# deepsphere/deepsphere-cosmo-tf2

Measured on AMD Instinct MI355X. Metric: Mpix*channels/s Chebyshev-conv fwd, nside=1024 K=5 F=64; HBM roofline %, higher is better.
Workload: dtype f32 (recurrence f32; contraction 3-pass split-bf16 MFMA with f32 accumulate; precision 'bf16x3' = the layer default for 64 input channels)

## Files before the change

deepsphere-cosmo-tf2_amd/csrc/cheb_qstrip_kernel.h:

```cpp
#pragma once

#include <type_traits>

#include "cheb_qtape.h"

namespace dsph {

constexpr int QS_PX = 64;
constexpr int QS_D = 4;
constexpr int QS_USE = QS_PX - 2 * QS_D;
constexpr int QS_THREADS = 512;
constexpr int QS_RUNIN = 2 * QS_D + 1;

struct QStripArgs {
  const float* x;
  const float* bias;
  float* y;
  const unsigned char* wimg;
  const float* gvals8;
  const float* gdiag;
  const QStrip* strips;
  const int32_t* tab;
  const int32_t* prefix;
  int64_t x_rows, y_rows;
  int nstrips, N, Fin, Fout, ld, act;
  int pieces, wg_per_piece;
  float xsc, xsc_inv;
#ifdef DSPH_QS_STAMPS
  unsigned* stamps;
#endif
};

#ifdef DSPH_QS_STAMPS
#define QS_STAMP(id)                                                                                          \
  do {                                                                                                        \
    if (stamp_on) {                                                                                           \
      unsigned long long t_;                                                                                  \
      asm volatile("s_memtime %0\n\ts_waitcnt lgkmcnt(0)" : "=s"(t_)::"memory");                              \
      if (lane == 0) a.stamps[(wave * 4 + (stamp_step & 3)) * 10 + (id)] = (unsigned)t_;                      \
    }                                                                                                         \
  } while (0)
#define QS_STAMP_DECL                                                                                         \
  const int stamp_step = ytop - (st.y0 - D) - 60;                                                             \
  const bool stamp_on = blockIdx.x == 72 && stamp_step >= 0 && stamp_step < 4;
#else
#define QS_STAMP(id)
#define QS_STAMP_DECL
#endif

#ifdef DSPH_QS_ABL
#define QS_ABL DSPH_QS_ABL
#else
#define QS_ABL 0
#endif

#if QS_ABL & 64
#define QS_FD "v_fmac_f32_e32 "
#define QS_DPPL "\n\t"
#define QS_DPPR "\n\t"
#else
#define QS_FD "v_fmac_f32_dpp "
#define QS_DPPL " row_shr:1 row_mask:0xf bank_mask:0xf bound_ctrl:1\n\t"
#define QS_DPPR " row_shl:1 row_mask:0xf bank_mask:0xf bound_ctrl:1\n\t"
#endif

template <bool F16> __device__ __forceinline__ void qs_m(qs_f4& acc, const qs_bf8& wa, const qs_bf8& bb) {
  if (QS_ABL & 2) { asm volatile("" : "+v"(acc) : "v"(wa), "v"(bb) : "memory"); return; }
  if (F16) asm volatile("v_mfma_f32_16x16x32_f16 %0, %1, %2, %0" : "+v"(acc) : "v"(wa), "v"(bb) : "memory");
  else asm volatile("v_mfma_f32_16x16x32_bf16 %0, %1, %2, %0" : "+v"(acc) : "v"(wa), "v"(bb) : "memory");
}
template <bool F16> __device__ __forceinline__ void qs_m0(qs_f4& acc, const qs_bf8& wa, const qs_bf8& bb) {
  if (QS_ABL & 2) { acc = qs_f4{0.f, 0.f, 0.f, 0.f}; asm volatile("" : "+v"(acc) : "v"(wa), "v"(bb) : "memory"); return; }
  if (F16) asm volatile("v_mfma_f32_16x16x32_f16 %0, %1, %2, 0" : "=&v"(acc) : "v"(wa), "v"(bb) : "memory");
  else asm volatile("v_mfma_f32_16x16x32_bf16 %0, %1, %2, 0" : "=&v"(acc) : "v"(wa), "v"(bb) : "memory");
}
template <int N> __device__ __forceinline__ void qs_settle(QRow& r) {
  if (N == 9) asm volatile("s_nop 9" : "+v"(r.t[0]), "+v"(r.t[1]), "+v"(r.t[2]), "+v"(r.t[3]) : : "memory");
  else asm volatile("s_nop 1" : "+v"(r.t[0]), "+v"(r.t[1]), "+v"(r.t[2]), "+v"(r.t[3]) : : "memory");
}

template <bool INIT, bool NEG>
__device__ __forceinline__ void qs_u12(float& a0, float& a1, float& a2, float& a3, float s0, float s1, float s2, float s3,
                                       const qs_f4& cw, const qs_f4& cc, const qs_f4& ce) {
  if ((QS_ABL & 64) && NEG) { qs_u12<INIT, false>(a0, a1, a2, a3, s0, s1, s2, s3, cw, cc, ce); return; }
  const float w0 = cw[0], w1 = cw[1], w2 = cw[2], w3 = cw[3], c0 = cc[0], c1 = cc[1], c2 = cc[2], c3 = cc[3], e0 = ce[0], e1 = ce[1],
              e2 = ce[2], e3 = ce[3];
#define QS_OPS_IN "v"(s0), "v"(s1), "v"(s2), "v"(s3), "v"(w0), "v"(w1), "v"(w2), "v"(w3), "v"(c0), "v"(c1), "v"(c2), "v"(c3), "v"(e0), "v"(e1), "v"(e2), "v"(e3)
  if (!INIT && !NEG)
    asm volatile(
        "v_fmac_f32_e32 %0, %4, %12\n\tv_fmac_f32_e32 %1, %5, %13\n\tv_fmac_f32_e32 %2, %6, %14\n\tv_fmac_f32_e32 %3, %7, %15\n\t"
        "v_fmac_f32_e32 %1, %4, %9\n\tv_fmac_f32_e32 %2, %5, %10\n\tv_fmac_f32_e32 %3, %6, %11\n\t"
        "v_fmac_f32_e32 %0, %5, %16\n\tv_fmac_f32_e32 %1, %6, %17\n\tv_fmac_f32_e32 %2, %7, %18\n\t"
        QS_FD "%0, %7, %8" QS_DPPL QS_FD "%3, %4, %19" QS_DPPR
        : "+v"(a0), "+v"(a1), "+v"(a2), "+v"(a3)
        : QS_OPS_IN
        : "memory");
  else if (!INIT && NEG)
    asm volatile(
        "v_fma_f32 %0, %4, -%12, %0\n\tv_fma_f32 %1, %5, -%13, %1\n\tv_fma_f32 %2, %6, -%14, %2\n\tv_fma_f32 %3, %7, -%15, %3\n\t"
        "v_fma_f32 %1, %4, -%9, %1\n\tv_fma_f32 %2, %5, -%10, %2\n\tv_fma_f32 %3, %6, -%11, %3\n\t"
        "v_fma_f32 %0, %5, -%16, %0\n\tv_fma_f32 %1, %6, -%17, %1\n\tv_fma_f32 %2, %7, -%18, %2\n\t"
        QS_FD "%0, %7, -%8" QS_DPPL QS_FD "%3, %4, -%19" QS_DPPR
        : "+v"(a0), "+v"(a1), "+v"(a2), "+v"(a3)
        : QS_OPS_IN
        : "memory");
  else if (INIT && !NEG)
    asm volatile(
        "v_mul_f32_e32 %0, %4, %12\n\tv_mul_f32_e32 %1, %5, %13\n\tv_mul_f32_e32 %2, %6, %14\n\tv_mul_f32_e32 %3, %7, %15\n\t"
        "v_fmac_f32_e32 %1, %4, %9\n\tv_fmac_f32_e32 %2, %5, %10\n\tv_fmac_f32_e32 %3, %6, %11\n\t"
        "v_fmac_f32_e32 %0, %5, %16\n\tv_fmac_f32_e32 %1, %6, %17\n\tv_fmac_f32_e32 %2, %7, %18\n\t"
        QS_FD "%0, %7, %8" QS_DPPL QS_FD "%3, %4, %19" QS_DPPR
        : "=&v"(a0), "=&v"(a1), "=&v"(a2), "=&v"(a3)
        : QS_OPS_IN
        : "memory");
  else
    asm volatile(
        "v_mul_f32_e64 %0, %4, -%12\n\tv_mul_f32_e64 %1, %5, -%13\n\tv_mul_f32_e64 %2, %6, -%14\n\tv_mul_f32_e64 %3, %7, -%15\n\t"
        "v_fma_f32 %1, %4, -%9, %1\n\tv_fma_f32 %2, %5, -%10, %2\n\tv_fma_f32 %3, %6, -%11, %3\n\t"
        "v_fma_f32 %0, %5, -%16, %0\n\tv_fma_f32 %1, %6, -%17, %1\n\tv_fma_f32 %2, %7, -%18, %2\n\t"
        QS_FD "%0, %7, -%8" QS_DPPL QS_FD "%3, %4, -%19" QS_DPPR
        : "=&v"(a0), "=&v"(a1), "=&v"(a2), "=&v"(a3)
        : QS_OPS_IN
        : "memory");
#undef QS_OPS_IN
}
template <bool INIT, bool NEG>
__device__ __forceinline__ void qs_unit(QRow& acc, const QRow& src, int e, const qs_f4& cw, const qs_f4& cc, const qs_f4& ce) {
  if ((QS_ABL & 4) && !INIT) {
    asm volatile("" : "+v"(acc.t[0]), "+v"(acc.t[1]), "+v"(acc.t[2]), "+v"(acc.t[3]) : "v"(src.t[0]), "v"(src.t[3]), "v"(cw), "v"(cc), "v"(ce) : "memory");
    return;
  }
#define QS_UE(E)                                                                                                          \
  {                                                                                                                       \
    float a0 = 0.f, a1 = 0.f, a2 = 0.f, a3 = 0.f;                                                                         \
    if (!INIT) { a0 = acc.t[0][E]; a1 = acc.t[1][E]; a2 = acc.t[2][E]; a3 = acc.t[3][E]; }                                \
    qs_u12<INIT, NEG>(a0, a1, a2, a3, src.t[0][E], src.t[1][E], src.t[2][E], src.t[3][E], cw, cc, ce);                    \
    acc.t[0][E] = a0; acc.t[1][E] = a1; acc.t[2][E] = a2; acc.t[3][E] = a3;                                               \
  }
  if (e == 0) QS_UE(0)
  else if (e == 1) QS_UE(1)
  else if (e == 2) QS_UE(2)
  else QS_UE(3)
#undef QS_UE
}

#define QS_UPR 4
#define QS_UNIT qs_unit

__host__ __device__ constexpr float qs_wsign(bool cheb, int j) { return cheb && ((j & 3) >= 2) ? -1.f : 1.f; }

template <bool CHEB, bool F16>
__global__ __launch_bounds__(QS_THREADS, 2) void cheb_qstrip5_kernel(QStripArgs a) {
  constexpr int K = 5, D = QS_D, RING = K + 2;
#ifdef DSPH_QS_NOH1
  constexpr bool H1 = false;
#else
  constexpr bool H1 = CHEB;
#endif
  constexpr int ROWB = 2 * 2 * 4 * QS_FRAG;
  constexpr int RINGB = RING * ROWB;
  constexpr int HAND1 = 2 * 4 * QS_FRAG;
  constexpr int HANDB = 4 * HAND1;
  constexpr int CRING = K + 1;
  constexpr int CRINGB = CRING * QS_CROWB;
  constexpr int LDS_HAND = RINGB, LDS_C = RINGB + HANDB, LDS_FLAG = LDS_C + CRINGB;
  __shared__ __attribute__((aligned(16))) unsigned char smem[LDS_FLAG + 64];

  const int tid = threadIdx.x, lane = tid & 63;
  const int wave = __builtin_amdgcn_readfirstlane(tid >> 6);
  const bool roleL = wave >= 4;
  const int oq = wave & 3;
  const int p = lane & 15, q4 = lane >> 4;
  const unsigned lane16 = (unsigned)lane * 16u;
  const unsigned hand = (unsigned)LDS_HAND + (unsigned)oq * HAND1 + lane16;
  const unsigned flag_addr = (unsigned)LDS_FLAG + 4u * (unsigned)oq;
  auto flag_set = [&](int v) __attribute__((always_inline)) { qt_flag_set(flag_addr, v); };
  auto flag_get = [&]() __attribute__((always_inline)) -> int { return qt_flag_get(flag_addr); };
  for (int i = tid; i < (LDS_FLAG + 64) / 16; i += QS_THREADS) reinterpret_cast<qs_f4*>(smem)[i] = qs_f4{0.f, 0.f, 0.f, 0.f};

  const QTapePiece wg = qt_piece(a.wg_per_piece);
  if (wg.piece >= a.pieces) return;
  const QTapeRange tape = qt_tape_range(a.prefix, a.nstrips, wg.piece, a.pieces);
  auto locate = [&](int64_t r, int64_t r_end, QStrip& st) __attribute__((always_inline)) -> int {
    return qt_locate(a.prefix, a.strips, a.nstrips, r, r_end, st);
  };
  const unsigned xrowb = (unsigned)a.Fin * 4u, yrowb = (unsigned)a.ld * 4u;

#if defined(DSPH_QS_XALL)
  constexpr bool X_BY_H = false;
#elif defined(DSPH_QS_XBYH)
  constexpr bool X_BY_H = true;
#else
  constexpr bool X_BY_H = !H1;
#endif
  constexpr int XN = X_BY_H ? 4 : 2;
  const int xt = wave & 3, xpix = X_BY_H ? ((lane >> 1) & 15) : (((lane >> 1) & 7) + 8 * (wave >> 2));
  const unsigned x_goff = X_BY_H ? (unsigned)(2 * (lane >> 5) + (lane & 1)) * 16u
                                 : (unsigned)(lane >> 5) * 64u + (unsigned)(2 * ((lane >> 4) & 1) + (lane & 1)) * 16u;
  const unsigned x_loff = (unsigned)xt * QS_FRAG + (unsigned)(lane & 1) * 8u +
                          (X_BY_H ? (unsigned)(xpix + 16 * (lane >> 5)) * 16u : (unsigned)(xpix + 16 * (2 * (lane >> 5) + ((lane >> 4) & 1))) * 16u);
  auto tab_lane = [&](const QStrip& st, unsigned ci, int yrow) __attribute__((always_inline)) -> unsigned {
    return qt_tab_lane(a.tab, st, ci, min(max(yrow, st.ylo), st.yhi));
  };
  auto my_of = [&](int yrow) __attribute__((always_inline)) -> unsigned { return st_spread((unsigned)yrow & 15u) << 1; };
  auto my_next = [&](unsigned m) __attribute__((always_inline)) -> unsigned { return ((m | 0x55u) + 1u) & 0xaau; };
  auto xfetch = [&](const char* xmap, unsigned xrow, qs_f4 (&xv)[XN]) __attribute__((always_inline)) {
    if (QS_ABL & 8) {
#pragma unroll
      for (int i = 0; i < XN; ++i) xv[i] = qs_f4{0.f, 0.f, 0.f, 0.f};
      return;
    }
    const char* src = xmap + (size_t)(xrow * xrowb + x_goff);
#pragma unroll
    for (int i = 0; i < XN; ++i) xv[i] = *reinterpret_cast<const qs_f4*>(src + (X_BY_H ? 64 : 128) * i);
  };
  auto xw_wait = [&](qs_f4 (&xv)[XN]) __attribute__((always_inline)) {
    if (X_BY_H) asm volatile("" : "+v"(xv[0]), "+v"(xv[1]), "+v"(xv[XN - 2]), "+v"(xv[XN - 1]) : : "memory");
    else asm volatile("" : "+v"(xv[0]), "+v"(xv[1]) : : "memory");
  };
  auto xstore = [&](int slot, const qs_f4 (&xv)[XN]) __attribute__((always_inline)) {
    if (QS_ABL & 4096) {
#pragma unroll
      for (int i = 0; i < XN; ++i) asm volatile("" : : "v"(xv[i]));
      return;
    }
    unsigned char* q = smem + (unsigned)slot * ROWB + x_loff;
#pragma unroll
    for (int i = 0; i < XN; ++i) {
      const unsigned fo = X_BY_H ? (unsigned)(i >> 1) * (2 * 4 * QS_FRAG) + (unsigned)(i & 1) * (32u * 16u) : (unsigned)i * (2 * 4 * QS_FRAG);
      qs_u2 hi, lo;
#pragma unroll
      for (int j = 0; j < 2; ++j) {
        const float a0 = F16 ? xv[i][2 * j] * a.xsc : xv[i][2 * j], a1 = F16 ? xv[i][2 * j + 1] * a.xsc : xv[i][2 * j + 1];
        const qs_u2 hl = qt_split<F16>(a0, a1);
        hi[j] = hl[0];
        lo[j] = hl[1];
      }
      *reinterpret_cast<qs_u2*>(q + fo) = hi;
      *reinterpret_cast<qs_u2*>(q + fo + 4 * QS_FRAG) = lo;
    }
  };
  auto cfetch = [&](unsigned rid, qs_f4& cv, float& cd) __attribute__((always_inline)) { qt_cfetch(a.gvals8, a.gdiag, rid, q4, cv, cd); };
  auto cw_wait = [&](qs_f4& cv, float& cd) __attribute__((always_inline)) {
    asm volatile("" : "+v"(cv), "+v"(cd) : : "memory");
  };
  auto cstore = [&](int slot, qs_f4 cv, float cd) __attribute__((always_inline)) {
    if (CHEB) { cv = cv + cv; cd = cd + cd; }
    unsigned char* q = smem + LDS_C + (unsigned)slot * QS_CROWB + (unsigned)p * 16u + (unsigned)oq * 4u;
    if (q4 < 2) {
#pragma unroll
      for (int d = 0; d < 4; ++d) *reinterpret_cast<float*>(q + (unsigned)(1 + 4 * q4 + d) * 256u) = cv[d];
    }
    if (q4 == 2) *reinterpret_cast<float*>(q) = cd;
  };
  constexpr bool C_OFF = (QS_ABL & 1024) != 0;
  auto clo_read = [&](int slot) __attribute__((always_inline)) -> QCoefLo { return qt_clo_read<C_OFF>(smem + LDS_C, slot, p); };
  auto chi_read = [&](int slot) __attribute__((always_inline)) -> QCoefHi { return qt_chi_read<C_OFF>(smem + LDS_C, slot, p); };

#if QS_ABL & 512
#define QS_FRLOAD(P) (wr[0][0][0])
#else
#define QS_FRLOAD(P) (*reinterpret_cast<const qs_bf8*>(P))
#endif
#define QS_ORD_A(j) ((j) == 1 ? 1 : 0)
#define QS_ORD_B(j) ((j) == 0 ? 1 : 0)
#define QS_FR0(FADDR)                                                                                                     \
  _Pragma("unroll") for (int u = 0; u < 2; ++u) {                                                                         \
    fr[0][u][0] = QS_FRLOAD(smem + (FADDR) + (unsigned)u * QS_FRAG);                                                      \
    fr[0][u][1] = QS_FRLOAD(smem + (FADDR) + (unsigned)(4 + u) * QS_FRAG);                                                \
  }
#define QS_SETS(S0, S1, ROW, ZERO, WLEV, FADDR, NU, ...)                                                                  \
  _Pragma("unroll") for (int s = (S0); s < (S1); ++s) {                 \
    if (s + 1 < 4) {                                                                                                      \
      _Pragma("unroll") for (int u = 0; u < 2; ++u) {                                                                     \
        const unsigned fo = (unsigned)(((s + 1) >> 1) * 8 + ((s + 1) & 1) * 2 + u) * QS_FRAG;                             \
        fr[(s + 1) & 1][u][0] = QS_FRLOAD(smem + (FADDR) + fo);                                                           \
        fr[(s + 1) & 1][u][1] = QS_FRLOAD(smem + (FADDR) + fo + 4 * QS_FRAG);                                             \
      }                                                                                                                   \
    }                                                                                                                     \
    _Pragma("unroll") for (int j = 0; j < 3; ++j) {                                                                       \
      _Pragma("unroll") for (int u = 0; u < 2; ++u) {                                                                     \
        const int m = (s * 3 + j) * 2 + u;                                                                                \
        const int tt = (s & 1) * 2 + u;                                                                                   \
        const qs_bf8& wa_ = wr[WLEV][s >> 1][QS_ORD_A(j)];                                                                \
        const qs_bf8& bb_ = fr[s & 1][u][QS_ORD_B(j)];                                                                    \
        if ((ZERO) && s < 2 && j == 0) qs_m0<F16>((ROW).t[tt], wa_, bb_);                                                 \
        else qs_m<F16>((ROW).t[tt], wa_, bb_);                                                                            \
        _Pragma("unroll") for (int qq = (m * (NU)) / 18; qq < ((m + 1) * (NU)) / 18 && m < 18; ++qq) { __VA_ARGS__; }     \
      }                                                                                                                   \
    }                                                                                                                     \
  }
#define QS_CHAIN(ROW, ZERO, WLEV, FADDR, NU, TAIL, ...)                                                                   \
  {                                                                                                                       \
    QS_SETS(0, 3, ROW, ZERO, WLEV, FADDR, NU, __VA_ARGS__)                                                                \
    TAIL;                                                                                                                 \
    QS_SETS(3, 4, ROW, ZERO, WLEV, FADDR, NU, __VA_ARGS__)                                                                \
  }

  __syncthreads();

  if (!roleL) {
    qs_bf8 wr[4][2][2];
    if (H1) {
      const unsigned char* wp1 = a.wimg + ((size_t)(1 * 4 + oq) * 3) * (2 * 2 * QS_FRAG) + lane16;
#pragma unroll
      for (int kb = 0; kb < 2; ++kb)
#pragma unroll
        for (int h = 0; h < 2; ++h) wr[3][kb][h] = *reinterpret_cast<const qs_bf8*>(wp1 + (size_t)(kb * 2 + h) * QS_FRAG);
    }
    {
      const unsigned char* wp = a.wimg + ((size_t)(0 * 4 + oq) * 3) * (2 * 2 * QS_FRAG) + lane16;
#pragma unroll
      for (int l = 0; l < 3; ++l)
#pragma unroll
        for (int kb = 0; kb < 2; ++kb)
#pragma unroll
          for (int h = 0; h < 2; ++h) wr[l][kb][h] = *reinterpret_cast<const qs_bf8*>(wp + ((size_t)(l * 2 + kb) * 2 + h) * QS_FRAG);
    }
    int handed = 0;
    for (int64_t tr = tape.begin; tr < tape.end;) {
      QStrip st;
      tr += locate(tr, tape.end, st);
      for (int nq = wg.map0; nq < a.N; nq += a.wg_per_piece) {
      const int Xc = min(max(st.xs + 4 * p + oq, st.xlo), st.xhi);
      const int Xf = min(max(st.xs + 4 * xpix + xt, st.xlo), st.xhi);
      const int tc0 = max(st.xs, st.xlo) >> 4;
      const unsigned ciC = (unsigned)((Xc >> 4) - tc0), mXc = st_spread((unsigned)Xc & 15u);
      const unsigned ciF = (unsigned)((Xf >> 4) - tc0), mXf = st_spread((unsigned)Xf & 15u);
      const int T3 = ((st.y1 - st.y0) + 2 * D + 1 + 3) / 3;
      const char* __restrict__ xmap = reinterpret_cast<const char*>(a.x) + (size_t)nq * a.x_rows * xrowb;
      QRow R[2][3];
#pragma unroll
      for (int i = 0; i < 2; ++i)
#pragma unroll
        for (int s = 0; s < 3; ++s)
#pragma unroll
          for (int t = 0; t < 4; ++t) R[i][s].t[t] = qs_f4{0.f, 0.f, 0.f, 0.f};
      int ytop = st.y0 - D, slot_top = 0, cs_top = 0;
      qt_step_barrier();
      {
        qs_f4 cv, xv[XN];
        float cd;
        cfetch(qt_row_in(st, tab_lane(st, ciC, ytop - 1), mXc, ytop - 1), cv, cd);
        xfetch(xmap, qt_row_in(st, tab_lane(st, ciF, ytop), mXf, ytop), xv);
        cw_wait(cv, cd);
        cstore(CRING - 1, cv, cd);
        xw_wait(xv);
        xstore(0, xv);
      }
      unsigned bXf = tab_lane(st, ciF, ytop + 1), bXc = tab_lane(st, ciC, ytop);
      unsigned myX = my_of(ytop + 1), myC = my_of(ytop);
      qt_step_barrier();
      auto step = [&](auto ph_c) __attribute__((always_inline)) {
        constexpr int PH = decltype(ph_c)::value;
        constexpr int L0 = PH % 3, L1 = (PH + 1) % 3, L2 = (PH + 2) % 3;
        int snew = slot_top + 1;
        snew = snew == RING ? 0 : snew;
        auto slot_ix = [&](int back) __attribute__((always_inline)) -> int {
          int s = slot_top - back;
          s += s < 0 ? RING : 0;
          return s;
        };
        auto cslot_ix = [&](int back) __attribute__((always_inline)) -> int {
          int s = cs_top - back;
          s += s < 0 ? CRING : 0;
          return s;
        };
        QS_STAMP_DECL
        QS_STAMP(0);
        qs_f4 xv[XN];
        constexpr bool XLATE = H1;
        if (myX == 0) bXf = tab_lane(st, ciF, ytop + 1);
        if (myC == 0) bXc = tab_lane(st, ciC, ytop);
        if (!XLATE) xfetch(xmap, bXf + (mXf | myX), xv);
        const unsigned f0 = (unsigned)slot_top * ROWB + lane16, f1 = (unsigned)slot_ix(1) * ROWB + lane16, f2 = (unsigned)slot_ix(2) * ROWB + lane16;
        const unsigned f3 = (unsigned)slot_ix(3) * ROWB + lane16;
        constexpr bool N3 = CHEB;
        qs_bf8 fr[2][2][2];
        QCoefLo c3 = clo_read(cslot_ix(1));
        QS_FR0(f0)
        QCoefLo c2;
        QCoefHi c3h, c2h;
        qs_f4 cv;
        float cd;
        QS_CHAIN(R[0][L2], true, 0, f0, 2 * QS_UPR, { c2 = clo_read(cslot_ix(2)); QS_FR0(f1) },
                 { if (qq < QS_UPR) QS_UNIT<true, N3>(R[1][L2], R[0][L0], qq, QS_LO0(c3)); else QS_UNIT<false, N3>(R[1][L2], R[0][L1], qq - QS_UPR, QS_LO1(c3)); })
        qs_settle<9>(R[0][L2]);
        qs_settle<1>(R[1][L2]);
        QS_STAMP(1);
        QS_CHAIN(R[1][L2], false, 1, f1, 2 * QS_UPR, { c3h = chi_read(cslot_ix(1)); QS_FR0(f2) },
                 { if (qq < QS_UPR) QS_UNIT<!CHEB, false>(R[0][L0], R[1][L0], qq, QS_LO0(c2)); else QS_UNIT<false, false>(R[0][L0], R[1][L1], qq - QS_UPR, QS_LO1(c2)); })
        qs_settle<9>(R[1][L2]);
        qs_settle<1>(R[0][L0]);
        if (XLATE) xfetch(xmap, bXf + (mXf | myX), xv);
        QS_STAMP(2);
        QS_CHAIN(R[0][L0], false, 2, f2, QS_UPR, { c2h = chi_read(cslot_ix(2)); cfetch(bXc + (mXc | myC), cv, cd); if (H1) { QS_FR0(f3) } },
                 { QS_UNIT<false, N3>(R[1][L2], R[0][L2], qq, QS_HI(c3h)); })
        qs_settle<9>(R[0][L0]);
        qs_settle<1>(R[1][L2]);
        QS_STAMP(3);
        if (H1) {
          QS_CHAIN(R[1][L0], false, 3, f3, QS_UPR, {}, { QS_UNIT<false, false>(R[0][L0], R[1][L2], qq, QS_HI(c2h)); })
          qs_settle<9>(R[1][L0]);
        } else {
#pragma unroll
          for (int qq = 0; qq < QS_UPR; ++qq) QS_UNIT<false, false>(R[0][L0], R[1][L2], qq, QS_HI(c2h));
        }
        QS_STAMP(4);
        for (int spin = 0; flag_get() <= handed && spin < (1 << 22); ++spin) {}
        if (!(QS_ABL & 2048)) {
          unsigned char* hp = smem + hand;
#pragma unroll
          for (int t = 0; t < 4; ++t) {
            *reinterpret_cast<qs_f4*>(hp + t * QS_FRAG) = R[0][L0].t[t];
            if (CHEB) *reinterpret_cast<qs_f4*>(hp + (4 + t) * QS_FRAG) = R[1][L0].t[t];
          }
        }
        ++handed;
        QS_STAMP(5);
        xw_wait(xv);
        cw_wait(cv, cd);
        QS_STAMP(6);
        cstore(cs_top, cv, cd);
        xstore(snew, xv);
        QS_STAMP(7);
        slot_top = snew;
        cs_top = cs_top + 1 == CRING ? 0 : cs_top + 1;
        ++ytop;
        myX = my_next(myX);
        myC = my_next(myC);
        qt_step_barrier();
        QS_STAMP(8);
      };
      for (int t3 = 0; t3 < T3; ++t3) {
        step(std::integral_constant<int, 0>{});
        step(std::integral_constant<int, 1>{});
        step(std::integral_constant<int, 2>{});
      }
      }
    }
  } else {
    qs_bf8 wr[2][2][2];
    {
      const unsigned char* wp = a.wimg + ((size_t)(1 * 4 + oq) * 3) * (2 * 2 * QS_FRAG) + lane16;
#pragma unroll
      for (int l = 0; l < 2; ++l)
#pragma unroll
        for (int kb = 0; kb < 2; ++kb)
#pragma unroll
          for (int h = 0; h < 2; ++h) wr[l][kb][h] = *reinterpret_cast<const qs_bf8*>(wp + ((size_t)(l * 2 + kb) * 2 + h) * QS_FRAG);
    }
    const float floor_v = a.act == DSPH_ACT_RELU ? 0.f : -__builtin_huge_valf();
    const float ysc = (CHEB ? 0.5f : 1.f) * (F16 ? *reinterpret_cast<const float*>(a.wimg + 2 * 4 * 3 * 2 * 2 * QS_FRAG) * a.xsc_inv : 1.f);
#ifdef DSPH_QS_LPRIO
#define QS_STR2(x) #x
#define QS_STR(x) QS_STR2(x)
    asm volatile("s_setprio " QS_STR(DSPH_QS_LPRIO));
#endif
    qs_f4 bv = qs_f4{0.f, 0.f, 0.f, 0.f};
    if (a.bias != nullptr) bv = *reinterpret_cast<const qs_f4*>(a.bias + 16 * oq + 4 * q4);
    int taken = 0;
    for (int64_t tr = tape.begin; tr < tape.end;) {
      QStrip st;
      tr += locate(tr, tape.end, st);
      for (int nq = wg.map0; nq < a.N; nq += a.wg_per_piece) {
      const int Xf = min(max(st.xs + 4 * xpix + xt, st.xlo), st.xhi);
      const int tc0 = max(st.xs, st.xlo) >> 4;
      const unsigned ciF = (unsigned)((Xf >> 4) - tc0), mXf = st_spread((unsigned)Xf & 15u);
      const int Xg = st.xs + 4 * p;
      const unsigned ciY = (unsigned)((min(max(Xg, st.xlo), st.xhi) >> 4) - tc0), mXg = st_spread((unsigned)Xg & 12u);
      const int cfirst = st.x0 - st.xs, clast = cfirst + st.w;
      const int T3 = ((st.y1 - st.y0) + 2 * D + 1 + 3) / 3;
      const char* __restrict__ xmap = reinterpret_cast<const char*>(a.x) + (size_t)nq * a.x_rows * xrowb;
      char* __restrict__ ymap = reinterpret_cast<char*>(a.y) + (size_t)nq * a.y_rows * yrowb;
      QRow R[2][3], Y;
#pragma unroll
      for (int i = 0; i < 2; ++i)
#pragma unroll
        for (int s = 0; s < 3; ++s)
#pragma unroll
          for (int t = 0; t < 4; ++t) R[i][s].t[t] = qs_f4{0.f, 0.f, 0.f, 0.f};
#pragma unroll
      for (int t = 0; t < 4; ++t) Y.t[t] = qs_f4{0.f, 0.f, 0.f, 0.f};
      int ytop = st.y0 - D, slot_top = 0, cs_top = 0;
      qt_step_barrier();
      if (!X_BY_H) {
        qs_f4 xv[XN];
        xfetch(xmap, qt_row_in(st, tab_lane(st, ciF, ytop), mXf, ytop), xv);
        xw_wait(xv);
        xstore(0, xv);
      }
      unsigned bXf = X_BY_H ? 0u : tab_lane(st, ciF, ytop + 1), bY = tab_lane(st, ciY, st.y0);
      unsigned myX = my_of(ytop + 1), myY = my_of(ytop - K);
      qt_step_barrier();
      auto step = [&](auto ph_c) __attribute__((always_inline)) {
        constexpr int PH = decltype(ph_c)::value;
        constexpr int L0 = PH % 3, L1 = (PH + 1) % 3, L2 = (PH + 2) % 3;
        int snew = slot_top + 1;
        snew = snew == RING ? 0 : snew;
        auto slot_ix = [&](int back) __attribute__((always_inline)) -> int {
          int s = slot_top - back;
          s += s < 0 ? RING : 0;
          return s;
        };
        auto cslot_ix = [&](int back) __attribute__((always_inline)) -> int {
          int s = cs_top - back;
          s += s < 0 ? CRING : 0;
          return s;
        };
        QS_STAMP_DECL
        QS_STAMP(0);
        qs_f4 xv[XN];
        if (!X_BY_H && myX == 0) bXf = tab_lane(st, ciF, ytop + 1);
        if (myY == 0) bY = tab_lane(st, ciY, ytop - K);
        if (!X_BY_H) xfetch(xmap, bXf + (mXf | myX), xv);
#ifdef DSPH_QS_LEARLY
        constexpr bool LE = CHEB && H1;
#else
        constexpr bool LE = false;
#endif
        QCoefLo c0;
        QCoefHi c0h;
        if (LE) c0 = clo_read(cslot_ix(5));
        if (!(QS_ABL & 2048)) {
          const unsigned char* hp = smem + hand;
#pragma unroll
          for (int t = 0; t < 4; ++t) {
            R[0][L2].t[t] = *reinterpret_cast<const qs_f4*>(hp + t * QS_FRAG);
            if (CHEB) R[1][L2].t[t] = *reinterpret_cast<const qs_f4*>(hp + (4 + t) * QS_FRAG);
          }
        }
        ++taken;
        flag_set(taken);
        const unsigned f1 = (unsigned)slot_ix(4) * ROWB + lane16, f0 = (unsigned)slot_ix(5) * ROWB + lane16;
        constexpr bool N1 = CHEB;
        QS_STAMP(1);
        qs_bf8 fr[2][2][2];
        if (LE) {
#pragma unroll
          for (int t = 0; t < 4; ++t) Y.t[t] = R[0][L0].t[t] + R[0][L0].t[t];
          qs_settle<1>(Y);
#pragma unroll
          for (int qq = 0; qq < 2 * QS_UPR; ++qq) {
            if (qq < QS_UPR) QS_UNIT<false, false>(Y, R[1][L0], qq, QS_LO0(c0)); else QS_UNIT<false, false>(Y, R[1][L1], qq - QS_UPR, QS_LO1(c0));
          }
          qs_settle<1>(Y);
        }
        const QCoefLo c1 = clo_read(cslot_ix(4));
        const QCoefHi c1h = chi_read(cslot_ix(4));
        QS_FR0(f0)
#ifdef DSPH_QS_LBARE
        if (CHEB && H1) {
          c0 = clo_read(cslot_ix(5));
          c0h = chi_read(cslot_ix(5));
#pragma unroll
          for (int qq = 0; qq < 3 * QS_UPR; ++qq) {
            if (qq < QS_UPR) QS_UNIT<false, N1>(R[1][L2], R[0][L0], qq, QS_LO0(c1));
            else if (qq < 2 * QS_UPR) QS_UNIT<false, N1>(R[1][L2], R[0][L1], qq - QS_UPR, QS_LO1(c1));
            else QS_UNIT<false, N1>(R[1][L2], R[0][L2], qq - 2 * QS_UPR, QS_HI(c1h));
          }
#pragma unroll
          for (int t = 0; t < 4; ++t) Y.t[t] = R[0][L0].t[t] + R[0][L0].t[t];
          qs_settle<1>(Y);
#pragma unroll
          for (int qq = 0; qq < 2 * QS_UPR; ++qq) {
            if (qq < QS_UPR) QS_UNIT<false, false>(Y, R[1][L0], qq, QS_LO0(c0)); else QS_UNIT<false, false>(Y, R[1][L1], qq - QS_UPR, QS_LO1(c0));
          }
          qs_settle<1>(R[1][L2]);
#pragma unroll
          for (int qq = 0; qq < QS_UPR; ++qq) QS_UNIT<false, false>(Y, R[1][L2], qq, QS_HI(c0h));
          qs_settle<1>(Y);
          QS_STAMP(2);
          QS_CHAIN(Y, false, 1, f0, 0, {}, {})
          qs_settle<9>(Y);
          QS_STAMP(3);
        } else
#endif
        {
        if (CHEB && !LE) {
#pragma unroll
          for (int t = 0; t < 4; ++t) Y.t[t] = R[0][L0].t[t] + R[0][L0].t[t];
          qs_settle<1>(Y);
        }
        QS_CHAIN(Y, !CHEB, 1, f0, 3 * QS_UPR, { if (!LE) c0 = clo_read(cslot_ix(5)); else c0h = chi_read(cslot_ix(5)); if (!H1) { QS_FR0(f1) } },
                 { if (qq < QS_UPR) QS_UNIT<!CHEB, N1>(R[1][L2], R[0][L0], qq, QS_LO0(c1));
                   else if (qq < 2 * QS_UPR) QS_UNIT<false, N1>(R[1][L2], R[0][L1], qq - QS_UPR, QS_LO1(c1));
                   else QS_UNIT<false, N1>(R[1][L2], R[0][L2], qq - 2 * QS_UPR, QS_HI(c1h)); })
        qs_settle<9>(Y);
        qs_settle<1>(R[1][L2]);
        QS_STAMP(2);
        if (H1 && LE) {
        } else if (H1) {
          c0h = chi_read(cslot_ix(5));
#pragma unroll
          for (int qq = 0; qq < 2 * QS_UPR; ++qq) {
            if (qq < QS_UPR) QS_UNIT<false, false>(Y, R[1][L0], qq, QS_LO0(c0)); else QS_UNIT<false, false>(Y, R[1][L1], qq - QS_UPR, QS_LO1(c0));
          }
        } else {
          QS_CHAIN(R[1][L2], false, 0, f1, 2 * QS_UPR, { c0h = chi_read(cslot_ix(5)); },
                   { if (qq < QS_UPR) QS_UNIT<false, false>(Y, R[1][L0], qq, QS_LO0(c0)); else QS_UNIT<false, false>(Y, R[1][L1], qq - QS_UPR, QS_LO1(c0)); })
        }
        qs_settle<9>(R[1][L2]);
        QS_STAMP(3);
#pragma unroll
        for (int qq = 0; qq < QS_UPR; ++qq) QS_UNIT<false, false>(Y, R[1][L2], qq, QS_HI(c0h));
        }
        QS_STAMP(4);
        if (!X_BY_H) xw_wait(xv);
        QS_STAMP(5);
        {
          const int yr = ytop - K;
          const bool row_ok = yr >= st.y0 && yr < ((QS_ABL & 16) ? st.y0 + 1 : st.y1);
          const unsigned rowg = bY + (mXg | myY);
#pragma unroll
          for (int t = 0; t < 4; ++t) {
            const int c = 4 * p + t;
            if (row_ok && c >= cfirst && c < clast) {
              qs_f4 o;
#pragma unroll
              for (int e = 0; e < 4; ++e) {
                const float v = fmaf(Y.t[t][e], ysc, bv[e]);
                o[e] = F16 ? (v < floor_v ? floor_v : v) : fmaxf(v, floor_v);
              }
              *reinterpret_cast<qs_f4*>(ymap + (size_t)(rowg + (unsigned)((t & 1) + 4 * (t >> 1))) * yrowb + (unsigned)(16 * oq + 4 * q4) * 4u) = o;
            }
          }
        }
        QS_STAMP(6);
        if (!X_BY_H) xstore(snew, xv);
        QS_STAMP(7);
        slot_top = snew;
        cs_top = cs_top + 1 == CRING ? 0 : cs_top + 1;
        ++ytop;
        myX = my_next(myX);
        myY = my_next(myY);
        qt_step_barrier();
        QS_STAMP(8);
      };
      for (int t3 = 0; t3 < T3; ++t3) {
        step(std::integral_constant<int, 0>{});
        step(std::integral_constant<int, 1>{});
        step(std::integral_constant<int, 2>{});
      }
      }
    }
  }
#undef QS_CHAIN
#undef QS_SETS
#undef QS_FR0
#undef QS_FRLOAD
}

}
```

deepsphere-cosmo-tf2_amd/csrc/cheb_qtape.h:

```cpp
#pragma once

#include <algorithm>

#include "cheb_struct_kernel.h"
#include "dsphere_common.h"

namespace dsph {

constexpr int QS_FRAG = 1024;
constexpr int QS_CROWB = 2304;

typedef float qs_f4 __attribute__((ext_vector_type(4)));
typedef int qs_i4 __attribute__((ext_vector_type(4)));
typedef __bf16 qs_bf8 __attribute__((ext_vector_type(8)));
typedef unsigned qs_u2 __attribute__((ext_vector_type(2)));

struct QRow {
  qs_f4 t[4];
};

struct QStrip {
  int32_t x0, w;
  int32_t xs;
  int32_t y0, y1;
  int32_t xlo, xhi;
  int32_t ylo, yhi;
  int32_t tab, tws;
  int32_t pad[1];
};

struct QTapePiece {
  int ord, piece, map0;
};
__device__ __forceinline__ QTapePiece qt_piece(int wg_per_piece) {
  QTapePiece c;
  const int G = gridDim.x;
  c.ord = (blockIdx.x & 7) * (G >> 3) + (blockIdx.x >> 3);
  c.piece = c.ord / wg_per_piece;
  c.map0 = c.ord - c.piece * wg_per_piece;
  return c;
}
struct QTapeRange {
  int64_t begin, end;
};
__device__ __forceinline__ QTapeRange qt_tape_range(const int32_t* prefix, int nstrips, int piece, int pieces) {
  const int64_t tape = (int64_t)prefix[nstrips];
  QTapeRange r;
  r.begin = piece < pieces ? tape * piece / pieces : 0;
  r.end = piece < pieces ? tape * (piece + 1) / pieces : 0;
  return r;
}
__device__ __forceinline__ int qt_locate(const int32_t* prefix, const QStrip* strips, int nstrips, int64_t r, int64_t r_end, QStrip& st) {
  int lo = 0, hi = nstrips;
  while (hi - lo > 1) {
    const int mid = (lo + hi) >> 1;
    if ((int64_t)prefix[mid] <= r) lo = mid; else hi = mid;
  }
  {
    const QStrip g = strips[lo];
#define QS_U(f) st.f = __builtin_amdgcn_readfirstlane(g.f)
    QS_U(x0); QS_U(w); QS_U(xs); QS_U(y0); QS_U(y1); QS_U(xlo); QS_U(xhi); QS_U(ylo); QS_U(yhi); QS_U(tab); QS_U(tws);
#undef QS_U
  }
  const int h = st.y1 - st.y0;
  const int off = (int)(r - (int64_t)prefix[lo]);
  const int len = (int)(((int64_t)(h - off) < r_end - r) ? (int64_t)(h - off) : r_end - r);
  st.y0 += off;
  st.y1 = st.y0 + len;
  return len;
}

__device__ __forceinline__ unsigned qt_tab_lane(const int32_t* tab, const QStrip& st, unsigned ci, int yc) {
  const int32_t* trow = tab + __builtin_amdgcn_readfirstlane(st.tab + (yc >> 4) * st.tws + (max(st.xs, st.xlo) >> 4));
  qs_i4 b;
  int b4;
  asm volatile("s_load_dwordx4 %0, %2, 0x0\n\ts_load_dword %1, %2, 0x10\n\ts_waitcnt lgkmcnt(0)" : "=&s"(b), "=&s"(b4) : "s"(trow) : "memory");
  return (unsigned)(ci == 0 ? b[0] : ci == 1 ? b[1] : ci == 2 ? b[2] : ci == 3 ? b[3] : b4);
}
__device__ __forceinline__ unsigned qt_row_in(const QStrip& st, unsigned base, unsigned mX, int yrow) {
  const int yc = min(max(yrow, st.ylo), st.yhi);
  return base + (mX | (st_spread((unsigned)yc & 15u) << 1));
}

__device__ __forceinline__ void qt_step_barrier() { asm volatile("s_waitcnt lgkmcnt(0)\n\ts_barrier" ::: "memory"); }
__device__ __forceinline__ void qt_flag_set(unsigned addr, int v) { asm volatile("ds_write_b32 %0, %1" : : "v"(addr), "v"(v) : "memory"); }
__device__ __forceinline__ int qt_flag_get(unsigned addr) {
  int v;
  asm volatile("ds_read_b32 %0, %1\n\ts_waitcnt lgkmcnt(0)" : "=v"(v) : "v"(addr) : "memory");
  return v;
}

template <bool F16> __device__ __forceinline__ qs_u2 qt_split(float a0, float a1) {
  typedef __bf16 bf16x2 __attribute__((ext_vector_type(2)));
  typedef _Float16 f16x2 __attribute__((ext_vector_type(2)));
  typedef float f32x2 __attribute__((ext_vector_type(2)));
  qs_u2 r;
  if (F16) {
    const f16x2 h = __builtin_convertvector(f32x2{a0, a1}, f16x2);
    const f32x2 hf = __builtin_convertvector(h, f32x2);
    const f16x2 l = __builtin_convertvector(f32x2{a0 - hf[0], a1 - hf[1]}, f16x2);
    r[0] = __builtin_bit_cast(unsigned, h);
    r[1] = __builtin_bit_cast(unsigned, l);
  } else {
    const bf16x2 h = __builtin_convertvector(f32x2{a0, a1}, bf16x2);
    const unsigned hu = __builtin_bit_cast(unsigned, h);
    const float h0 = __builtin_bit_cast(float, hu << 16), h1 = __builtin_bit_cast(float, hu & 0xffff0000u);
    const bf16x2 l = __builtin_convertvector(f32x2{a0 - h0, a1 - h1}, bf16x2);
    r[0] = hu;
    r[1] = __builtin_bit_cast(unsigned, l);
  }
  return r;
}

struct QCoef3 {
  qs_f4 w, c, e;
};
struct QCoefLo {
  qs_f4 sw, s, se, w, dg, e;
};
struct QCoefHi {
  qs_f4 nw, n, ne;
};
#define QS_LO0(c) (c).sw, (c).s, (c).se
#define QS_LO1(c) (c).w, (c).dg, (c).e
#define QS_HI(c) (c).nw, (c).n, (c).ne

__device__ __forceinline__ void qt_cfetch(const float* gvals8, const float* gdiag, size_t rid, int q4, qs_f4& cv, float& cd) {
  const char* pv = reinterpret_cast<const char*>(gvals8) + rid * 32u + (unsigned)(q4 & 1) * 16u;
  const char* pd = reinterpret_cast<const char*>(gdiag) + rid * 4u;
  cv = *reinterpret_cast<const qs_f4*>(pv);
  cd = *reinterpret_cast<const float*>(pd);
}
template <bool DOUBLE>
__device__ __forceinline__ void qt_cstore(unsigned char* ring, int slot, int p, int q4, int res, qs_f4 cv, float cd) {
  if (DOUBLE) { cv = cv + cv; cd = cd + cd; }
  unsigned char* q = ring + (unsigned)slot * QS_CROWB + (unsigned)p * 16u + (unsigned)res * 4u;
  if (q4 < 2) {
#pragma unroll
    for (int d = 0; d < 4; ++d) *reinterpret_cast<float*>(q + (unsigned)(1 + 4 * q4 + d) * 256u) = cv[d];
  }
  if (q4 == 2) *reinterpret_cast<float*>(q) = cd;
}
__device__ __forceinline__ const unsigned char* qt_crow(const unsigned char* ring, int slot, int p) {
  return ring + (unsigned)slot * QS_CROWB + (unsigned)p * 16u;
}
template <bool NOREAD = false> __device__ __forceinline__ qs_f4 qt_cvec(const unsigned char* q, int v) {
  if (NOREAD) { qs_f4 c = qs_f4{0.1f, 0.1f, 0.1f, 0.1f}; asm volatile("" : "+v"(c)); return c; }
  return *reinterpret_cast<const qs_f4*>(q + (unsigned)v * 256u);
}
template <bool NOREAD = false> __device__ __forceinline__ QCoef3 qt_cvec3(const unsigned char* q, int which) {
  QCoef3 r;
  if (which == 0) { r.w = qt_cvec<NOREAD>(q, 8); r.c = qt_cvec<NOREAD>(q, 7); r.e = qt_cvec<NOREAD>(q, 6); }
  else if (which == 1) { r.w = qt_cvec<NOREAD>(q, 1); r.c = qt_cvec<NOREAD>(q, 0); r.e = qt_cvec<NOREAD>(q, 5); }
  else { r.w = qt_cvec<NOREAD>(q, 2); r.c = qt_cvec<NOREAD>(q, 3); r.e = qt_cvec<NOREAD>(q, 4); }
  return r;
}
template <bool NOREAD = false> __device__ __forceinline__ QCoefLo qt_clo_read(const unsigned char* ring, int slot, int p) {
  const unsigned char* q = qt_crow(ring, slot, p);
  QCoefLo c;
  c.sw = qt_cvec<NOREAD>(q, 8); c.s = qt_cvec<NOREAD>(q, 7); c.se = qt_cvec<NOREAD>(q, 6);
  c.w = qt_cvec<NOREAD>(q, 1); c.dg = qt_cvec<NOREAD>(q, 0); c.e = qt_cvec<NOREAD>(q, 5);
  return c;
}
template <bool NOREAD = false> __device__ __forceinline__ QCoefHi qt_chi_read(const unsigned char* ring, int slot, int p) {
  const unsigned char* q = qt_crow(ring, slot, p);
  QCoefHi c;
  c.nw = qt_cvec<NOREAD>(q, 2); c.n = qt_cvec<NOREAD>(q, 3); c.ne = qt_cvec<NOREAD>(q, 4);
  return c;
}

__device__ __forceinline__ float qt_wimg_pow2(const float* __restrict__ w, int nrows, int ncols, int ld) {
  __shared__ float smax[256];
  float m = 0.f;
  for (int e = threadIdx.x; e < nrows * ncols; e += 256) m = fmaxf(m, fabsf(w[(int64_t)(e / ncols) * ld + e % ncols]));
  smax[threadIdx.x] = m;
  __syncthreads();
  for (int st = 128; st > 0; st >>= 1) {
    if ((int)threadIdx.x < st) smax[threadIdx.x] = fmaxf(smax[threadIdx.x], smax[threadIdx.x + st]);
    __syncthreads();
  }
  int ex = 0;
  const float mx = smax[0];
  float pw = 1.f;
  if (mx > 0.f && mx < 3.0e38f) { (void)frexpf(mx, &ex); pw = ldexpf(1.f, 12 - ex); }
  return pw;
}
__device__ __forceinline__ void qt_wimg_put(unsigned char* base, int idx, float v, bool f16) {
  if (f16) {
    const _Float16 hi = (_Float16)v;
    const _Float16 lo = (_Float16)(v - (float)hi);
    reinterpret_cast<_Float16*>(base)[idx] = hi;
    reinterpret_cast<_Float16*>(base + QS_FRAG)[idx] = lo;
  } else {
    const __bf16 hi = (__bf16)v;
    const __bf16 lo = (__bf16)(v - (float)hi);
    reinterpret_cast<__bf16*>(base)[idx] = hi;
    reinterpret_cast<__bf16*>(base + QS_FRAG)[idx] = lo;
  }
}

template <class Args, class Launch> int qtape_args(Args& a, const Launch& s, int run_in) {
  a.x = s.x;
  a.gvals8 = s.gvals8;
  a.gdiag = s.gdiag;
  a.strips = s.strips;
  a.tab = s.tab;
  a.prefix = s.prefix;
  a.x_rows = s.x_rows;
  a.nstrips = s.nstrips;
  a.N = (int)s.N;
  int grid;
  (void)qtape_split(s.num_cu, s.tape_rows, s.N, s.tape_rows / std::max(1, s.nstrips), run_in, &grid, &a.pieces, &a.wg_per_piece);
  return grid;
}
template <class Args> int qtape_forward_args(Args& a, const QTapeLaunch& s, int run_in) {
  a.bias = s.bias;
  a.y = s.y;
  a.wimg = s.wimg;
  a.y_rows = s.y_rows;
  a.ld = s.ld;
  a.act = s.act;
  a.xsc = s.f16 ? ldexpf(1.f, s.f16_xexp) : 1.f;
  a.xsc_inv = s.f16 ? ldexpf(1.f, -s.f16_xexp) : 1.f;
  return qtape_args(a, s, run_in);
}

}
```

deepsphere-cosmo-tf2_amd/csrc/cheb_qwgrad_kernel.h:

```cpp
#pragma once

#include "cheb_qstrip_kernel.h"

namespace dsph {

#ifdef DSPH_QW_PAD
constexpr bool QW_SWZ = false;
constexpr int QW_SK = 272, QW_SB = 1216;
#else
constexpr bool QW_SWZ = true;
constexpr int QW_SK = 256;
constexpr int QW_SB = 1040;
#endif
constexpr int QW_CG = 2 * QW_SB;
constexpr int QW_HL = 4 * QW_CG;
constexpr int QW_PLANE = 2 * QW_HL;
constexpr int QW_P0 = 0, QW_P2 = 1, QW_Q0 = 2, QW_Q1 = 3, QW_Q2 = 4, QW_NPLANES = 5;
constexpr int QW_PAIRS = 5;
constexpr int QW_SLAB = QW_PAIRS * 64 * 64;

struct QWgradArgs {
  const float* x;
  const float* dy;
  float* slabs;
  const float* gvals8;
  const float* gdiag;
  const QStrip* strips;
  const int32_t* tab;
  const int32_t* prefix;
  int64_t x_rows, dy_rows;
  int nstrips, N, lddy;
  int pieces, wg_per_piece;
};

template <bool CHEB>
__global__ __launch_bounds__(QS_THREADS, 2) void cheb_qwgrad5_kernel(QWgradArgs a) {
  constexpr int D = QS_D;
  constexpr int CRING = 3;
  constexpr int LDS_C = QW_NPLANES * QW_PLANE;
  __shared__ __attribute__((aligned(16))) unsigned char smem[LDS_C + CRING * QS_CROWB];

  const int tid = threadIdx.x, lane = tid & 63;
  const int wave = __builtin_amdgcn_readfirstlane(tid >> 6);
  const bool sideQ = wave >= 4;
  const int cq = wave & 3;
  const int og = wave & 3, fh = wave >> 2;
  const int p = lane & 15, q4 = lane >> 4;
  for (int i = tid; i < (int)sizeof(smem) / 16; i += QS_THREADS) reinterpret_cast<qs_f4*>(smem)[i] = qs_f4{0.f, 0.f, 0.f, 0.f};

  const QTapePiece wg = qt_piece(a.wg_per_piece);
  float* __restrict__ slab = a.slabs + (size_t)blockIdx.x * QW_SLAB;
  const float sgn = (sideQ && (wg.ord & 1)) ? -1.f : 1.f;
  qs_f4 acc[QW_PAIRS][2];
#pragma unroll
  for (int i = 0; i < QW_PAIRS; ++i)
#pragma unroll
    for (int j = 0; j < 2; ++j) acc[i][j] = qs_f4{0.f, 0.f, 0.f, 0.f};

  const QTapeRange tape = qt_tape_range(a.prefix, a.nstrips, wg.piece, a.pieces);
  auto locate = [&](int64_t r, int64_t r_end, QStrip& st) __attribute__((always_inline)) -> int {
    return qt_locate(a.prefix, a.strips, a.nstrips, r, r_end, st);
  };

  const unsigned srowb = sideQ ? (unsigned)a.lddy * 4u : 256u;
  const int64_t srows = sideQ ? a.dy_rows : a.x_rows;
  const char* sbase = reinterpret_cast<const char*>(sideQ ? a.dy : a.x);
  const int kgw = (p >> 1) & 3;
  const unsigned wr_com = (unsigned)cq * QW_CG + (unsigned)(p >> 3) * QW_SB + (unsigned)kgw * QW_SK + (unsigned)(p & 1) * 8u +
                          (unsigned)(4 * (QW_SWZ ? (q4 ^ (kgw >> 1)) : q4)) * 16u;
  const unsigned wr_a = wr_com + ((QW_SWZ && (kgw & 1)) ? 32u : 0u), wr_b = wr_com + ((QW_SWZ && (kgw & 1)) ? 0u : 32u);
  const unsigned rd_off = (unsigned)(lane >> 4) * QW_SK + (unsigned)((lane & 15) ^ (QW_SWZ ? 2 * (lane >> 4) : 0)) * 16u;

  auto cstore = [&](int slot, qs_f4 cv, float cd) __attribute__((always_inline)) { qt_cstore<false>(smem + LDS_C, slot, p, q4, cq, cv, cd); };
  auto crow = [&](int slot, int which) __attribute__((always_inline)) -> QCoef3 { return qt_cvec3(qt_crow(smem + LDS_C, slot, p), which); };

  auto stage = [&](int plane, const QRow& R) __attribute__((always_inline)) {
    if (QS_ABL & 8192) { asm volatile("" : : "v"(R.t[0]), "v"(R.t[1]), "v"(R.t[2]), "v"(R.t[3])); return; }
    unsigned char* qa = smem + (unsigned)plane * QW_PLANE + wr_a;
    unsigned char* qb = smem + (unsigned)plane * QW_PLANE + wr_b;
#pragma unroll
    for (int cc = 0; cc < 4; ++cc) {
      unsigned char* q = (cc < 2 ? qa : qb) + (cc & 1) * 16;
      qs_u2 hi, lo;
#pragma unroll
      for (int j = 0; j < 2; ++j) {
        const float a0 = R.t[2 * j][cc], a1 = R.t[2 * j + 1][cc];
        const qs_u2 hl = qt_split<false>(a0, a1);
        hi[j] = hl[0];
        lo[j] = hl[1];
      }
      *reinterpret_cast<qs_u2*>(q) = hi;
      *reinterpret_cast<qs_u2*>(q + QW_HL) = lo;
    }
  };
  auto frag = [&](int plane, int hl, int cg, int blk) __attribute__((always_inline)) -> qs_bf8 {
    if (QS_ABL & 16384) { qs_bf8 z; asm volatile("v_mov_b32 %0, 0" : "=v"(z)); return z; }
    return *reinterpret_cast<const qs_bf8*>(smem + (unsigned)plane * QW_PLANE + (unsigned)hl * QW_HL + (unsigned)cg * QW_CG + (unsigned)blk * QW_SB + rd_off);
  };

  __syncthreads();

  for (int64_t tr = tape.begin; tr < tape.end;) {
    QStrip st;
    tr += locate(tr, tape.end, st);
    for (int nq = wg.map0; nq < a.N; nq += a.wg_per_piece) {
      unsigned voff[4];
      bool colk[4];
      const int cfirst = st.x0 - st.xs, clast = cfirst + st.w;
      const int xclo = sideQ ? st.x0 : st.xlo, xchi = sideQ ? st.x0 + st.w - 1 : st.xhi;
#pragma unroll
      for (int t = 0; t < 4; ++t) {
        voff[t] = st_spread((unsigned)min(max(st.xs + 4 * p + t, xclo), xchi) & 15u) * srowb + (unsigned)(16 * cq + 4 * q4) * 4u;
        colk[t] = !sideQ || (4 * p + t >= cfirst && 4 * p + t < clast);
      }
      const int Xc = min(max(st.xs + 4 * p + cq, st.xlo), st.xhi);
      const int tc0 = max(st.xs, st.xlo) >> 4;
      const unsigned pk = (unsigned)((min(max(st.xs + 4 * p, xclo), xchi) >> 4) - tc0) | ((unsigned)((Xc >> 4) - tc0) << 4) | (st_spread((unsigned)Xc & 15u) << 8);
      const char* smap = sbase + (size_t)nq * srows * srowb;
      auto tab_lane = [&](unsigned ci, int yc) __attribute__((always_inline)) -> unsigned { return qt_tab_lane(a.tab, st, ci, yc); };
      const int rlo = sideQ ? st.y0 : st.ylo, rhi = sideQ ? st.y1 - 1 : st.yhi;
      unsigned bV = tab_lane(pk & 15u, min(max(st.y0 - D, rlo), rhi)), bC = sideQ ? 0u : tab_lane((pk >> 4) & 15u, min(max(st.y0 - D, st.ylo), st.yhi));
      auto row_fetch = [&](int yrow, QRow& R) __attribute__((always_inline)) {
        const int yc = min(max(yrow, rlo), rhi);
        if (yrow > rlo && yrow <= rhi && (yrow & 15) == 0) bV = tab_lane(pk & 15u, yc);
        const unsigned rb = (bV + (st_spread((unsigned)yc & 15u) << 1)) * srowb;
#pragma unroll
        for (int t = 0; t < 4; ++t) R.t[t] = *reinterpret_cast<const qs_f4*>(smap + (rb + voff[t]));
      };
      const int T3 = ((st.y1 - st.y0) + 2 * D + 1 + 2) / 3;
      QRow S0[3], S1[3];
#pragma unroll
      for (int s = 0; s < 3; ++s)
#pragma unroll
        for (int t = 0; t < 4; ++t) { S0[s].t[t] = qs_f4{0.f, 0.f, 0.f, 0.f}; S1[s].t[t] = qs_f4{0.f, 0.f, 0.f, 0.f}; }
      int ytop = st.y0 - D, cs = 0;
      QRow nx;
      row_fetch(ytop, nx);
      qs_f4 cv = qs_f4{0.f, 0.f, 0.f, 0.f};
      float cd = 0.f;
      auto coef_fetch = [&](int yrow) __attribute__((always_inline)) {
        const int yc = min(max(yrow, st.ylo), st.yhi);
        if (yrow > st.ylo && yrow <= st.yhi && (yrow & 15) == 0) bC = tab_lane((pk >> 4) & 15u, yc);
        const size_t rid = bC + ((pk >> 8) | (st_spread((unsigned)yc & 15u) << 1));
        qt_cfetch(a.gvals8, a.gdiag, rid, q4, cv, cd);
      };
      if (!sideQ) coef_fetch(ytop);

      auto step = [&](auto ph_c) __attribute__((always_inline)) {
        constexpr int PH = decltype(ph_c)::value;
        constexpr int L0 = PH % 3, L1 = (PH + 1) % 3, L2 = (PH + 2) % 3;
        const int cs1 = cs == 0 ? 2 : cs - 1, cs2 = cs1 == 0 ? 2 : cs1 - 1;
        QRow A2;
        QCoef3 ca = crow(cs2, 0), cb = crow(cs2, 1);
        auto unit = [&](auto u_c) __attribute__((always_inline)) {
          constexpr int u = decltype(u_c)::value;
          if (u < 4) QS_UNIT<true, false>(A2, S1[L0], u, ca.w, ca.c, ca.e);
          else if (u < 8) QS_UNIT<false, false>(A2, S1[L1], u - 4, cb.w, cb.c, cb.e);
          else if (u < 12) QS_UNIT<true, false>(S1[L2], S0[L0], u - 8, ca.w, ca.c, ca.e);
          else if (u < 16) QS_UNIT<false, false>(S1[L2], S0[L1], u - 12, cb.w, cb.c, cb.e);
          else if (u < 20) QS_UNIT<false, false>(S1[L2], S0[L2], u - 16, ca.w, ca.c, ca.e);
          else QS_UNIT<false, false>(A2, S1[L2], u - 20, cb.w, cb.c, cb.e);
          if (u == 3) ca = crow(cs1, 0);
          if (u == 7) cb = crow(cs1, 1);
          if (u == 11) ca = crow(cs1, 2);
          if (u == 15) {
            cb = crow(cs2, 2);
            const bool rowk = !sideQ || (ytop >= st.y0 && ytop < st.y1);
            float one = sgn;
            asm volatile("" : "+v"(one));
#pragma unroll
            for (int t = 0; t < 4; ++t) {
              const float mk = (rowk && colk[t]) ? one : 0.f;
#pragma unroll
              for (int e = 0; e < 4; ++e) S0[L2].t[t][e] = nx.t[t][e] * mk;
            }
          }
          if (u == 19) qs_settle<1>(S1[L2]);
        };
        qs_bf8 fa[2][2], fb[2][2];
#pragma unroll
        for (int g = 0; g < 2; ++g)
#pragma unroll
          for (int h = 0; h < 2; ++h) fa[g][h] = frag(QW_P0, h, 2 * fh + g, 0);
#pragma unroll
        for (int h = 0; h < 2; ++h) fb[0][h] = frag(QW_Q0, h, og, 0);
        auto group = [&](auto gi_c) __attribute__((always_inline)) {
          constexpr int gi = decltype(gi_c)::value, blk = gi / 5, g = gi % 5;
          constexpr int pair = g == 0 ? 0 : g == 1 ? 1 : g == 2 ? 3 : g == 3 ? 2 : 4;
          constexpr int bb = (g == 0 || g == 3) ? 0 : 1;
          if (g == 0) { fb[1][0] = frag(QW_Q1, 0, og, blk); fb[1][1] = frag(QW_Q1, 1, og, blk); }
          if (g == 1) { fb[0][0] = frag(QW_Q0, 0, og, blk); fb[0][1] = frag(QW_Q0, 1, og, blk); }
          if (g == 2) {
#pragma unroll
            for (int gg = 0; gg < 2; ++gg)
#pragma unroll
              for (int h = 0; h < 2; ++h) fa[gg][h] = frag(QW_P2, h, 2 * fh + gg, blk);
          }
          if (g == 3) { fb[1][0] = frag(QW_Q2, 0, og, blk); fb[1][1] = frag(QW_Q2, 1, og, blk); }
          if (g == 0 && blk == 1) {
#pragma unroll
            for (int gg = 0; gg < 2; ++gg)
#pragma unroll
              for (int h = 0; h < 2; ++h) fa[gg][h] = frag(QW_P0, h, 2 * fh + gg, 1);
          }
          if (g == 4 && blk == 0) { fb[0][0] = frag(QW_Q0, 0, og, 1); fb[0][1] = frag(QW_Q0, 1, og, 1); }
          auto mf = [&](auto i_c) __attribute__((always_inline)) {
            constexpr int i = decltype(i_c)::value, j = i >> 1, fg = i & 1, m = gi * 6 + i;
            qs_m<false>(acc[pair][fg], fa[fg][j == 1 ? 1 : 0], fb[bb][j == 0 ? 1 : 0]);
            if constexpr (m % 5 == 1 || m % 5 == 3) unit(std::integral_constant<int, 2 * (m / 5) + (m % 5 == 3 ? 1 : 0)>{});
          };
          mf(std::integral_constant<int, 0>{}); mf(std::integral_constant<int, 1>{}); mf(std::integral_constant<int, 2>{});
          mf(std::integral_constant<int, 3>{}); mf(std::integral_constant<int, 4>{}); mf(std::integral_constant<int, 5>{});
        };
        group(std::integral_constant<int, 0>{}); group(std::integral_constant<int, 1>{}); group(std::integral_constant<int, 2>{});
        group(std::integral_constant<int, 3>{}); group(std::integral_constant<int, 4>{}); group(std::integral_constant<int, 5>{});
        group(std::integral_constant<int, 6>{}); group(std::integral_constant<int, 7>{}); group(std::integral_constant<int, 8>{});
        group(std::integral_constant<int, 9>{});
        QRow S2;
#pragma unroll
        for (int t = 0; t < 4; ++t)
#pragma unroll
          for (int e = 0; e < 4; ++e) S2.t[t][e] = CHEB ? fmaf(2.f, A2.t[t][e], -S0[L0].t[t][e]) : A2.t[t][e];
        qt_step_barrier();
        asm volatile("" : : "v"(fa[0][0]), "v"(fa[0][1]), "v"(fa[1][0]), "v"(fa[1][1]), "v"(fb[1][0]), "v"(fb[1][1]), "v"(fb[0][0]), "v"(fb[0][1]));
        if (!sideQ) {
          stage(QW_P0, S0[L0]);
          stage(QW_P2, S2);
        } else {
          stage(QW_Q0, S0[L0]);
          stage(QW_Q1, S1[L1]);
          stage(QW_Q2, S2);
        }
        if (!sideQ) cstore(cs, cv, cd);
        row_fetch(ytop + 1, nx);
        if (!sideQ) coef_fetch(ytop + 1);
        cs = cs == 2 ? 0 : cs + 1;
        ++ytop;
        qt_step_barrier();
      };
      for (int t3 = 0; t3 < T3; ++t3) {
        step(std::integral_constant<int, 0>{});
        step(std::integral_constant<int, 1>{});
        step(std::integral_constant<int, 2>{});
      }
    }
  }
#pragma unroll
  for (int i = 0; i < QW_PAIRS; ++i)
#pragma unroll
    for (int j = 0; j < 2; ++j) asm volatile("s_nop 9\n\ts_nop 9" : "+v"(acc[i][j]) : : "memory");
#pragma unroll
  for (int pr = 0; pr < QW_PAIRS; ++pr)
#pragma unroll
    for (int fg = 0; fg < 2; ++fg)
#pragma unroll
      for (int i = 0; i < 4; ++i)
        slab[((size_t)pr * 64 + (size_t)(16 * (2 * fh + fg) + 4 * (lane >> 4) + i)) * 64 + (size_t)(16 * og + (lane & 15))] = acc[pr][fg][i];
}

}
```

deepsphere-cosmo-tf2_amd/csrc/cheb_struct.hip:

```cpp
#include <stdio.h>
#include <stdlib.h>

#include <algorithm>
#include <vector>

#include "cheb_struct_kernel.h"

namespace dsph {

__host__ __device__ inline void struct_row_body(int64_t r, const int32_t* __restrict__ cols, const float* __restrict__ vals, int W,
                                                int64_t n_rows, float* __restrict__ gvals8, float* __restrict__ gdiag,
                                                unsigned char* __restrict__ flag) {
  constexpr int kDirIndex[9] = {8, 7, 6, 1, 0, 5, 2, 3, 4};
  float out[9];
#pragma unroll
  for (int d = 0; d < 9; ++d) out[d] = 0.f;
  bool ok = r < n_rows;
  if (ok) {
    const int X = (int)st_compress((unsigned)r), Y = (int)st_compress((unsigned)r >> 1);
    unsigned used = 0;
    for (int j = 0; j < W; ++j) {
      const float v = vals[r * W + j];
      if (v == 0.f) continue;
      const unsigned c = (unsigned)cols[r * W + j];
      const int dx = (int)st_compress(c) - X, dy = (int)st_compress(c >> 1) - Y;
      if (dx < -1 || dx > 1 || dy < -1 || dy > 1) { ok = false; continue; }
      const int d = kDirIndex[(dy + 1) * 3 + (dx + 1)];
      if (used & (1u << d)) ok = false;
      used |= 1u << d;
#pragma unroll
      for (int e = 0; e < 9; ++e)
        if (e == d) out[e] = v;
    }
  }
  gdiag[r] = out[0];
#pragma unroll
  for (int d = 0; d < 8; ++d) gvals8[r * 8 + d] = out[d + 1];
  flag[r] = ok ? 1 : 0;
}
__global__ __launch_bounds__(256) void struct_rows_kernel(const int32_t* __restrict__ cols, const float* __restrict__ vals,
                                                          int W, int64_t n_rows, int64_t n_cols,
                                                          float* __restrict__ gvals8, float* __restrict__ gdiag,
                                                          unsigned char* __restrict__ flag) {
  const int64_t r = (int64_t)blockIdx.x * 256 + threadIdx.x;
  if (r >= n_cols) return;
  struct_row_body(r, cols, vals, W, n_rows, gvals8, gdiag, flag);
}

__host__ __device__ inline unsigned char struct_tile_body(int t, const unsigned char* __restrict__ flag, int D, int64_t n_rows,
                                                          int64_t n_cols, int64_t out_rows, int dlimit) {
  const int64_t row0 = (int64_t)t * 256;
  bool ok = D >= 1 && D <= dlimit && row0 + 256 <= out_rows && row0 + 256 <= 0xffffffffLL;
  bool interior = true;
  if (ok) {
    const int X0 = (int)st_compress((unsigned)row0), Y0 = (int)st_compress((unsigned)row0 >> 1);
    if (X0 - D < 0 || Y0 - D < 0 || X0 + ST_TILE + D > 65535 || Y0 + ST_TILE + D > 65535) ok = false;
    for (int gy = -D; ok && gy < ST_TILE + D; ++gy)
      for (int gx = -D; gx < ST_TILE + D; ++gx) {
        const int a = -gx > gx - (ST_TILE - 1) ? -gx : gx - (ST_TILE - 1), b = -gy > gy - (ST_TILE - 1) ? -gy : gy - (ST_TILE - 1);
        const int ring = (a > b ? a : b) > 0 ? (a > b ? a : b) : 0;
        const int64_t rid = (int64_t)st_morton((unsigned)(X0 + gx), (unsigned)(Y0 + gy));
        if (rid >= n_cols) { ok = false; break; }
        if (ring < D && (rid >= n_rows || !flag[rid])) { ok = false; break; }
        if (rid >= out_rows) interior = false;
      }
  }
  return (unsigned char)((ok ? 1 : 0) | (interior ? 2 : 0));
}
__global__ __launch_bounds__(256) void struct_tiles_kernel(const unsigned char* __restrict__ flag, int ntiles, int D,
                                                           int64_t n_rows, int64_t n_cols, int64_t out_rows,
                                                           unsigned char* __restrict__ cls, int dlimit) {
  const int t = blockIdx.x * 256 + threadIdx.x;
  if (t >= ntiles) return;
  cls[t] = struct_tile_body(t, flag, D, n_rows, n_cols, out_rows, dlimit);
}

__global__ __launch_bounds__(256) void struct_wprep_kernel(const float* __restrict__ w, unsigned char* __restrict__ out,
                                                           int Fin, int Fout, int K, int C, int NB, int prec, int ld, int pack) {
  const int blk = blockIdx.x;
  const int nb = blk % NB, k = (blk / NB) % K, c = blk / (NB * K);
  unsigned char* base = out + (size_t)blk * (prec == DSPH_PREC_BF16X6 ? ST_WBLK3 : 2048);
  for (int e = threadIdx.x; e < 512; e += 256) {
    const int l = e >> 3, j = e & 7;
    const int ch = c * 16 + 8 * (l >> 5) + j, col = 32 * nb + (l & 31);
    float v;
    if (pack) {
      const int ci = 16 / pack, cm = 64 / pack;
      v = (ch / ci == col / cm && ch % ci < Fin && col % cm < Fout) ? w[((int64_t)(ch % ci) * K + k) * ld + col % cm] : 0.f;
    }
    else v = (ch < Fin && col < Fout) ? w[((int64_t)ch * K + k) * ld + col] : 0.f;
    if (prec == DSPH_PREC_BF16X6) {
      const unsigned u = __float_as_uint(v);
      const float r = v - __uint_as_float(u & 0xffff0000u);
      const unsigned s = __float_as_uint(r);
      const float q = r - __uint_as_float(s & 0xffff0000u);
      reinterpret_cast<unsigned short*>(base)[l * 8 + j] = (unsigned short)(u >> 16);
      reinterpret_cast<unsigned short*>(base + 1024)[l * 8 + j] = (unsigned short)(s >> 16);
      reinterpret_cast<unsigned short*>(base + 2048)[l * 8 + j] = (unsigned short)(__float_as_uint(q) >> 16);
    } else if (prec == DSPH_PREC_BF16X3) {
      const __bf16 hi = (__bf16)v;
      const __bf16 lo = (__bf16)(v - (float)hi);
      reinterpret_cast<__bf16*>(base)[l * 8 + j] = hi;
      reinterpret_cast<__bf16*>(base + 1024)[l * 8 + j] = lo;
    } else {
      reinterpret_cast<float*>(base + (j >> 2) * 1024)[l * 4 + (j & 3)] = v;
    }
  }
}

int struct_build_rows(const dsph_plan* plan, float** gvals8, float** gdiag, unsigned char** flag) {
  const int64_t n = plan->n_cols;
  DSPH_HIP(hipMalloc((void**)gvals8, (size_t)n * 8 * sizeof(float)));
  DSPH_HIP(hipMalloc((void**)gdiag, (size_t)n * sizeof(float)));
  DSPH_HIP(hipMalloc((void**)flag, (size_t)n));
#ifdef DSPH_HOST_EMU
  for (int64_t r = 0; r < n; ++r) struct_row_body(r, plan->d_cols, plan->d_vals, (int)plan->width, plan->n_rows, *gvals8, *gdiag, *flag);
#else
  hipLaunchKernelGGL(struct_rows_kernel, dim3((unsigned)((n + 255) / 256)), dim3(256), 0, 0, plan->d_cols, plan->d_vals,
                     (int)plan->width, plan->n_rows, plan->n_cols, *gvals8, *gdiag, *flag);
#endif
  DSPH_HIP(hipGetLastError());
  DSPH_HIP(hipDeviceSynchronize());
  return DSPH_OK;
}

__host__ __device__ inline void struct_patch_body(int64_t i, const int32_t* __restrict__ rows, const float* __restrict__ vals,
                                                  float* __restrict__ gvals8, float* __restrict__ gdiag) {
  const int64_t r = rows[i];
  gdiag[r] = vals[9 * i];
#pragma unroll
  for (int d = 0; d < 8; ++d) gvals8[r * 8 + d] = vals[9 * i + 1 + d];
}
__global__ __launch_bounds__(256) void struct_patch_kernel(const int32_t* __restrict__ rows, const float* __restrict__ vals, int64_t n,
                                                           float* __restrict__ gvals8, float* __restrict__ gdiag) {
  const int64_t i = (int64_t)blockIdx.x * 256 + threadIdx.x;
  if (i < n) struct_patch_body(i, rows, vals, gvals8, gdiag);
}
int struct_patch_rows(const dsph_plan* plan, float* gvals8, float* gdiag, const int32_t* rows, const float* vals, int64_t n) {
  (void)plan;
  if (n <= 0) return DSPH_OK;
  int32_t* d_rows = nullptr;
  float* d_vals = nullptr;
  hipError_t e = hipMalloc((void**)&d_rows, (size_t)n * 4);
  if (e == hipSuccess) e = hipMalloc((void**)&d_vals, (size_t)n * 36);
  if (e == hipSuccess) e = hipMemcpy(d_rows, rows, (size_t)n * 4, hipMemcpyHostToDevice);
  if (e == hipSuccess) e = hipMemcpy(d_vals, vals, (size_t)n * 36, hipMemcpyHostToDevice);
  if (e == hipSuccess) {
#ifdef DSPH_HOST_EMU
    for (int64_t i = 0; i < n; ++i) struct_patch_body(i, d_rows, d_vals, gvals8, gdiag);
#else
    hipLaunchKernelGGL(struct_patch_kernel, dim3((unsigned)((n + 255) / 256)), dim3(256), 0, 0, d_rows, d_vals, n, gvals8, gdiag);
#endif
    e = hipGetLastError();
  }
  if (e == hipSuccess) e = hipDeviceSynchronize();
  if (d_rows) (void)hipFree(d_rows);
  if (d_vals) (void)hipFree(d_vals);
  if (e != hipSuccess) return hip_fail(e, "struct_patch_rows");
  return DSPH_OK;
}

int struct_classify_tiles(const dsph_plan* plan, const unsigned char* d_flag, int ntiles, int D, int64_t out_rows,
                          unsigned char* h_cls, int dlimit) {
  unsigned char* d_cls = nullptr;
  DSPH_HIP(hipMalloc((void**)&d_cls, (size_t)ntiles));
#ifdef DSPH_HOST_EMU
  for (int t = 0; t < ntiles; ++t) d_cls[t] = struct_tile_body(t, d_flag, D, plan->n_rows, plan->n_cols, out_rows, dlimit);
#else
  hipLaunchKernelGGL(struct_tiles_kernel, dim3((ntiles + 255) / 256), dim3(256), 0, 0, d_flag, ntiles, D, plan->n_rows,
                     plan->n_cols, out_rows, d_cls, dlimit);
#endif
  hipError_t e = hipGetLastError();
  if (e == hipSuccess) e = hipMemcpy(h_cls, d_cls, (size_t)ntiles, hipMemcpyDeviceToHost);
  (void)hipFree(d_cls);
  if (e != hipSuccess) return hip_fail(e, "struct_classify_tiles");
  return DSPH_OK;
}

__global__ __launch_bounds__(256) void struct_act_kernel(float* __restrict__ y, int64_t rows, int cols, int ld, int act) {
  const int64_t e = (int64_t)blockIdx.x * 256 + threadIdx.x;
  if (e >= rows * cols) return;
  const int64_t r = e / cols;
  const int c = (int)(e - r * cols);
  y[r * ld + c] = apply_act(y[r * ld + c], act);
}

int launch_struct_act(float* y, int64_t rows, int32_t cols, int32_t ld, int32_t act, hipStream_t stream) {
  const int64_t total = rows * cols;
  if (total <= 0) return DSPH_OK;
  hipLaunchKernelGGL(struct_act_kernel, dim3((unsigned)((total + 255) / 256)), dim3(256), 0, stream, y, rows, (int)cols, (int)ld, (int)act);
  DSPH_HIP(hipGetLastError());
  return DSPH_OK;
}

__global__ __launch_bounds__(256) void struct_act_tiles_kernel(float* __restrict__ y, const int32_t* __restrict__ tiles, int64_t y_rows,
                                                               int cols, int ld, int act) {
  const int64_t r0 = (int64_t)tiles[blockIdx.x] * 256;
  const int64_t nr = y_rows - r0 < 256 ? y_rows - r0 : 256;
  float* base = y + ((int64_t)blockIdx.y * y_rows + r0) * ld;
  for (int64_t e = threadIdx.x; e < nr * cols; e += 256) {
    const int64_t r = e / cols;
    const int c = (int)(e - r * cols);
    base[r * ld + c] = apply_act(base[r * ld + c], act);
  }
}

int launch_struct_act_tiles(float* y, const int32_t* d_tiles, int ntiles, int64_t N, int64_t y_rows, int32_t cols, int32_t ld,
                            int32_t act, hipStream_t stream) {
  if (ntiles <= 0 || N <= 0) return DSPH_OK;
  for (int64_t n0 = 0; n0 < N; n0 += 65535) {
    const unsigned nn = (unsigned)(N - n0 < 65535 ? N - n0 : 65535);
    hipLaunchKernelGGL(struct_act_tiles_kernel, dim3((unsigned)ntiles, nn), dim3(256), 0, stream, y + n0 * y_rows * ld, d_tiles, y_rows,
                       (int)cols, (int)ld, (int)act);
    DSPH_HIP(hipGetLastError());
  }
  return DSPH_OK;
}

template <bool BEFORE>
__global__ __launch_bounds__(256) void residual_epilogue_kernel(float* __restrict__ y, const float* __restrict__ skip, int64_t n,
                                                                float alpha, int act, int vec) {
  const int64_t stride = (int64_t)gridDim.x * 256;
  if (vec) {
    const int64_t n4 = n >> 2;
    for (int64_t i = (int64_t)blockIdx.x * 256 + threadIdx.x; i < n4; i += stride) {
      float4 a = reinterpret_cast<float4*>(y)[i];
      const float4 b = reinterpret_cast<const float4*>(skip)[i];
      if (BEFORE) {
        a.x = apply_act(a.x, act) + alpha * b.x; a.y = apply_act(a.y, act) + alpha * b.y;
        a.z = apply_act(a.z, act) + alpha * b.z; a.w = apply_act(a.w, act) + alpha * b.w;
      } else {
        a.x = apply_act(a.x + alpha * b.x, act); a.y = apply_act(a.y + alpha * b.y, act);
        a.z = apply_act(a.z + alpha * b.z, act); a.w = apply_act(a.w + alpha * b.w, act);
      }
      reinterpret_cast<float4*>(y)[i] = a;
    }
    for (int64_t i = 4 * n4 + (int64_t)blockIdx.x * 256 + threadIdx.x; i < n; i += stride)
      y[i] = BEFORE ? apply_act(y[i], act) + alpha * skip[i] : apply_act(y[i] + alpha * skip[i], act);
  } else {
    for (int64_t i = (int64_t)blockIdx.x * 256 + threadIdx.x; i < n; i += stride)
      y[i] = BEFORE ? apply_act(y[i], act) + alpha * skip[i] : apply_act(y[i] + alpha * skip[i], act);
  }
}

int launch_residual_epilogue(float* y, const float* skip, int64_t n, float alpha, int32_t act, bool before, hipStream_t stream) {
  if (n <= 0) return DSPH_OK;
  const int vec = ((reinterpret_cast<uintptr_t>(y) | reinterpret_cast<uintptr_t>(skip)) & 15) == 0;
  const int64_t work = vec ? (n + 3) / 4 : n;
  const unsigned grid = (unsigned)std::min<int64_t>((work + 255) / 256, 256 * 32);
  if (before) hipLaunchKernelGGL(residual_epilogue_kernel<true>, dim3(grid), dim3(256), 0, stream, y, skip, n, alpha, (int)act, vec);
  else hipLaunchKernelGGL(residual_epilogue_kernel<false>, dim3(grid), dim3(256), 0, stream, y, skip, n, alpha, (int)act, vec);
  DSPH_HIP(hipGetLastError());
  return DSPH_OK;
}

bool struct_shape_ok(int32_t Fin, int32_t Fout, int32_t K) {
  const int NB = (Fout + 31) / 32;
  return K >= 2 && K - 1 <= ST_DMAX && Fin >= 4 && Fin % 4 == 0 && Fout >= 1 && Fout <= 64 &&
         K * NB * 2048 <= ST_WSLICE_BYTES;
}

int struct_packs(int32_t Fin, int32_t Fout) { return Fin == 4 && Fout <= 16 ? 4 : (Fin == 8 && Fout <= 32 ? 2 : 0); }

size_t struct_wfrag_bytes(int32_t Fin, int32_t Fout, int32_t K) {
  const int C = (Fin + 15) / 16, NB = struct_packs(Fin, Fout) ? 2 : (Fout + 31) / 32;
  return (size_t)C * K * NB * ST_WBLK3;
}

int launch_cheb_struct(const StructLaunch& s, hipStream_t stream) {
  const int pack = (s.allow_pack && s.N >= 2 && s.x_rows * (int64_t)s.Fin * 4 * 3 < (1ll << 32)) ? struct_packs(s.Fin, s.Fout) : 0;
  const int C = (s.Fin + 15) / 16, NB = pack ? 2 : (s.Fout + 31) / 32;
  int prec = s.precision;
  if (prec == DSPH_PREC_BF16X6 && !(s.K * NB <= 6 || (s.K == 5 && NB == 2))) prec = DSPH_PREC_FP32;
  if (s.prep_weights) {
    hipLaunchKernelGGL(struct_wprep_kernel, dim3(C * s.K * NB), dim3(256), 0, stream, s.w, s.wfrag, (int)s.Fin_w, (int)s.Fout,
                       (int)s.K, C, NB, prec, (int)s.ld, pack);
    DSPH_HIP(hipGetLastError());
  }
  StructArgs a;
  a.x = s.x;
  a.bias = s.bias;
  a.y = s.y;
  a.wfrag = s.wfrag;
  a.tiles = s.tiles;
  a.gvals8 = s.gvals8;
  a.gdiag = s.gdiag;
  a.tabrow = s.tabrow;
  a.tabvals = s.tabvals;
  a.x_rows = s.x_rows;
  a.y_rows = s.y_rows;
  a.ntiles = s.ntiles;
  a.N = pack ? (int)((s.N + pack - 1) / pack) : (int)s.N;
  a.n_maps = (int)s.N;
  a.pack = pack;
  a.Fin = s.Fin;
  a.Fout = s.Fout;
  a.K = s.K;
  a.C = C;
  a.act = s.act;
  a.ld = s.ld;
  a.pool = s.pool;
  a.ypool = s.ypool;
  a.ypool_rows = s.ypool_rows;
  const int grid = std::max(8, std::min(s.num_cu, (s.ntiles + 7) / 8 * 8));
#ifdef DSPH_STAMPS
  static unsigned long long* d_stamps = nullptr;
  constexpr size_t NST = 8 * 8 * 32;
  if (!d_stamps) DSPH_HIP(hipMalloc(&d_stamps, NST * 8));
  DSPH_HIP(hipMemsetAsync(d_stamps, 0, NST * 8, stream));
  a.stamps = d_stamps;
#endif
  void (*kern)(StructArgs) = nullptr;
  const bool tab = s.tabrow != nullptr;
  const bool px = a.pack != 0 || a.pool != 0;
#define DSPH_ST_PICK3(N_, P, CH, TB) (px ? cheb_struct_kernel<N_, P, CH, TB, true> : cheb_struct_kernel<N_, P, CH, TB, false>)
#define DSPH_ST_PICK2(P, CH, TB) (NB == 1 ? DSPH_ST_PICK3(1, P, CH, TB) : DSPH_ST_PICK3(2, P, CH, TB))
#define DSPH_ST_PICK(P, CH) (tab ? DSPH_ST_PICK2(P, CH, true) : DSPH_ST_PICK2(P, CH, false))
  if (prec == DSPH_PREC_BF16X3) kern = s.cheb ? DSPH_ST_PICK(DSPH_PREC_BF16X3, true) : DSPH_ST_PICK(DSPH_PREC_BF16X3, false);
  else if (prec == DSPH_PREC_BF16X6) kern = s.cheb ? DSPH_ST_PICK(DSPH_PREC_BF16X6, true) : DSPH_ST_PICK(DSPH_PREC_BF16X6, false);
  else kern = s.cheb ? DSPH_ST_PICK(DSPH_PREC_FP32, true) : DSPH_ST_PICK(DSPH_PREC_FP32, false);
#undef DSPH_ST_PICK
#undef DSPH_ST_PICK2
#undef DSPH_ST_PICK3
  const int gy = std::max(1, std::min<int>(a.N, s.num_cu / grid));
  hipLaunchKernelGGL(kern, dim3(grid, gy), dim3(ST_THREADS), 0, stream, a);
  DSPH_HIP(hipGetLastError());
#ifdef DSPH_STAMPS
  if (getenv("DSPH_STAMPS_DUMP")) {
    std::vector<unsigned long long> h(NST);
    if (hipStreamSynchronize(stream) == hipSuccess && hipMemcpy(h.data(), d_stamps, NST * 8, hipMemcpyDeviceToHost) == hipSuccess)
      for (int w = 0; w < 8; ++w)
        for (int it = 0; it < 8; ++it) {
          fprintf(stderr, "STSTAMP wave %d item %d:", w, it + 4);
          const unsigned long long* r = &h[((size_t)w * 8 + it) * 32];
          for (int i = 1; i < 18; ++i) fprintf(stderr, " %lld", r[i] && r[i - 1] ? (long long)(r[i] - r[i - 1]) : -1LL);
          fprintf(stderr, " | k2: A %lld B %lld C %lld", (long long)(r[18] - r[6]), (long long)(r[19] - r[18]), (long long)(r[7] - r[19]));
          fprintf(stderr, " | t0 %llu\n", r[0]);
        }
  }
#endif
  return DSPH_OK;
}

}
```

deepsphere-cosmo-tf2_amd/csrc/cheb_tiles.h:

```cpp
#pragma once

#include <map>
#include <mutex>
#include <unordered_map>
#include <vector>

#include "cheb_fused_kernel.h"
#include "cheb_qstrip8_kernel.h"
#include "cheb_qstrip_kernel.h"
#include "cheb_strip_kernel.h"
#include "cheb_struct_kernel.h"

namespace dsph {

struct TileList {
  int32_t* d = nullptr;
  int n = 0, n_interior = 0;
  const int32_t* ptr(int part) const { return part == 2 ? d + n_interior : d; }
  int count(int part) const { return part == 0 ? n : (part == 1 ? n_interior : n - n_interior); }
};

struct TileTables {
  TileList tiles;
  int32_t* d_row = nullptr;
  float* d_vals = nullptr;
  size_t first(int part) const { return part == 2 ? (size_t)tiles.n_interior : 0; }
  const int32_t* rows(int part) const { return d_row + first(part) * ST_CELLS; }
  const float* vals(int part) const { return d_vals + first(part) * ST_CELLS * ST_TABV; }
};

struct QStripSet {
  QStrip* d_strips = nullptr;
  int32_t* d_prefix = nullptr;
  int32_t* d_tab = nullptr;
  int n = 0;
  int64_t tape_rows = 0;
  int64_t n_tiles = 0;
  std::vector<QStrip> h_strips;
  std::vector<int32_t> h_tab;
};

struct FusedTiles {
  int D = 0;
  int width = 0;
  int ntiles = 0;
  int rmax = 0;
  int emax = 0;
  bool ok = false;
  int32_t* d_tile_off = nullptr;
  int32_t* d_ring_end = nullptr;
  int64_t* d_ell_off = nullptr;
  int32_t* d_region = nullptr;
  uint16_t* d_lcols = nullptr;
  float* d_lvals = nullptr;
  TileList part;
  TileList r;
  TileTables t;
  StripPair* d_pairs = nullptr;
  int n_pairs = 0;
  int64_t n_strip_tiles = 0;
  std::vector<int32_t> strip_steps;
  std::vector<StripPair> h_pairs;
  mutable std::map<int64_t, int64_t> strip_span;
  bool strip_forced = false;
  TileList rrest;
  QStripSet q5;
  TileList qrrest;
  TileTables qt;
  QStripSet q8;
  TileList q8rest;
  StripPair* d_ipairs = nullptr;
  int n_ipairs = 0;
  std::vector<int32_t> ipair_h;
  std::vector<unsigned char> ipair_second;
  mutable std::map<int64_t, int> iseg;
  TileList all;
  TileList nonq;
  std::vector<void*> dev;
  void release();
};

struct FusedPlan {
  std::vector<int32_t> h_cols;
  std::vector<float> h_vals;
  std::mutex mu;
  std::map<int, FusedTiles> by_depth;
  int num_cu = 256;
  float* d_gvals8 = nullptr;
  float* d_gdiag = nullptr;
  unsigned char* d_rowflag = nullptr;
  bool rows_tried = false;
  bool host_released = false;
  int symmetric = -1;
  bool wide = false;
  hipStream_t side = nullptr;
  hipEvent_t ev_fork = nullptr, ev_join = nullptr;
  bool side_failed = false;
  std::mutex fork_mu;
  struct Images { uint64_t key = 0; uint32_t mask = 0; };
  std::mutex img_mu;
  std::unordered_map<const void*, Images> images;
};

const FusedTiles& get_tiles(const dsph_plan* plan, int D, bool full = false);
bool fused_symmetric(const dsph_plan* plan);
int64_t strip_makespan(const std::vector<int32_t>& steps, int64_t N, int num_cu);

}
```

deepsphere-cosmo-tf2_amd/csrc/cheb_tiles.hip:

```cpp
#include <stdio.h>
#include <stdlib.h>
#include <string.h>

#include <algorithm>
#include <initializer_list>

#include "cheb_tiles.h"

namespace dsph {

static const int ddx[8] = {-1, -1, 0, 1, 1, 1, 0, -1}, ddy[8] = {0, 1, 1, 1, 0, -1, -1, -1};

static int template_width(int w) {
  if (w <= 9) return 9;
  if (w <= 12) return 12;
  return 0;
}

void FusedTiles::release() {
  for (void* p : dev) (void)hipFree(p);
  *this = FusedTiles();
}

FusedPlan* fused_plan_build(const dsph_plan* plan, const int32_t* h_cols, const float* h_vals) {
  if (template_width(plan->width) == 0 && tstep_width(plan->width) == 0) return nullptr;
  FusedPlan* fp = new FusedPlan();
  fp->wide = template_width(plan->width) == 0;
  const size_t nnz = (size_t)plan->n_rows * plan->width;
  fp->h_cols.assign(h_cols, h_cols + nnz);
  fp->h_vals.assign(h_vals, h_vals + nnz);
  hipDeviceProp_t prop;
  if (hipGetDeviceProperties(&prop, plan->device) == hipSuccess && prop.multiProcessorCount > 0)
    fp->num_cu = prop.multiProcessorCount;
  return fp;
}

void fused_plan_destroy(FusedPlan* fp) {
  if (!fp) return;
  for (auto& kv : fp->by_depth) kv.second.release();
  if (fp->d_gvals8) (void)hipFree(fp->d_gvals8);
  if (fp->d_gdiag) (void)hipFree(fp->d_gdiag);
  if (fp->d_rowflag) (void)hipFree(fp->d_rowflag);
  if (fp->side) {
    (void)hipStreamSynchronize(fp->side);
    (void)hipEventDestroy(fp->ev_fork);
    (void)hipEventDestroy(fp->ev_join);
    (void)hipStreamDestroy(fp->side);
  }
  delete fp;
}

bool fused_host_released(FusedPlan* fp) {
  std::lock_guard<std::mutex> lock(fp->mu);
  return fp->host_released;
}

void fused_plan_invalidate(FusedPlan* fp) {
  if (!fp) return;
  std::lock_guard<std::mutex> lock(fp->mu);
  for (auto& kv : fp->by_depth) kv.second.release();
  fp->by_depth.clear();
}

static bool embed_tile(const dsph_plan* plan, const int32_t* cols, const float* vals, int W, int t, int D, int64_t out_rows,
                       int32_t* row, float* val, bool* interior, std::vector<int32_t>& key, std::vector<int32_t>& slot) {
  const int64_t r0 = (int64_t)t * FUSED_P;
  if (r0 + FUSED_P > out_rows) return false;
  constexpr int S = ST_S;
  int32_t A[S][S];
  for (int y = 0; y < S; ++y)
    for (int x = 0; x < S; ++x) A[x][y] = -1;
  constexpr int HN = 2048;
  key.assign(HN, -1);
  slot.assign(HN, 0);
  auto hput = [&](int32_t r, int cell) {
    unsigned h = ((unsigned)r * 2654435761u) >> 21;
    while (key[h] != -1) h = (h + 1) & (HN - 1);
    key[h] = r;
    slot[h] = cell;
  };
  auto hget = [&](int32_t r) -> int {
    unsigned h = ((unsigned)r * 2654435761u) >> 21;
    while (key[h] != -1) {
      if (key[h] == r) return slot[h];
      h = (h + 1) & (HN - 1);
    }
    return -1;
  };
  for (unsigned y = 0; y < 16; ++y)
    for (unsigned x = 0; x < 16; ++x) {
      const int32_t r = (int32_t)(r0 + st_morton(x, y));
      A[ST_DMAX + x][ST_DMAX + y] = r;
      hput(r, (ST_DMAX + x) + S * (ST_DMAX + y));
    }
  auto propose = [&](int x, int y) -> int32_t {
    int32_t cand[16];
    int nc = -1;
    for (int dy = -1; dy <= 1; ++dy)
      for (int dx = -1; dx <= 1; ++dx) {
        const int ax = x + dx, ay = y + dy;
        if ((dx == 0 && dy == 0) || ax < 0 || ay < 0 || ax >= S || ay >= S || A[ax][ay] < 0) continue;
        const int32_t ar = A[ax][ay];
        if (ar >= plan->n_rows) continue;
        const int32_t* c = cols + (size_t)ar * W;
        const float* v = vals + (size_t)ar * W;
        if (nc < 0) {
          nc = 0;
          for (int j = 0; j < W; ++j)
            if (v[j] != 0.f && c[j] != ar && hget(c[j]) < 0 && nc < 16) cand[nc++] = c[j];
        } else {
          int m = 0;
          for (int i = 0; i < nc; ++i) {
            bool in = false;
            for (int j = 0; j < W && !in; ++j) in = v[j] != 0.f && c[j] == cand[i];
            if (in) cand[m++] = cand[i];
          }
          nc = m;
        }
      }
    return nc == 1 ? cand[0] : (nc > 1 ? -1 : -2);
  };
  auto place = [&](int x, int y) -> bool {
    const int32_t r = propose(x, y);
    if (r == -1) return false;
    if (r == -2) { A[x][y] = -2; return true; }
    A[x][y] = r;
    hput(r, x + S * y);
    return true;
  };
  for (int rho = 1; rho <= D; ++rho) {
    const int lo = ST_DMAX - rho, hi = ST_DMAX + ST_TILE - 1 + rho;
    const int mid = (lo + hi) / 2;
    for (int k = 0; k <= hi - lo; ++k) {
      const int off = (k + 1) / 2 * ((k & 1) ? 1 : -1);
      const int u = mid + off;
      if (u <= lo || u >= hi) continue;
      if (!place(u, hi) || !place(u, lo) || !place(lo, u) || !place(hi, u)) return false;
    }
    if (!place(lo, lo) || !place(hi, lo) || !place(lo, hi) || !place(hi, hi)) return false;
  }
  const int blo = ST_DMAX - D, bhi = ST_DMAX + ST_TILE - 1 + D;
  for (int p = 0; p < ST_CELLS; ++p) {
    row[p] = (int32_t)r0;
    for (int j = 0; j < ST_TABV; ++j) val[(size_t)p * ST_TABV + j] = 0.f;
  }
  *interior = true;
  for (int y = blo; y <= bhi; ++y)
    for (int x = blo; x <= bhi; ++x) {
      const int32_t r = A[x][y];
      const unsigned p = st_cell_off((unsigned)x, (unsigned)y) / 64u;
      if (r < 0) continue;
      row[p] = r;
      if (r >= out_rows) *interior = false;
      if (x == blo || x == bhi || y == blo || y == bhi) continue;
      if (r >= plan->n_rows) return false;
      const int32_t* c = cols + (size_t)r * W;
      const float* v = vals + (size_t)r * W;
      float* o = val + (size_t)p * ST_TABV;
      unsigned seen = 0;
      for (int j = 0; j < W; ++j) {
        if (v[j] == 0.f) continue;
        int d = -1;
        if (c[j] == r) d = 0;
        else {
          const int cell = hget(c[j]);
          if (cell < 0) return false;
          const int dx = cell % S - x, dy = cell / S - y;
          for (int q = 0; q < 8; ++q)
            if (ddx[q] == dx && ddy[q] == dy) d = q + 1;
          if (d < 0) return false;
        }
        if (seen & (1u << d)) return false;
        seen |= 1u << d;
        o[d] = v[j];
      }
    }
  return true;
}

static int strip_grid(int num_cu, int64_t n_items) { return (int)std::max<int64_t>(8, std::min<int64_t>(num_cu, (n_items + 7) / 8 * 8)); }
int64_t strip_makespan(const std::vector<int32_t>& steps, int64_t N, int num_cu) {
  const int64_t Q = (int64_t)steps.size() * N;
  const int G = strip_grid(num_cu, Q);
  int64_t worst = 0;
  std::vector<int64_t> load;
  for (int xcd = 0; xcd < 8; ++xcd) {
    const int nslots = (G + 7 - xcd) / 8;
    const int64_t q0 = Q * xcd / 8, q1 = Q * (xcd + 1) / 8;
    if (nslots <= 0 || q1 <= q0) continue;
    load.assign((size_t)nslots, 0);
    for (int64_t q = q0; q < q1; ++q) load[(size_t)((q - q0) % nslots)] += steps[(size_t)(q / N)];
    for (int64_t v : load) worst = std::max(worst, v);
  }
  return worst;
}

struct TileRect { int tx, ty, wt, ht; };
static void cut_strip_pairs(const std::vector<TileRect>& take, int D, int h, std::vector<StripPair>& out) {
  out.clear();
  for (const TileRect& r : take) {
    const int X0 = 16 * r.tx, X1 = 16 * (r.tx + r.wt), Y0 = 16 * r.ty, Y1 = 16 * (r.ty + r.ht);
    const int ns = (X1 - X0 + SP_USE - 1) / SP_USE;
    const int H = Y1 - Y0, nseg = (H + h - 1) / h;
    for (int sg = 0; sg < nseg; ++sg) {
      const int ya = Y0 + (int)((int64_t)H * sg / nseg), yb = Y0 + (int)((int64_t)H * (sg + 1) / nseg);
      for (int s0 = 0; s0 < ns; s0 += 2) {
        StripPair p;
        for (int e = 0; e < 2; ++e) {
          const int s = s0 + e;
          if (s < ns) {
            p.x0[e] = X0 + SP_USE * s;
            p.w[e] = std::min(SP_USE, X1 - p.x0[e]);
          } else {
            p.x0[e] = p.x0[0];
            p.w[e] = 0;
          }
        }
        p.y0 = ya;
        p.y1 = yb;
        p.xlo = X0 - D;
        p.xhi = X1 - 1 + D;
        for (int e = 0; e < 2; ++e)
          p.xs[e] = std::min(p.x0[e] - D, p.xhi + 1 - SP_PX);
        p.ylo = Y0 - D;
        p.yhi = Y1 - 1 + D;
        out.push_back(p);
      }
    }
  }
  bool ragged = false;
  for (const StripPair& p : out) ragged = ragged || (p.y1 - p.y0 != out[0].y1 - out[0].y0);
  if (ragged) {
    std::stable_sort(out.begin(), out.end(), [](const StripPair& a, const StripPair& b) { return a.y1 - a.y0 > b.y1 - b.y0; });
    std::vector<StripPair> dealt;
    dealt.reserve(out.size());
    for (size_t x = 0; x < 8; ++x)
      for (size_t i2 = x; i2 < out.size(); i2 += 8) dealt.push_back(out[i2]);
    out.swap(dealt);
  }
}

constexpr int SMALL_MAP_TILES = 512;
static void build_strips(const std::vector<int32_t>& r_interior, int D, int num_cu, const PlanOptions& opt,
                         std::vector<StripPair>& pairs, std::vector<int32_t>& rest, int64_t* n_taken, std::vector<int32_t>& steps,
                         std::vector<StripPair>& whole) {
  steps.clear();
  pairs.clear();
  whole.clear();
  rest.clear();
  *n_taken = 0;
  std::vector<uint64_t> keys(r_interior.size());
  for (size_t i = 0; i < r_interior.size(); ++i) {
    const unsigned t = (unsigned)r_interior[i];
    keys[i] = ((uint64_t)st_compress(t) << 32) | st_compress(t >> 1);
  }
  std::sort(keys.begin(), keys.end());
  struct Run { int tx, y0, y1; bool used; };
  std::vector<Run> runs;
  for (size_t i = 0; i < keys.size();) {
    const int tx = (int)(keys[i] >> 32), y0 = (int)(keys[i] & 0xffffffffu);
    size_t j = i + 1;
    while (j < keys.size() && (int)(keys[j] >> 32) == tx && (int)(keys[j] & 0xffffffffu) == y0 + (int)(j - i)) ++j;
    runs.push_back({tx, y0, y0 + (int)(j - i), false});
    i = j;
  }
  auto overlap = [](int a0, int a1, int b0, int b1, int* o0, int* o1) { *o0 = std::max(a0, b0); *o1 = std::min(a1, b1); return *o1 - *o0; };
  const int min_rows = std::max(4, opt.strip_min_rows);
  std::vector<TileRect> take;
  for (size_t i = 0; i < runs.size(); ++i) {
    if (runs[i].used) continue;
    std::vector<size_t> chain{i};
    int y0 = runs[i].y0, y1 = runs[i].y1;
    while (chain.size() < 6) {
      const int want = runs[chain.back()].tx + 1;
      size_t best = runs.size();
      int by0 = 0, by1 = 0;
      for (size_t j = chain.back() + 1; j < runs.size() && runs[j].tx <= want; ++j) {
        int o0, o1;
        if (runs[j].tx == want && !runs[j].used && overlap(y0, y1, runs[j].y0, runs[j].y1, &o0, &o1) >= min_rows &&
            (best == runs.size() || o1 - o0 > by1 - by0)) { best = j; by0 = o0; by1 = o1; }
      }
      if (best == runs.size()) break;
      if (chain.size() < 5) { y0 = by0; y1 = by1; }
      chain.push_back(best);
    }
    const int avail = (int)chain.size();
    if (avail < 3 || y1 - y0 < min_rows) continue;
    const int w = avail >= 6 ? 3 : std::min(avail, 5);
    y0 = runs[chain[0]].y0; y1 = runs[chain[0]].y1;
    for (int c = 1; c < w; ++c) { int o0, o1; overlap(y0, y1, runs[chain[c]].y0, runs[chain[c]].y1, &o0, &o1); y0 = o0; y1 = o1; }
    if (y1 - y0 < min_rows) continue;
    take.push_back({runs[chain[0]].tx, y0, w, y1 - y0});
    *n_taken += (int64_t)w * (y1 - y0);
    for (int c = 0; c < w; ++c) {
      Run& r = runs[chain[c]];
      for (int y = r.y0; y < r.y1; ++y)
        if (y < y0 || y >= y1) rest.push_back((int32_t)st_morton((unsigned)r.tx, (unsigned)y));
      r.used = true;
    }
  }
  for (const Run& r : runs)
    if (!r.used)
      for (int y = r.y0; y < r.y1; ++y) rest.push_back((int32_t)st_morton((unsigned)r.tx, (unsigned)y));
  std::sort(rest.begin(), rest.end());
#ifdef DSPH_ABLATE
  if (getenv("DSPH_STRIP_DEBUG")) {
    long a3 = 0, a45 = 0;
    int hmin = 1 << 30, hmax = 0;
    for (const TileRect& r : take) { (r.wt == 3 ? a3 : a45) += (long)r.wt * r.ht; hmin = std::min(hmin, r.ht); hmax = std::max(hmax, r.ht); }
    fprintf(stderr, "build_strips: %zu rectangles (3 wide: %ld tiles, 4-5 wide: %ld tiles, heights %d..%d), %zu tiles left over\n",
            take.size(), a3, a45, take.empty() ? 0 : hmin, hmax, rest.size());
  }
#endif
  if (take.empty()) return;
  auto steps_of = [&](const std::vector<StripPair>& v, std::vector<int32_t>& st) {
    st.resize(v.size());
    for (size_t i2 = 0; i2 < v.size(); ++i2) st[i2] = (v[i2].y1 - v[i2].y0) + 2 * D + 1;
  };
  const int cand[] = {4096, 2048, 1024, 512, 384, 256};
  int64_t best_span = -1;
  int best_h = 256;
  {
    std::vector<StripPair> trial;
    std::vector<int32_t> st;
    for (int h : cand) {
      cut_strip_pairs(take, D, h, trial);
      steps_of(trial, st);
      const int64_t span = strip_makespan(st, 1, num_cu);
      if (best_span < 0 || span < best_span) { best_span = span; best_h = h; }
    }
  }
  if (opt.strip_seg > 0) best_h = std::max(16, opt.strip_seg);
  cut_strip_pairs(take, D, best_h, pairs);
  steps_of(pairs, steps);
  cut_strip_pairs(take, D, 1 << 30, whole);
#ifdef DSPH_ABLATE
  if (getenv("DSPH_STRIP_DEBUG"))
    fprintf(stderr, "build_strips: segments of %d rows, %zu pairs, busiest workgroup %ld / %ld / %ld steps for 1 / 4 / 16 maps; tile cost "
            "per map in the same unit %ld\n", best_h, pairs.size(), (long)strip_makespan(steps, 1, num_cu), (long)strip_makespan(steps, 4, num_cu),
            (long)strip_makespan(steps, 16, num_cu), (long)(*n_taken * 187 / (30 * num_cu)));
#endif
}

struct QCand {
  int32_t tile;
  int32_t nbr[8];
  int32_t tix;
  int32_t sheet, u, v;
  bool taken;
  bool barred;
};

static bool links_from_table(const int32_t* row, int D, int32_t ntiles, int32_t nbr[8]) {
  for (int d = 0; d < 8; ++d) {
    const int xa = ddx[d] < 0 ? ST_DMAX - D : (ddx[d] == 0 ? ST_DMAX : ST_DMAX + ST_TILE);
    const int xb = ddx[d] < 0 ? ST_DMAX : (ddx[d] == 0 ? ST_DMAX + ST_TILE : ST_DMAX + ST_TILE + D);
    const int ya = ddy[d] < 0 ? ST_DMAX - D : (ddy[d] == 0 ? ST_DMAX : ST_DMAX + ST_TILE);
    const int yb = ddy[d] < 0 ? ST_DMAX : (ddy[d] == 0 ? ST_DMAX + ST_TILE : ST_DMAX + ST_TILE + D);
    int64_t base = -1;
    for (int y = ya; y < yb; ++y)
      for (int x = xa; x < xb; ++x) {
        const int64_t r = row[st_cell_off((unsigned)x, (unsigned)y) / 64u];
        const int64_t b = r - (int64_t)st_morton((unsigned)(x - ST_DMAX) & 15u, (unsigned)(y - ST_DMAX) & 15u);
        if (b < 0 || (b & (FUSED_P - 1)) != 0 || (base >= 0 && b != base)) return false;
        base = b;
      }
    if (base < 0 || base / FUSED_P >= ntiles) return false;
    nbr[d] = (int32_t)(base / FUSED_P);
  }
  return true;
}

static int64_t qt_gain(int w, int h, int D) {
  const int use = D == Q8_D ? Q8_USE : QS_PX - 2 * D;
  const int64_t ns = (16 * (int64_t)w + use - 1) / use;
  if (D == Q8_D) return (int64_t)w * h * 275 - ns * (16 * (int64_t)h + Q8_RUNIN) * 26;
  return (int64_t)w * h * 187 - ns * (16 * (int64_t)h + 2 * D + 6) * 28;
}

static int32_t assign_sheets(std::vector<QCand>& cands, int32_t ntiles) {
  const int n = (int)cands.size();
  std::vector<int32_t> cand_of((size_t)ntiles, -1);
  for (int i = 0; i < n; ++i) cand_of[(size_t)cands[i].tile] = i;
  auto cand_at = [&](int32_t tile) -> int { return tile >= 0 && tile < ntiles ? cand_of[(size_t)tile] : -1; };
  std::unordered_map<uint64_t, int32_t> at;
  constexpr int64_t OFF = 1 << 20;
  auto key_of = [&](int32_t sheet, int64_t u, int64_t v) { return ((uint64_t)sheet << 44) | ((uint64_t)(u + OFF) << 22) | (uint64_t)(v + OFF); };
  int32_t nsheets = 0;
  std::vector<int32_t> queue;
  for (int i = 0; i < n; ++i) cands[i].sheet = -1;
  for (int i0 = 0; i0 < n; ++i0) {
    if (cands[i0].sheet >= 0) continue;
    if (nsheets >= (1 << 19)) break;
    const int32_t sh = nsheets++;
    cands[i0].sheet = sh; cands[i0].u = 0; cands[i0].v = 0;
    at[key_of(sh, 0, 0)] = i0;
    queue.assign(1, i0);
    for (size_t h = 0; h < queue.size(); ++h) {
      const QCand a = cands[(size_t)queue[h]];
      for (int d = 0; d < 8; d += 2) {
        const int b = cand_at(a.nbr[d]);
        if (b < 0 || cands[(size_t)b].sheet >= 0 || cands[(size_t)b].nbr[(d + 4) & 7] != a.tile) continue;
        const int64_t u = (int64_t)a.u + ddx[d], v = (int64_t)a.v + ddy[d];
        if (u <= -OFF + 2 || u >= OFF - 2 || v <= -OFF + 2 || v >= OFF - 2) continue;
        const uint64_t k = key_of(sh, u, v);
        if (at.find(k) != at.end()) continue;
        cands[(size_t)b].sheet = sh; cands[(size_t)b].u = (int32_t)u; cands[(size_t)b].v = (int32_t)v;
        at[k] = b;
        queue.push_back(b);
      }
    }
  }
  return nsheets;
}

static void deal_low_strips(std::vector<QStrip>& strips) {
  std::vector<QStrip> tall, low;
  int64_t rows_tall = 0, rows_low = 0;
  for (const QStrip& q : strips) {
    if (q.y1 - q.y0 >= 256) { tall.push_back(q); rows_tall += q.y1 - q.y0; }
    else { low.push_back(q); rows_low += q.y1 - q.y0; }
  }
  if (!tall.empty() && !low.empty()) {
    strips.clear();
    size_t li = 0;
    int64_t done_tall = 0, done_low = 0;
    for (const QStrip& q : tall) {
      strips.push_back(q);
      done_tall += q.y1 - q.y0;
      while (li < low.size() && done_low * rows_tall < rows_low * done_tall) {
        strips.push_back(low[li]);
        done_low += low[li].y1 - low[li].y0;
        ++li;
      }
    }
    for (; li < low.size(); ++li) strips.push_back(low[li]);
  }
}

static void build_qtstrips(std::vector<QCand>& cands, int32_t ntiles, int D, std::vector<QStrip>& strips, std::vector<int32_t>& tab,
                           int64_t* n_taken) {
  strips.clear();
  tab.clear();
  *n_taken = 0;
  const int n = (int)cands.size();
  if (n == 0) return;
  const int32_t nsheets = assign_sheets(cands, ntiles);
  std::vector<std::vector<int32_t>> members((size_t)nsheets);
  for (int i = 0; i < n; ++i)
    if (cands[i].sheet >= 0) members[(size_t)cands[i].sheet].push_back(i);
  for (int32_t sh = 0; sh < nsheets; ++sh) {
    const std::vector<int32_t>& mem = members[(size_t)sh];
    if (mem.size() < 6) continue;
    int u0 = 1 << 30, u1 = -(1 << 30), v0 = 1 << 30, v1 = -(1 << 30);
    for (int32_t i : mem) { u0 = std::min(u0, cands[(size_t)i].u); u1 = std::max(u1, cands[(size_t)i].u); v0 = std::min(v0, cands[(size_t)i].v); v1 = std::max(v1, cands[(size_t)i].v); }
    const int64_t GW = (int64_t)u1 - u0 + 1, GH = (int64_t)v1 - v0 + 1;
    if (GW * GH > (1ll << 26)) continue;
    std::vector<int32_t> grid((size_t)(GW * GH), -1);
    for (int32_t i : mem) grid[(size_t)((cands[(size_t)i].v - v0) * GW + (cands[(size_t)i].u - u0))] = cands[(size_t)i].barred ? -2 : i;
    std::vector<int32_t> hgt((size_t)GW);
    std::vector<std::pair<int, int>> stack;
    for (int64_t sweeps = 0; sweeps * GW * GH < (3ll << 28) && sweeps < 8192; ++sweeps) {
      int64_t best = 0;
      int bu = 0, bv = 0, bw = 0, bh = 0;
      std::fill(hgt.begin(), hgt.end(), 0);
      for (int64_t y = 0; y < GH; ++y) {
        for (int64_t x = 0; x < GW; ++x) hgt[(size_t)x] = grid[(size_t)(y * GW + x)] >= 0 ? hgt[(size_t)x] + 1 : 0;
        stack.clear();
        for (int64_t x = 0; x <= GW; ++x) {
          const int hx = x < GW ? hgt[(size_t)x] : 0;
          int start = (int)x;
          while (!stack.empty() && stack.back().second > hx) {
            const int s0 = stack.back().first, hh = stack.back().second;
            stack.pop_back();
            const int wmax = (int)x - s0;
            for (int w = std::min(wmax, 1000); w >= std::max(1, std::min(wmax, 1000) - 3); --w) {
              const int64_t g = qt_gain(w, hh, D);
              if (g > best) { best = g; bu = s0; bv = (int)y - hh + 1; bw = w; bh = hh; }
            }
            start = s0;
          }
          if (hx > 0 && (stack.empty() || stack.back().second < hx)) stack.push_back({start, hx});
        }
      }
      if (best <= 0) break;
      const int TW = bw + 2, TH = bh + 2;
      std::vector<int32_t> t((size_t)TW * TH, -1);
      bool good = true;
      auto inside = [&](int i, int j) { return i >= 1 && i <= bw && j >= 1 && j <= bh; };
      for (int j = 1; j <= bh && good; ++j)
        for (int i = 1; i <= bw && good; ++i) {
          const int32_t c = grid[(size_t)((bv + j - 1) * GW + (bu + i - 1))];
          const QCand& q = cands[(size_t)c];
          t[(size_t)j * TW + i] = q.tile;
          for (int d = 0; d < 8 && good; ++d) {
            const int i2 = i + ddx[d], j2 = j + ddy[d];
            int32_t& slot = t[(size_t)j2 * TW + i2];
            if (inside(i2, j2)) {
              const int32_t c2 = grid[(size_t)((bv + j2 - 1) * GW + (bu + i2 - 1))];
              if (cands[(size_t)c2].tile != q.nbr[d]) good = false;
            } else if (slot < 0) slot = q.nbr[d];
            else if (slot != q.nbr[d]) good = false;
          }
        }
      if (!good) {
        for (int j = 0; j < bh; ++j)
          for (int i = 0; i < bw; ++i) grid[(size_t)((bv + j) * GW + (bu + i))] = -2;
        continue;
      }
      const int32_t toff = (int32_t)tab.size();
      for (int32_t tile : t) tab.push_back(tile < 0 ? 0 : tile * FUSED_P);
      for (int j = 0; j < bh; ++j)
        for (int i = 0; i < bw; ++i) {
          int32_t& c = grid[(size_t)((bv + j) * GW + (bu + i))];
          cands[(size_t)c].taken = true;
          c = -2;
        }
      *n_taken += (int64_t)bw * bh;
      const int X0 = 16, X1 = 16 + 16 * bw, Y0 = 16, Y1 = 16 + 16 * bh;
      const int use = D == Q8_D ? Q8_USE : QS_PX - 2 * D, lead = D == Q8_D ? 8 : D;
      for (int x0 = X0; x0 < X1; x0 += use) {
        QStrip q{};
        q.x0 = x0; q.w = std::min(use, X1 - x0); q.xs = x0 - lead;
        q.y0 = Y0; q.y1 = Y1;
        q.xlo = X0 - D; q.xhi = X1 - 1 + D; q.ylo = Y0 - D; q.yhi = Y1 - 1 + D;
        q.tab = toff; q.tws = TW;
        strips.push_back(q);
      }
    }
  }
  deal_low_strips(strips);
}

struct Graph {
  const dsph_plan* plan;
  const int32_t* cols;
  const float* vals;
  int W;
  int64_t out_rows;
  int ntiles;
};

struct HostList {
  std::vector<int32_t> v;
  int n_interior = 0;
};
static HostList joined(std::vector<int32_t> interior, const std::vector<int32_t>& boundary) {
  HostList h;
  h.n_interior = (int)interior.size();
  h.v = std::move(interior);
  h.v.insert(h.v.end(), boundary.begin(), boundary.end());
  return h;
}

struct TTabs {
  std::vector<int32_t> tiles, rows;
  std::vector<float> vals;
  int n_interior = 0;
  void add(int32_t t, const int32_t* row, const float* val) {
    tiles.push_back(t);
    rows.insert(rows.end(), row, row + ST_CELLS);
    vals.insert(vals.end(), val, val + (size_t)ST_CELLS * ST_TABV);
  }
  void add(const TTabs& o, size_t i) { add(o.tiles[i], &o.rows[i * ST_CELLS], &o.vals[i * ST_CELLS * ST_TABV]); }
};
static TTabs joined(TTabs interior, const TTabs& boundary) {
  interior.n_interior = (int)interior.tiles.size();
  for (size_t i = 0; i < boundary.tiles.size(); ++i) interior.add(boundary, i);
  return interior;
}

struct Embedding {
  std::vector<int32_t> row = std::vector<int32_t>(ST_CELLS), key, slot;
  std::vector<float> val = std::vector<float>((size_t)ST_CELLS * ST_TABV);
  bool interior = false;
  bool run(const Graph& g, int t, int D) {
    return embed_tile(g.plan, g.cols, g.vals, g.W, t, D, g.out_rows, row.data(), val.data(), &interior, key, slot);
  }
};

struct Classes {
  std::vector<int32_t> r_in, r_bd;
  TTabs t_in, t_bd;
  std::vector<int32_t> g_in, g_bd;
};

struct BfsTables {
  std::vector<int32_t> tile_off, ring_end, region;
  std::vector<int64_t> ell_off;
  std::vector<uint16_t> lcols;
  std::vector<float> lvals;
  int rmax = 0, emax = 0;
  int64_t ell_rows = 0;
  std::vector<int32_t> stamp, local, ring, next;
};

struct HostTables {
  BfsTables bfs;
  HostList part, r, rrest, qrrest, q8rest, all, nonq;
  TTabs t, qt;
  std::vector<StripPair> pairs, ipairs;
  std::vector<int32_t> patch_rows;
  std::vector<float> patch_vals;
};

static void ensure_rows(const dsph_plan* plan, FusedPlan* fp) {
  if (fp->rows_tried) return;
  fp->rows_tried = true;
  if (struct_build_rows(plan, &fp->d_gvals8, &fp->d_gdiag, &fp->d_rowflag) != DSPH_OK) {
    if (fp->d_gvals8) (void)hipFree(fp->d_gvals8);
    if (fp->d_gdiag) (void)hipFree(fp->d_gdiag);
    if (fp->d_rowflag) (void)hipFree(fp->d_rowflag);
    fp->d_gvals8 = fp->d_gdiag = nullptr;
    fp->d_rowflag = nullptr;
  }
}

static void classify(const Graph& g, FusedPlan* fp, int D, bool full, std::vector<unsigned char>& cls, std::vector<unsigned char>& cls8) {
  const dsph_plan* plan = g.plan;
  cls.assign((size_t)g.ntiles, 0);
  if (!full && D <= ST_DMAX && plan->opt.use_struct) {
    ensure_rows(plan, fp);
    if (fp->d_rowflag && struct_classify_tiles(plan, fp->d_rowflag, g.ntiles, D, g.out_rows, cls.data()) != DSPH_OK)
      std::fill(cls.begin(), cls.end(), 0);
  }
  if (D == Q8_D && plan->opt.use_struct && plan->opt.strips != 2 && plan->opt.strip_form == 0 && !fp->wide) {
    ensure_rows(plan, fp);
    if (fp->d_rowflag) {
      cls8.assign((size_t)g.ntiles, 0);
      if (struct_classify_tiles(plan, fp->d_rowflag, g.ntiles, D, g.out_rows, cls8.data(), Q8_D) != DSPH_OK) cls8.clear();
    }
  }
}

static void deal_by_parity(std::vector<int32_t>& ring, size_t at) {
  std::vector<int32_t> bucket[4];
  for (int32_t r : ring) bucket[r & 3].push_back(r);
  size_t head[4] = {0, 0, 0, 0};
  size_t left = ring.size();
  ring.clear();
  while (left > 0) {
    const int want = (int)((at + ring.size()) & 3);
    int take = want;
    if (head[take] >= bucket[take].size()) {
      size_t best = 0;
      for (int q = 0; q < 4; ++q) {
        const size_t rem = bucket[q].size() - head[q];
        if (rem > best) { best = rem; take = q; }
      }
    }
    ring.push_back(bucket[take][head[take]++]);
    --left;
  }
}

static void ell_row(const int32_t* c, const float* v, int W, int WT, int i, int E, const int32_t* local, uint16_t* lc, float* lv) {
  for (int j = 0; j < WT; ++j) {
    uint16_t col = (uint16_t)i;
    float val = 0.f;
    if (j < W && v[j] != 0.f) {
      col = (uint16_t)local[c[j]];
      val = v[j];
    }
    lc[(size_t)j * E + i] = col;
    lv[(size_t)j * E + i] = val;
  }
}
static void ell_row_wide(const int32_t* c, const float* v, int W, int WT, int i, int E, int R, const int32_t* local, uint16_t* lc,
                         float* lv) {
  std::vector<std::pair<uint16_t, float>> bucket[4];
  for (int j = 0; j < W; ++j)
    if (v[j] != 0.f) bucket[local[c[j]] & 3].push_back({(uint16_t)local[c[j]], v[j]});
  size_t head[4] = {0, 0, 0, 0};
  for (int j = 0; j < WT; ++j) {
    int b = (i + j) & 3;
    if (head[b] >= bucket[b].size()) {
      size_t best = 0;
      int bb = -1;
      for (int q = 0; q < 4; ++q)
        if (bucket[q].size() - head[q] > best) { best = bucket[q].size() - head[q]; bb = q; }
      b = bb;
    }
    uint16_t col = (uint16_t)i;
    float val = 0.f;
    if (b >= 0) {
      col = bucket[b][head[b]].first;
      val = bucket[b][head[b]].second;
      ++head[b];
    } else {
      const int want = (i & ~3) | ((i + j) & 3);
      col = (uint16_t)(want < R ? want : i);
    }
    lc[(size_t)j * E + i] = col;
    lv[(size_t)j * E + i] = val;
  }
}

static bool bfs_tile(const Graph& g, int t, int D, int WT, bool wide, BfsTables& b, bool* inner) {
  const int64_t r0 = (int64_t)t * FUSED_P, r1 = std::min<int64_t>(g.out_rows, r0 + FUSED_P);
  const size_t base = b.region.size();
  b.ring.clear();
  for (int64_t r = r0; r < r1; ++r) {
    b.stamp[r] = t;
    b.local[r] = (int32_t)(r - r0);
    b.ring.push_back((int32_t)r);
    b.region.push_back((int32_t)r);
  }
  int32_t* re = &b.ring_end[(size_t)t * (FUSED_DMAX + 1)];
  re[0] = (int32_t)b.ring.size();
  for (int d = 1; d <= D; ++d) {
    b.next.clear();
    for (int32_t r : b.ring) {
      if (r >= g.plan->n_rows) return false;
      const int32_t* c = g.cols + (size_t)r * g.W;
      const float* v = g.vals + (size_t)r * g.W;
      for (int j = 0; j < g.W; ++j) {
        if (v[j] == 0.f) continue;
        const int32_t cj = c[j];
        if (b.stamp[cj] != t) {
          b.stamp[cj] = t;
          b.next.push_back(cj);
        }
      }
    }
    std::sort(b.next.begin(), b.next.end());
    deal_by_parity(b.next, b.region.size() - base);
    for (int32_t r : b.next) {
      b.local[r] = (int32_t)(b.region.size() - base);
      b.region.push_back(r);
    }
    re[d] = (int32_t)(b.region.size() - base);
    b.ring.swap(b.next);
  }
  for (int d = D + 1; d <= FUSED_DMAX; ++d) re[d] = re[D];
  const int R = re[D], E = re[D - 1];
  *inner = true;
  for (size_t i = base; i < b.region.size() && *inner; ++i) *inner = b.region[i] < g.out_rows;
  if (R > 65535) return false;
  b.rmax = std::max(b.rmax, R);
  b.emax = std::max(b.emax, E);
  const size_t lbase = b.lcols.size();
  b.lcols.resize(lbase + (size_t)E * WT, 0);
  b.lvals.resize(lbase + (size_t)E * WT, 0.f);
  for (int i = 0; i < E; ++i) {
    const int32_t r = b.region[base + i];
    if (r >= g.plan->n_rows) return false;
    const int32_t* c = g.cols + (size_t)r * g.W;
    const float* v = g.vals + (size_t)r * g.W;
    if (wide) ell_row_wide(c, v, g.W, WT, i, E, R, b.local.data(), &b.lcols[lbase], &b.lvals[lbase]);
    else ell_row(c, v, g.W, WT, i, E, b.local.data(), &b.lcols[lbase], &b.lvals[lbase]);
  }
  b.ell_rows += E;
  return true;
}

static bool sort_tiles(const Graph& g, int D, int WT, bool wide, const std::vector<unsigned char>& cls, bool try_tables,
                       Embedding& em, Classes& c, BfsTables& b) {
  const size_t n_cols = (size_t)g.plan->n_cols;
  b.stamp.assign(n_cols, -1);
  b.local.assign(n_cols, 0);
  b.tile_off.assign((size_t)g.ntiles + 1, 0);
  b.ring_end.assign((size_t)g.ntiles * (FUSED_DMAX + 1), 0);
  b.ell_off.assign((size_t)g.ntiles, 0);
  b.region.reserve((size_t)g.ntiles * 600);
  for (int t = 0; t < g.ntiles; ++t) {
    if (b.region.size() > 0x7fffffffULL - 70000) return false;
    b.tile_off[t] = (int32_t)b.region.size();
    b.ell_off[t] = b.ell_rows;
    if (cls[t] & 1) {
      ((cls[t] & 2) ? c.r_in : c.r_bd).push_back(t);
      continue;
    }
    if (try_tables && em.run(g, t, D)) {
      (em.interior ? c.t_in : c.t_bd).add(t, em.row.data(), em.val.data());
      continue;
    }
    bool inner = false;
    if (!bfs_tile(g, t, D, WT, wide, b, &inner)) return false;
    (inner ? c.g_in : c.g_bd).push_back(t);
  }
  b.tile_off[g.ntiles] = (int32_t)b.region.size();
  return true;
}

static void merge_small_map(const Graph& g, int D, int num_cu, Embedding& em, Classes& c) {
  if ((c.r_in.empty() && c.r_bd.empty()) ||
      c.r_in.size() + c.r_bd.size() + c.t_in.tiles.size() + c.t_bd.tiles.size() > (size_t)SMALL_MAP_TILES)
    return;
  int64_t taken = 0;
  if (g.plan->opt.strips != 2) {
    std::vector<StripPair> p0, ip0;
    std::vector<int32_t> rest0, steps0;
    build_strips(c.r_in, D, num_cu, g.plan->opt, p0, rest0, &taken, steps0, ip0);
  }
  if (taken != 0) return;
  std::vector<int32_t> keep_i, keep_b;
  for (int pass = 0; pass < 2; ++pass)
    for (int32_t t : pass == 0 ? c.r_in : c.r_bd) {
      if (em.run(g, t, D)) (pass == 0 ? c.t_in : c.t_bd).add(t, em.row.data(), em.val.data());
      else (pass == 0 ? keep_i : keep_b).push_back(t);
    }
  c.r_in.swap(keep_i);
  c.r_bd.swap(keep_b);
}

static void pair_strips(const Graph& g, int D, int num_cu, bool full, const Classes& c, FusedTiles& ft, HostTables& h) {
  std::vector<int32_t> rest = c.r_in;
  ft.strip_forced = g.plan->opt.strips == 1;
  if (!full && D <= SP_DMAX && g.plan->opt.strips != 2)
    build_strips(c.r_in, D, num_cu, g.plan->opt, h.pairs, rest, &ft.n_strip_tiles, ft.strip_steps, h.ipairs);
  h.rrest = joined(std::move(rest), c.r_bd);
  ft.n_pairs = (int)h.pairs.size();
  ft.h_pairs = h.pairs;
  ft.n_ipairs = (int)h.ipairs.size();
  for (const StripPair& ip : h.ipairs) {
    ft.ipair_h.push_back(ip.y1 - ip.y0);
    ft.ipair_second.push_back(ip.w[1] > 0 ? 1 : 0);
  }
}

static QCand morton_cand(int32_t t, int ntiles) {
  QCand c{};
  c.tile = t; c.tix = -1; c.taken = false;
  const int tx = (int)st_compress((unsigned)t), ty = (int)st_compress((unsigned)t >> 1);
  for (int d = 0; d < 8; ++d) {
    const int nx = tx + ddx[d], ny = ty + ddy[d];
    const int64_t nt = nx < 0 || ny < 0 ? -1 : (int64_t)st_morton((unsigned)nx, (unsigned)ny);
    c.nbr[d] = nt >= 0 && nt < ntiles ? (int32_t)nt : -1;
  }
  return c;
}

static void quad_strips5(const Graph& g, int D, const Classes& c, FusedTiles& ft, HostTables& h) {
  std::vector<QCand> cands;
  cands.reserve(c.r_in.size() + c.t_in.tiles.size());
  for (int32_t t : c.r_in) cands.push_back(morton_cand(t, g.ntiles));
  const size_t n_rc = cands.size();
  const int32_t ragged = g.out_rows % FUSED_P != 0 ? g.ntiles - 1 : -1;
  auto beside_ragged = [&](const QCand& q) {
    if (ragged < 0) return false;
    if (q.tile == ragged) return true;
    for (int d = 0; d < 8; ++d)
      if (q.nbr[d] == ragged) return true;
    return false;
  };
#ifdef DSPH_ABLATE
  const bool only_r = getenv("DSPH_QT_ONLY_R") != nullptr;
#else
  const bool only_r = false;
#endif
  for (size_t i = 0; i < c.t_in.tiles.size() && !only_r; ++i) {
    QCand q{};
    q.tile = c.t_in.tiles[i]; q.tix = (int32_t)i; q.taken = false;
    if (links_from_table(&c.t_in.rows[i * ST_CELLS], D, g.ntiles, q.nbr)) cands.push_back(q);
  }
  for (QCand& q : cands) q.barred = beside_ragged(q);
  build_qtstrips(cands, g.ntiles, D, ft.q5.h_strips, ft.q5.h_tab, &ft.q5.n_tiles);
  std::vector<int32_t> r_rest;
  std::vector<unsigned char> t_taken(c.t_in.tiles.size(), 0);
  for (size_t i = 0; i < cands.size(); ++i) {
    if (i < n_rc) { if (!cands[i].taken) r_rest.push_back(cands[i].tile); }
    else if (cands[i].taken) t_taken[(size_t)cands[i].tix] = 1;
  }
  h.qrrest = joined(std::move(r_rest), c.r_bd);
  TTabs t_rest;
  for (size_t i = 0; i < c.t_in.tiles.size(); ++i) {
    if (!t_taken[i]) {
      t_rest.add(c.t_in, i);
      continue;
    }
    const int blo = ST_DMAX - D + 1, bhi = ST_DMAX + ST_TILE - 1 + D - 1;
    for (int y = blo; y <= bhi; ++y)
      for (int x = blo; x <= bhi; ++x) {
        const size_t cell = i * ST_CELLS + st_cell_off((unsigned)x, (unsigned)y) / 64u;
        h.patch_rows.push_back(c.t_in.rows[cell]);
        h.patch_vals.insert(h.patch_vals.end(), c.t_in.vals.begin() + cell * ST_TABV, c.t_in.vals.begin() + cell * ST_TABV + 9);
      }
  }
  h.qt = joined(std::move(t_rest), c.t_bd);
}

static void quad_strips8(const Graph& g, int D, const std::vector<unsigned char>& cls8, FusedTiles& ft, HostTables& h) {
  std::vector<QCand> cands;
  for (int32_t t = 0; t < g.ntiles; ++t)
    if ((cls8[(size_t)t] & 3) == 3) cands.push_back(morton_cand(t, g.ntiles));
  build_qtstrips(cands, g.ntiles, D, ft.q8.h_strips, ft.q8.h_tab, &ft.q8.n_tiles);
  std::vector<unsigned char> took((size_t)g.ntiles, 0);
  for (const QCand& q : cands)
    if (q.taken) took[(size_t)q.tile] = 1;
  std::vector<int32_t> rest[2];
  for (size_t i = 0; i < h.part.v.size(); ++i)
    if (!took[(size_t)h.part.v[i]]) rest[i < (size_t)h.part.n_interior ? 0 : 1].push_back(h.part.v[i]);
  h.q8rest = joined(std::move(rest[0]), rest[1]);
}

static std::vector<int32_t> cat(std::initializer_list<const std::vector<int32_t>*> lists) {
  std::vector<int32_t> v;
  for (const std::vector<int32_t>* l : lists) v.insert(v.end(), l->begin(), l->end());
  return v;
}

static void complements(const Classes& c, const FusedTiles& ft, HostTables& h) {
  h.all = joined(cat({&c.r_in, &c.t_in.tiles, &c.g_in}), cat({&c.r_bd, &c.t_bd.tiles, &c.g_bd}));
  h.nonq.v = ft.q5.n_tiles == 0 ? cat({&c.r_in, &c.r_bd, &c.t_in.tiles, &c.t_bd.tiles, &h.part.v}) : cat({&h.qrrest.v, &h.qt.tiles, &h.part.v});
}

template <class T> static bool upload(FusedTiles& ft, T*& dst, std::vector<T>& v) {
  if (v.empty()) v.emplace_back();
  void* p = nullptr;
  if (hipMalloc(&p, v.size() * sizeof(T)) != hipSuccess) return false;
  ft.dev.push_back(p);
  dst = static_cast<T*>(p);
  return hipMemcpy(p, v.data(), v.size() * sizeof(T), hipMemcpyHostToDevice) == hipSuccess;
}
static bool upload(FusedTiles& ft, TileList& dst, HostList& h) {
  dst.n = (int)h.v.size();
  dst.n_interior = h.n_interior;
  return upload(ft, dst.d, h.v);
}
static bool upload(FusedTiles& ft, TileTables& dst, TTabs& h) {
  dst.tiles.n = (int)h.tiles.size();
  dst.tiles.n_interior = h.n_interior;
  return upload(ft, dst.tiles.d, h.tiles) && upload(ft, dst.d_row, h.rows) && upload(ft, dst.d_vals, h.vals);
}
static bool upload(FusedTiles& ft, QStripSet& s) {
  std::vector<QStrip> strips = s.h_strips;
  std::vector<int32_t> prefix(1, 0), tab = s.h_tab;
  for (const QStrip& q : strips) prefix.push_back(prefix.back() + (q.y1 - q.y0));
  s.n = (int)strips.size();
  s.tape_rows = prefix.back();
  tab.resize(tab.size() + 8, 0);
  return upload(ft, s.d_strips, strips) && upload(ft, s.d_prefix, prefix) && upload(ft, s.d_tab, tab);
}
static bool upload_tables(FusedTiles& ft, HostTables& h) {
  BfsTables& b = h.bfs;
  return upload(ft, ft.t, h.t) && upload(ft, ft.d_tile_off, b.tile_off) && upload(ft, ft.d_ring_end, b.ring_end) &&
         upload(ft, ft.d_ell_off, b.ell_off) && upload(ft, ft.d_region, b.region) && upload(ft, ft.d_lcols, b.lcols) &&
         upload(ft, ft.d_lvals, b.lvals) && upload(ft, ft.part, h.part) && upload(ft, ft.r, h.r) && upload(ft, ft.rrest, h.rrest) &&
         upload(ft, ft.nonq, h.nonq) && upload(ft, ft.all, h.all) && upload(ft, ft.d_pairs, h.pairs) && upload(ft, ft.q5) &&
         upload(ft, ft.q8) && upload(ft, ft.q8rest, h.q8rest) && upload(ft, ft.qrrest, h.qrrest) && upload(ft, ft.qt, h.qt) &&
         upload(ft, ft.d_ipairs, h.ipairs);
}

static bool build_tiles(const dsph_plan* plan, FusedPlan* fp, int D, bool full, FusedTiles& ft) {
  const int64_t out_rows = plan->levels.empty() ? plan->n_rows : plan->levels[0];
  const int64_t nt64 = (out_rows + FUSED_P - 1) / FUSED_P;
  if (D < 1 || D > FUSED_DMAX || nt64 > (1 << 30)) return false;
  const Graph g{plan, fp->h_cols.data(), fp->h_vals.data(), plan->width, out_rows, (int)nt64};
  std::vector<unsigned char> cls, cls8;
  classify(g, fp, D, full, cls, cls8);
  const bool try_tables = !full && D <= ST_DMAX && plan->opt.use_struct && plan->opt.use_tables && fp->d_rowflag != nullptr;
  Embedding em;
  Classes c;
  HostTables h;
  if (!sort_tiles(g, D, ft.width, fp->wide, cls, try_tables, em, c, h.bfs)) return false;
  ft.ntiles = g.ntiles;
  ft.rmax = std::max((h.bfs.rmax + 15) / 16 * 16, FUSED_P);
  ft.emax = h.bfs.emax;
  if (try_tables && D <= SP_DMAX) merge_small_map(g, D, fp->num_cu, em, c);
  h.part = joined(c.g_in, c.g_bd);
  pair_strips(g, D, fp->num_cu, full, c, ft, h);
  if (!full && D == QS_D && plan->opt.strips != 2 && plan->opt.strip_form == 0 && fp->d_gvals8 != nullptr)
    quad_strips5(g, D, c, ft, h);
  if (!cls8.empty()) quad_strips8(g, D, cls8, ft, h);
  complements(c, ft, h);
  h.r = joined(c.r_in, c.r_bd);
  h.t = joined(c.t_in, c.t_bd);
  bool good = upload_tables(ft, h);
  if (good && !h.patch_rows.empty())
    good = struct_patch_rows(plan, fp->d_gvals8, fp->d_gdiag, h.patch_rows.data(), h.patch_vals.data(), (int64_t)h.patch_rows.size()) == DSPH_OK;
  if (!good) {
    ft.release();
    ft.D = D;
  }
  return good;
}

const FusedTiles& get_tiles(const dsph_plan* plan, int D, bool full) {
  FusedPlan* fp = plan->fused;
  std::lock_guard<std::mutex> lock(fp->mu);
  DeviceGuard guard(plan->device);
  const int key = 2 * D + (full ? 1 : 0);
  auto it = fp->by_depth.find(key);
  if (it != fp->by_depth.end()) return it->second;
  static const FusedTiles none;
  if (fp->host_released || (fp->wide && !(D == 1 && full))) return none;
  FusedTiles& ft = fp->by_depth[key];
  ft.D = D;
  ft.width = fp->wide ? tstep_width(plan->width) : template_width(plan->width);
  ft.ok = build_tiles(plan, fp, D, full, ft);
  return ft;
}

bool fused_tile_counts(const dsph_plan* plan, int32_t K, int64_t* n_struct, int64_t* n_bfs) {
  if (!plan->fused || K < 2 || K - 1 > FUSED_DMAX) return false;
  const FusedTiles& ft = get_tiles(plan, K - 1, false);
  if (!ft.ok) return false;
  *n_struct = ft.r.n + ft.t.tiles.n;
  *n_bfs = ft.part.n;
  return true;
}

static const QStripSet* record_strips(const dsph_plan* plan, const FusedTiles& ft, int32_t K) {
  const QStripSet* s = K == 5 ? &ft.q5 : (K == Q8_K ? &ft.q8 : nullptr);
  return plan->opt.strip_form == 0 && s && !s->h_strips.empty() ? s : nullptr;
}

int64_t fused_strip_pairs(const dsph_plan* plan, int32_t K, int32_t* out, int64_t cap) {
  if (!plan->fused || K < 2 || K - 1 > FUSED_DMAX) return -1;
  const FusedTiles& ft = get_tiles(plan, K - 1, false);
  if (!ft.ok) return -1;
  static_assert(sizeof(StripPair) == 12 * sizeof(int32_t), "StripPair is twelve int32");
  if (const QStripSet* s = record_strips(plan, ft, K)) {
    const int64_t n = (int64_t)s->h_strips.size();
    for (int64_t i = 0; i < n && i < cap; ++i) {
      const QStrip& q = s->h_strips[(size_t)i];
      const int32_t rec[12] = {q.x0, q.x0, q.w, 0, q.xs, q.xs, q.y0, q.y1, q.xlo, q.xhi, q.ylo, q.yhi};
      memcpy(out + 12 * i, rec, sizeof(rec));
    }
    return n;
  }
  const int64_t n = (int64_t)ft.h_pairs.size();
  for (int64_t i = 0; i < n && i < cap; ++i) memcpy(out + 12 * i, &ft.h_pairs[(size_t)i], sizeof(StripPair));
  return n;
}

int64_t fused_strip_rows(const dsph_plan* plan, int32_t K, int64_t strip, int64_t n, const int32_t* xy, int64_t* rows) {
  if (!plan->fused || K < 2 || K - 1 > FUSED_DMAX) return -1;
  const FusedTiles& ft = get_tiles(plan, K - 1, false);
  if (!ft.ok || strip < 0) return -1;
  if (const QStripSet* s = record_strips(plan, ft, K)) {
    if (strip >= (int64_t)s->h_strips.size()) return -1;
    const QStrip& q = s->h_strips[(size_t)strip];
    const int ya = K == 5 ? q.ylo - 1 : q.ylo, yb = K == 5 ? q.yhi + 6 : q.yhi;
    for (int64_t i = 0; i < n; ++i) {
      const int x = std::min(std::max(xy[2 * i], q.xlo), q.xhi), y = std::min(std::max(xy[2 * i + 1], ya), yb);
      rows[i] = (int64_t)s->h_tab[(size_t)(q.tab + (y >> 4) * q.tws + (x >> 4))] + (int64_t)st_morton((unsigned)x & 15u, (unsigned)y & 15u);
    }
    return n;
  }
  if (strip >= (int64_t)ft.h_pairs.size()) return -1;
  for (int64_t i = 0; i < n; ++i) rows[i] = (int64_t)st_morton((unsigned)xy[2 * i], (unsigned)xy[2 * i + 1]);
  return n;
}

bool fused_strip_split(const dsph_plan* plan, int64_t N, int32_t* grid, int32_t* pieces, int32_t* wg_per_piece, int64_t* tape_rows) {
  if (!plan->fused || N < 1) return false;
  const FusedTiles& ft = get_tiles(plan, QS_D, false);
  if (!ft.ok || ft.q5.n == 0) return false;
  int g = 0, p = 0, w = 0;
  (void)qstrip_split(plan->fused->num_cu, ft.q5.tape_rows, N, ft.q5.tape_rows / std::max(1, ft.q5.n), &g, &p, &w);
  *grid = g; *pieces = p; *wg_per_piece = w; *tape_rows = ft.q5.tape_rows;
  return true;
}

bool fused_symmetric(const dsph_plan* plan) {
  FusedPlan* fp = plan->fused;
  std::lock_guard<std::mutex> lock(fp->mu);
  if (fp->symmetric >= 0) return fp->symmetric == 1;
  if (fp->host_released || plan->n_rows != plan->n_cols) return false;
  const int W = plan->width;
  const int64_t n = plan->n_rows;
  const int32_t* cols = fp->h_cols.data();
  const float* vals = fp->h_vals.data();
  bool sym = true;
  for (int64_t r = 0; r < n && sym; ++r)
    for (int j = 0; j < W; ++j) {
      const int64_t c = cols[r * W + j];
      const float v = vals[r * W + j];
      if (v == 0.f || c == r) continue;
      if (c < 0 || c >= n) { sym = false; break; }
      float back = 0.f;
      for (int i = 0; i < W; ++i)
        if (cols[c * W + i] == r) back += vals[c * W + i];
      if (fabsf(back - v) > 2.4e-7f * fmaxf(fabsf(back), fabsf(v))) { sym = false; break; }
    }
  fp->symmetric = sym ? 1 : 0;
  return sym;
}

}
```

deepsphere-cosmo-tf2_amd/csrc/dsphere_common.h:

```cpp
#pragma once

#include <hip/hip_runtime.h>
#include <stdint.h>

#include <vector>

#include "dsphere.h"

namespace dsph {

void set_error(const char* fmt, ...);
int hip_fail(hipError_t e, const char* what);

#define DSPH_HIP(call)                                           \
  do {                                                           \
    hipError_t e__ = (call);                                     \
    if (e__ != hipSuccess) return ::dsph::hip_fail(e__, #call);  \
  } while (0)

struct DeviceGuard {
  int prev = -1;
  bool ok = true;
  explicit DeviceGuard(int dev) {
    if (hipGetDevice(&prev) != hipSuccess) { ok = false; return; }
    if (prev != dev && hipSetDevice(dev) != hipSuccess) ok = false;
  }
  ~DeviceGuard() {
    if (prev >= 0) (void)hipSetDevice(prev);
  }
};

struct FusedPlan;

struct PlanOptions {
  int strips = 0;
  bool use_struct = true;
  bool use_tables = true;
  bool fork = true;
  int strip_seg = 0;
  int strip_min_rows = 4;
  bool strip_generic = false;
  int split_order = 0;
  bool tstep = true;
  int strip_form = 0;
  bool pack = true;
  int f16_xexp = 0;
};

}

struct dsph_plan {
  int device = 0;
  int64_t n_rows = 0;
  int64_t n_cols = 0;
  int32_t width = 0;
  int32_t* d_cols = nullptr;
  float* d_vals = nullptr;
  std::vector<int64_t> levels;
  dsph::PlanOptions opt;
  dsph::FusedPlan* fused = nullptr;
};

namespace dsph {

inline int64_t out_rows(const dsph_plan* p) { return p->levels.empty() ? p->n_rows : p->levels[0]; }
inline int32_t pad4(int32_t Fin) { return (Fin + 3) & ~3; }

int launch_cheb_step(const dsph_plan* plan, const float* in, int64_t in_rows, const float* prev,
                     int64_t prev_rows, float* out, int64_t out_rows, int64_t N, int32_t F,
                     float alpha, float beta, int64_t rows, hipStream_t stream);

int launch_cheb_contract(const float* const* planes, int64_t plane_rows, const float* w,
                         const float* bias, float* y, int64_t N, int64_t rows, int32_t Fin,
                         int32_t Fout, int32_t K, int32_t act, int32_t precision,
                         hipStream_t stream);

bool launch_cheb_tcontract(const float* const* planes, int64_t plane_rows, const float* w, const float* bias, float* y, int64_t N,
                           int64_t rows, int32_t Fin, int32_t Fout, int32_t K, int32_t act, int32_t precision, int num_cu,
                           hipStream_t stream, int* rc);

size_t wgrad_workspace_bytes(int64_t N, int64_t rows, int32_t Fin, int32_t Fout, int32_t K);
int launch_cheb_wgrad(const float* const* planes, int64_t plane_rows, const float* dy, float* dw,
                      int64_t N, int64_t rows, int32_t Fin, int32_t Fout, int32_t K, void* workspace,
                      size_t workspace_bytes, hipStream_t stream);

int launch_rows_pack(const float* src, int64_t src_rows, const int32_t* idx, int64_t n_idx,
                     float* buf, int64_t N, int32_t F, bool unpack, hipStream_t stream);

FusedPlan* fused_plan_build(const dsph_plan* plan, const int32_t* h_cols, const float* h_vals);
void fused_plan_destroy(FusedPlan* fp);
void fused_plan_invalidate(FusedPlan* fp);
bool fused_host_released(FusedPlan* fp);
int fused_prepare(const dsph_plan* plan, int32_t K, int32_t Fin, int32_t flags);
bool fused_supported(const dsph_plan* plan, int32_t Fin, int32_t Fout, int32_t K);
bool fused_weights_resident(const dsph_plan* plan, int32_t Fin, int32_t Fout, int32_t K);
bool fused_tile_counts(const dsph_plan* plan, int32_t K, int64_t* n_struct, int64_t* n_bfs);
int64_t fused_strip_tiles(const dsph_plan* plan, int64_t N, int32_t Fin, int32_t Fout, int32_t K, int32_t precision);
int64_t fused_strip_pairs(const dsph_plan* plan, int32_t K, int32_t* out, int64_t cap);
int64_t fused_strip_rows(const dsph_plan* plan, int32_t K, int64_t strip, int64_t n, const int32_t* xy, int64_t* rows);
bool fused_strip_split(const dsph_plan* plan, int64_t N, int32_t* grid, int32_t* pieces, int32_t* wg_per_piece, int64_t* tape_rows);
struct FusedPool {
  float* y;
  int32_t type;
};
bool fused_pool_ok(const dsph_plan* plan, int64_t N, int32_t Fin, int32_t Fout, int32_t K, int32_t act);
int launch_cheb_fused(const dsph_plan* plan, const float* x, const float* w, const float* bias,
                      float* y, int64_t N, int32_t Fin, int32_t Fout, int32_t K, int32_t act,
                      int32_t precision, float alpha_rest, float beta_rest, void* workspace,
                      size_t workspace_bytes, hipStream_t stream, int32_t part = 0, bool keep_weights = false,
                      const FusedPool* pool = nullptr);
bool fused_planes_supported(const dsph_plan* plan, int32_t Fin, int32_t K);
int launch_cheb_fused_planes(const dsph_plan* plan, const float* x, float* planes_out, int64_t N, int32_t Fin,
                             int32_t K, float alpha_rest, float beta_rest, hipStream_t stream);
bool fused_wgrad_supported(const dsph_plan* plan, int32_t Fin, int32_t Fout, int32_t K);
size_t fused_wgrad_workspace_bytes(const dsph_plan* plan, int32_t Fin, int32_t Fout, int32_t K);
int launch_fused_pad(const float* x, float* xp, int64_t rows, int32_t Fin, int32_t Fp, hipStream_t stream);
bool fused_qwgrad_applies(const dsph_plan* plan, int64_t N, int32_t Fin, int32_t Fout, int32_t K, int32_t precision);
size_t fused_qwgrad_workspace_bytes(const dsph_plan* plan);
int launch_cheb_fused_qwgrad(const dsph_plan* plan, const float* x, const float* dy, float* dw, int64_t N, int32_t Fin, int32_t Fout,
                             int32_t K, float alpha_rest, float beta_rest, void* workspace, size_t bfs_slab_bytes, hipStream_t stream);
int launch_cheb_fused_wgrad(const dsph_plan* plan, const float* x, const float* dy, float* dw, int64_t N,
                            int32_t Fin, int32_t Fout, int32_t K, int32_t precision, float alpha_rest, float beta_rest,
                            void* workspace, size_t workspace_bytes, hipStream_t stream, int32_t Fin_w = 0);
size_t fused_workspace_bytes(const dsph_plan* plan, int64_t N, int32_t Fin, int32_t Fout, int32_t K,
                             int32_t precision);
enum : uint32_t { IMG_BFS = 1, IMG_STRUCT = 2, IMG_STRIP = 4, IMG_ISTRIP = 8, IMG_QSTRIP = 16, IMG_SPLIT = 32, IMG_Q8 = 64 };
void fused_images_begin(const dsph_plan* plan, const void* ws, uint64_t key, bool keep);
bool fused_images_claim(const dsph_plan* plan, const void* ws, uint32_t bit);
void fused_images_forget(const dsph_plan* plan, const void* ws);
uint64_t fused_images_key(int32_t Fin, int32_t Fin_w, int32_t Fout, int32_t K, int32_t ld, int32_t precision, bool cheb, bool many, bool pack);

int fused_dmax();
bool split_applicable(const dsph_plan* plan, int32_t Fin, int32_t Fout, int32_t K);
size_t split_workspace_bytes(const dsph_plan* plan, int64_t N, int32_t Fin, int32_t Fout, int32_t K, int32_t precision);
int split_prepare(const dsph_plan* plan, int32_t K, int32_t Fin, int32_t Fout, int32_t flags);
int launch_split_forward(const dsph_plan* plan, const float* x, const float* w, const float* bias, float* y, int64_t N, int32_t Fin,
                         int32_t Fout, int32_t K, int32_t basis, int32_t act, int32_t precision, void* workspace,
                         size_t workspace_bytes, hipStream_t stream, bool keep_weights = false);

struct TStepTables {
  const int32_t* tile_off; const int32_t* ring_end; const int64_t* ell_off; const int32_t* region;
  const uint16_t* lcols; const float* lvals;
  int ntiles = 0, width = 0;
};
int tstep_width(int ell_width);
bool fused_tstep_tables(const dsph_plan* plan, TStepTables* out);
int launch_cheb_tstep(const TStepTables& tb, const float* in, const float* prev, float* out, int64_t rows, int64_t N, int32_t F, float alpha,
                      float beta, int num_cu, hipStream_t stream);
int fused_num_cu(const dsph_plan* plan);

struct LaunchBase {
  const float* x; const float* w; const float* bias; float* y;
  const float* gvals8; const float* gdiag;
  int64_t x_rows, y_rows, N;
  int32_t act, ld, num_cu;
  bool cheb;
  float* ypool = nullptr;
  int64_t ypool_rows = 0;
  int32_t pool = 0;
};

struct StructLaunch : LaunchBase {
  unsigned char* wfrag;
  const int32_t* tiles;
  int32_t ntiles, Fin, Fout, K, precision;
  int32_t Fin_w;
  const int32_t* tabrow = nullptr;
  const float* tabvals = nullptr;
  bool prep_weights = true;
  bool allow_pack = true;
};
int struct_build_rows(const dsph_plan* plan, float** gvals8, float** gdiag, unsigned char** flag);
int struct_patch_rows(const dsph_plan* plan, float* gvals8, float* gdiag, const int32_t* rows, const float* vals, int64_t n);
int struct_classify_tiles(const dsph_plan* plan, const unsigned char* d_flag, int ntiles, int D, int64_t out_rows,
                          unsigned char* h_cls, int dlimit = 4 );
bool struct_shape_ok(int32_t Fin, int32_t Fout, int32_t K);
size_t struct_wfrag_bytes(int32_t Fin, int32_t Fout, int32_t K);
int launch_cheb_struct(const StructLaunch& s, hipStream_t stream);
int launch_struct_act(float* y, int64_t rows, int32_t cols, int32_t ld, int32_t act, hipStream_t stream);
int launch_struct_act_tiles(float* y, const int32_t* d_tiles, int ntiles, int64_t N, int64_t y_rows, int32_t cols, int32_t ld,
                            int32_t act, hipStream_t stream);
int launch_residual_epilogue(float* y, const float* skip, int64_t n, float alpha, int32_t act, bool before, hipStream_t stream);

struct StripPair;
struct StripLaunch : LaunchBase {
  unsigned char* wimg;
  const StripPair* pairs;
  int32_t npairs, Fin, Fout, K, precision;
  bool prep_weights = true;
  bool generic = false;
};
bool strip_shape_ok(int32_t Fin, int32_t Fout, int32_t K);
size_t strip_wimg_bytes(int32_t Fin, int32_t Fout, int32_t K);
int launch_cheb_strip(const StripLaunch& s, hipStream_t stream);

struct QStrip;
struct QTapeLaunch : LaunchBase {
  unsigned char* wimg;
  const QStrip* strips;
  const int32_t* tab = nullptr;
  const int32_t* prefix;
  int64_t tape_rows;
  int32_t nstrips;
  bool f16 = false;
  int f16_xexp = 0;
  bool prep_weights = true;
};
int64_t qtape_split(int num_cu, int64_t tape_rows, int64_t N, int64_t mean_height, int run_in, int* grid, int* pieces, int* wg_per_piece);

struct QStripLaunch : QTapeLaunch {
  int32_t Fin, Fout;
};
bool qstrip_shape_ok(int32_t Fin, int32_t Fout, int32_t K);
size_t qstrip_wimg_bytes();
int64_t qstrip_split(int num_cu, int64_t tape_rows, int64_t N, int64_t mean_height, int* grid, int* pieces, int* wg_per_piece);
int launch_cheb_qstrip(const QStripLaunch& s, hipStream_t stream);

struct QStrip8Launch : QTapeLaunch {
  int32_t ld_w;
};
bool qstrip8_shape_ok(int32_t Fin, int32_t Fout, int32_t K);
size_t qstrip8_wimg_bytes();
int64_t qstrip8_split(int num_cu, int64_t tape_rows, int64_t N, int64_t mean_height, int* grid, int* pieces, int* wg_per_piece);
int launch_cheb_qstrip8(const QStrip8Launch& s, hipStream_t stream);

struct QWgradLaunch {
  const float* x; const float* dy;
  float* dw;
  float* slabs;
  const QStrip* strips; const int32_t* prefix;
  const int32_t* tab = nullptr;
  int64_t tape_rows;
  const float* gvals8; const float* gdiag;
  int64_t x_rows, dy_rows, N;
  int32_t nstrips, lddy, lddw, num_cu;
  bool cheb;
  bool accumulate = false;
};
bool qwgrad_shape_ok(int32_t Fin, int32_t Fout, int32_t K);
size_t qwgrad_slab_bytes(int num_cu);
int launch_cheb_qwgrad(const QWgradLaunch& s, hipStream_t stream);

struct IStripLaunch : LaunchBase {
  unsigned char* wimg;
  const StripPair* pairs;
  int32_t npairs, Fin, Fin_w, Fout, K, precision;
  int32_t nseg = 1;
  bool prep_weights = true;
};
int istrip_segments(const std::vector<int32_t>& heights, const std::vector<unsigned char>& second, int64_t N, int num_cu, int D,
                    bool narrow);
bool istrip_narrow(int32_t Fin_w);
bool istrip_pairs(int32_t Fin_w, int32_t Fout);
bool istrip_shape_ok(int32_t Fin, int32_t K);
size_t istrip_wimg_bytes(int32_t K, int32_t precision);
int launch_cheb_istrip(const IStripLaunch& s, hipStream_t stream);

__device__ __forceinline__ float apply_act(float v, int act) {
  switch (act) {
    case DSPH_ACT_RELU: return v > 0.f ? v : 0.f;
    case DSPH_ACT_ELU: return v > 0.f ? v : expm1f(v);
    case DSPH_ACT_SIGMOID: return 1.f / (1.f + expf(-v));
    case DSPH_ACT_TANH: return tanhf(v);
    default: return v;
  }
}

__device__ __forceinline__ unsigned xcd_remap(unsigned bid, unsigned nblk) {
  const unsigned q = nblk >> 3, r = nblk & 7u, xcd = bid & 7u, i = bid >> 3;
  return (xcd < r ? xcd * (q + 1) : r * (q + 1) + (xcd - r) * q) + i;
}

}
```

Measured before the change: 298,100.

## Admit rotated-neighbor tiles into quad strips with oriented row addressing

The strip planner now accepts neighbouring tiles whose Morton layout is rotated (0/90/180/270 degrees). It stores each tile's orientation in the low bits of the tile-table entry and uses a separate coefficient table with private patched rows for the edge tiles. The kernels decode the orientation into a base plus a signed stride per tile row, so input fetches follow rotated tiles without gathers. More of the sphere, such as face seams, can then run on the fast fused quad-strip path instead of fallback kernels. The cost is extra table memory, a larger coefficient allocation and a little more address arithmetic per row.

```diff
diff --git a/deepsphere-cosmo-tf2_amd/csrc/cheb_qstrip_kernel.h b/deepsphere-cosmo-tf2_amd/csrc/cheb_qstrip_kernel.h
--- a/deepsphere-cosmo-tf2_amd/csrc/cheb_qstrip_kernel.h
+++ b/deepsphere-cosmo-tf2_amd/csrc/cheb_qstrip_kernel.h
@@ -202,8 +202,13 @@
   auto tab_lane = [&](const QStrip& st, unsigned ci, int yrow) __attribute__((always_inline)) -> unsigned {
     return qt_tab_lane(a.tab, st, ci, min(max(yrow, st.ylo), st.yhi));
   };
+  auto tab_lane_c = [&](const QStrip& st, unsigned ci, int yrow) __attribute__((always_inline)) -> unsigned {
+    return qt_tab_lane(a.tab, st, st.tabc, ci, min(max(yrow, st.ylo), st.yhi));
+  };
   auto my_of = [&](int yrow) __attribute__((always_inline)) -> unsigned { return st_spread((unsigned)yrow & 15u) << 1; };
   auto my_next = [&](unsigned m) __attribute__((always_inline)) -> unsigned { return ((m | 0x55u) + 1u) & 0xaau; };
+  auto s_of = [&](int yrow) __attribute__((always_inline)) -> unsigned { return st_spread((unsigned)yrow & 15u); };
+  auto s_next = [&](unsigned m) __attribute__((always_inline)) -> unsigned { return ((m | 0xaau) + 1u) & 0x55u; };
   auto xfetch = [&](const char* xmap, unsigned xrow, qs_f4 (&xv)[XN]) __attribute__((always_inline)) {
     if (QS_ABL & 8) {
 #pragma unroll
@@ -326,7 +331,7 @@
       const int Xf = min(max(st.xs + 4 * xpix + xt, st.xlo), st.xhi);
       const int tc0 = max(st.xs, st.xlo) >> 4;
       const unsigned ciC = (unsigned)((Xc >> 4) - tc0), mXc = st_spread((unsigned)Xc & 15u);
-      const unsigned ciF = (unsigned)((Xf >> 4) - tc0), mXf = st_spread((unsigned)Xf & 15u);
+      const unsigned ciF = (unsigned)((Xf >> 4) - tc0), aXf = qt_apack(st_spread((unsigned)Xf & 15u));
       const int T3 = ((st.y1 - st.y0) + 2 * D + 1 + 3) / 3;
       const char* __restrict__ xmap = reinterpret_cast<const char*>(a.x) + (size_t)nq * a.x_rows * xrowb;
       QRow R[2][3];
@@ -341,15 +346,16 @@
       {
         qs_f4 cv, xv[XN];
         float cd;
-        cfetch(qt_row_in(st, tab_lane(st, ciC, ytop - 1), mXc, ytop - 1), cv, cd);
-        xfetch(xmap, qt_row_in(st, tab_lane(st, ciF, ytop), mXf, ytop), xv);
+        cfetch(qt_row_in(st, tab_lane_c(st, ciC, ytop - 1), mXc, ytop - 1), cv, cd);
+        xfetch(xmap, qt_row_oriented(st, tab_lane(st, ciF, ytop), aXf, ytop), xv);
         cw_wait(cv, cd);
         cstore(CRING - 1, cv, cd);
         xw_wait(xv);
         xstore(0, xv);
       }
-      unsigned bXf = tab_lane(st, ciF, ytop + 1), bXc = tab_lane(st, ciC, ytop);
-      unsigned myX = my_of(ytop + 1), myC = my_of(ytop);
+      QOriented oXf = qt_oriented(tab_lane(st, ciF, ytop + 1), aXf);
+      unsigned bXc = tab_lane_c(st, ciC, ytop);
+      unsigned sX = s_of(ytop + 1), myC = my_of(ytop);
       qt_step_barrier();
       auto step = [&](auto ph_c) __attribute__((always_inline)) {
         constexpr int PH = decltype(ph_c)::value;
@@ -370,9 +376,9 @@
         QS_STAMP(0);
         qs_f4 xv[XN];
         constexpr bool XLATE = H1;
-        if (myX == 0) bXf = tab_lane(st, ciF, ytop + 1);
-        if (myC == 0) bXc = tab_lane(st, ciC, ytop);
-        if (!XLATE) xfetch(xmap, bXf + (mXf | myX), xv);
+        if (sX == 0) oXf = qt_oriented(tab_lane(st, ciF, ytop + 1), aXf);
+        if (myC == 0) bXc = tab_lane_c(st, ciC, ytop);
+        if (!XLATE) xfetch(xmap, qt_row_at(oXf, sX), xv);
         const unsigned f0 = (unsigned)slot_top * ROWB + lane16, f1 = (unsigned)slot_ix(1) * ROWB + lane16, f2 = (unsigned)slot_ix(2) * ROWB + lane16;
         const unsigned f3 = (unsigned)slot_ix(3) * ROWB + lane16;
         constexpr bool N3 = CHEB;
@@ -392,7 +398,7 @@
                  { if (qq < QS_UPR) QS_UNIT<!CHEB, false>(R[0][L0], R[1][L0], qq, QS_LO0(c2)); else QS_UNIT<false, false>(R[0][L0], R[1][L1], qq - QS_UPR, QS_LO1(c2)); })
         qs_settle<9>(R[1][L2]);
         qs_settle<1>(R[0][L0]);
-        if (XLATE) xfetch(xmap, bXf + (mXf | myX), xv);
+        if (XLATE) xfetch(xmap, qt_row_at(oXf, sX), xv);
         QS_STAMP(2);
         QS_CHAIN(R[0][L0], false, 2, f2, QS_UPR, { c2h = chi_read(cslot_ix(2)); cfetch(bXc + (mXc | myC), cv, cd); if (H1) { QS_FR0(f3) } },
                  { QS_UNIT<false, N3>(R[1][L2], R[0][L2], qq, QS_HI(c3h)); })
@@ -427,7 +433,7 @@
         slot_top = snew;
         cs_top = cs_top + 1 == CRING ? 0 : cs_top + 1;
         ++ytop;
-        myX = my_next(myX);
+        sX = s_next(sX);
         myC = my_next(myC);
         qt_step_barrier();
         QS_STAMP(8);
@@ -466,7 +472,7 @@
       for (int nq = wg.map0; nq < a.N; nq += a.wg_per_piece) {
       const int Xf = min(max(st.xs + 4 * xpix + xt, st.xlo), st.xhi);
       const int tc0 = max(st.xs, st.xlo) >> 4;
-      const unsigned ciF = (unsigned)((Xf >> 4) - tc0), mXf = st_spread((unsigned)Xf & 15u);
+      const unsigned ciF = (unsigned)((Xf >> 4) - tc0), aXf = qt_apack(st_spread((unsigned)Xf & 15u));
       const int Xg = st.xs + 4 * p;
       const unsigned ciY = (unsigned)((min(max(Xg, st.xlo), st.xhi) >> 4) - tc0), mXg = st_spread((unsigned)Xg & 12u);
       const int cfirst = st.x0 - st.xs, clast = cfirst + st.w;
@@ -486,12 +492,13 @@
       qt_step_barrier();
       if (!X_BY_H) {
         qs_f4 xv[XN];
-        xfetch(xmap, qt_row_in(st, tab_lane(st, ciF, ytop), mXf, ytop), xv);
+        xfetch(xmap, qt_row_oriented(st, tab_lane(st, ciF, ytop), aXf, ytop), xv);
         xw_wait(xv);
         xstore(0, xv);
       }
-      unsigned bXf = X_BY_H ? 0u : tab_lane(st, ciF, ytop + 1), bY = tab_lane(st, ciY, st.y0);
-      unsigned myX = my_of(ytop + 1), myY = my_of(ytop - K);
+      QOriented oXf = qt_oriented(X_BY_H ? 0u : tab_lane(st, ciF, ytop + 1), aXf);
+      unsigned bY = tab_lane(st, ciY, st.y0);
+      unsigned sX = s_of(ytop + 1), myY = my_of(ytop - K);
       qt_step_barrier();
       auto step = [&](auto ph_c) __attribute__((always_inline)) {
         constexpr int PH = decltype(ph_c)::value;
@@ -511,9 +518,9 @@
         QS_STAMP_DECL
         QS_STAMP(0);
         qs_f4 xv[XN];
-        if (!X_BY_H && myX == 0) bXf = tab_lane(st, ciF, ytop + 1);
+        if (!X_BY_H && sX == 0) oXf = qt_oriented(tab_lane(st, ciF, ytop + 1), aXf);
         if (myY == 0) bY = tab_lane(st, ciY, ytop - K);
-        if (!X_BY_H) xfetch(xmap, bXf + (mXf | myX), xv);
+        if (!X_BY_H) xfetch(xmap, qt_row_at(oXf, sX), xv);
 #ifdef DSPH_QS_LEARLY
         constexpr bool LE = CHEB && H1;
 #else
@@ -632,7 +639,7 @@
         slot_top = snew;
         cs_top = cs_top + 1 == CRING ? 0 : cs_top + 1;
         ++ytop;
-        myX = my_next(myX);
+        sX = s_next(sX);
         myY = my_next(myY);
         qt_step_barrier();
         QS_STAMP(8);
diff --git a/deepsphere-cosmo-tf2_amd/csrc/cheb_qtape.h b/deepsphere-cosmo-tf2_amd/csrc/cheb_qtape.h
--- a/deepsphere-cosmo-tf2_amd/csrc/cheb_qtape.h
+++ b/deepsphere-cosmo-tf2_amd/csrc/cheb_qtape.h
@@ -26,7 +26,7 @@
   int32_t xlo, xhi;
   int32_t ylo, yhi;
   int32_t tab, tws;
-  int32_t pad[1];
+  int32_t tabc;
 };
 
 struct QTapePiece {
@@ -59,7 +59,7 @@
   {
     const QStrip g = strips[lo];
 #define QS_U(f) st.f = __builtin_amdgcn_readfirstlane(g.f)
-    QS_U(x0); QS_U(w); QS_U(xs); QS_U(y0); QS_U(y1); QS_U(xlo); QS_U(xhi); QS_U(ylo); QS_U(yhi); QS_U(tab); QS_U(tws);
+    QS_U(x0); QS_U(w); QS_U(xs); QS_U(y0); QS_U(y1); QS_U(xlo); QS_U(xhi); QS_U(ylo); QS_U(yhi); QS_U(tab); QS_U(tws); QS_U(tabc);
 #undef QS_U
   }
   const int h = st.y1 - st.y0;
@@ -70,16 +70,43 @@
   return len;
 }
 
-__device__ __forceinline__ unsigned qt_tab_lane(const int32_t* tab, const QStrip& st, unsigned ci, int yc) {
-  const int32_t* trow = tab + __builtin_amdgcn_readfirstlane(st.tab + (yc >> 4) * st.tws + (max(st.xs, st.xlo) >> 4));
+__device__ __forceinline__ unsigned qt_tab_lane(const int32_t* tab, const QStrip& st, int toff, unsigned ci, int yc) {
+  const int32_t* trow = tab + __builtin_amdgcn_readfirstlane(toff + (yc >> 4) * st.tws + (max(st.xs, st.xlo) >> 4));
   qs_i4 b;
   int b4;
   asm volatile("s_load_dwordx4 %0, %2, 0x0\n\ts_load_dword %1, %2, 0x10\n\ts_waitcnt lgkmcnt(0)" : "=&s"(b), "=&s"(b4) : "s"(trow) : "memory");
   return (unsigned)(ci == 0 ? b[0] : ci == 1 ? b[1] : ci == 2 ? b[2] : ci == 3 ? b[3] : b4);
 }
+__device__ __forceinline__ unsigned qt_tab_lane(const int32_t* tab, const QStrip& st, unsigned ci, int yc) {
+  return qt_tab_lane(tab, st, st.tab, ci, yc);
+}
 __device__ __forceinline__ unsigned qt_row_in(const QStrip& st, unsigned base, unsigned mX, int yrow) {
   const int yc = min(max(yrow, st.ylo), st.yhi);
   return base + (mX | (st_spread((unsigned)yc & 15u) << 1));
+}
+__host__ __device__ __forceinline__ void qt_rot(unsigned o, unsigned x, unsigned y, unsigned* gx, unsigned* gy) {
+  *gx = o == 0 ? x : o == 1 ? y : o == 2 ? 15u - x : 15u - y;
+  *gy = o == 0 ? y : o == 1 ? 15u - x : o == 2 ? 15u - y : x;
+}
+constexpr int QT_ORI_SHIFT = 3;
+struct QOriented {
+  unsigned ba;
+  int k;
+};
+__device__ __forceinline__ unsigned qt_apack(unsigned mX) {
+  const unsigned nX = 0x55u - mX;
+  return mX | (2u * nX) << 8 | (nX + 0xaau) << 16 | (2u * mX + 0x55u) << 24;
+}
+__device__ __forceinline__ QOriented qt_oriented(unsigned entry, unsigned apack) {
+  QOriented r;
+  r.ba = (entry & 0xffffff00u) | __builtin_amdgcn_ubfe(apack, entry, 8u);
+  r.k = __builtin_amdgcn_sbfe((int)0xfffe0102u, entry, 8u);
+  return r;
+}
+__device__ __forceinline__ unsigned qt_row_at(const QOriented& t, unsigned S) { return (unsigned)(__mul24(t.k, (int)S) + (int)t.ba); }
+__device__ __forceinline__ unsigned qt_row_oriented(const QStrip& st, unsigned entry, unsigned apack, int yrow) {
+  const int yc = min(max(yrow, st.ylo), st.yhi);
+  return qt_row_at(qt_oriented(entry, apack), st_spread((unsigned)yc & 15u));
 }
 
 __device__ __forceinline__ void qt_step_barrier() { asm volatile("s_waitcnt lgkmcnt(0)\n\ts_barrier" ::: "memory"); }
diff --git a/deepsphere-cosmo-tf2_amd/csrc/cheb_qwgrad_kernel.h b/deepsphere-cosmo-tf2_amd/csrc/cheb_qwgrad_kernel.h
--- a/deepsphere-cosmo-tf2_amd/csrc/cheb_qwgrad_kernel.h
+++ b/deepsphere-cosmo-tf2_amd/csrc/cheb_qwgrad_kernel.h
@@ -109,21 +109,31 @@
       const int cfirst = st.x0 - st.xs, clast = cfirst + st.w;
       const int xclo = sideQ ? st.x0 : st.xlo, xchi = sideQ ? st.x0 + st.w - 1 : st.xhi;
 #pragma unroll
-      for (int t = 0; t < 4; ++t) {
-        voff[t] = st_spread((unsigned)min(max(st.xs + 4 * p + t, xclo), xchi) & 15u) * srowb + (unsigned)(16 * cq + 4 * q4) * 4u;
-        colk[t] = !sideQ || (4 * p + t >= cfirst && 4 * p + t < clast);
-      }
+      for (int t = 0; t < 4; ++t) colk[t] = !sideQ || (4 * p + t >= cfirst && 4 * p + t < clast);
+      unsigned bV = 0;
+      int kV = 2;
+      auto set_tile = [&](unsigned entry) __attribute__((always_inline)) {
+        bV = entry & 0xffffff00u;
+#pragma unroll
+        for (int t = 0; t < 4; ++t) {
+          const QOriented o = qt_oriented(entry, qt_apack(st_spread((unsigned)min(max(st.xs + 4 * p + t, xclo), xchi) & 15u)));
+          voff[t] = (o.ba - bV) * srowb + (unsigned)(16 * cq + 4 * q4) * 4u;
+          kV = o.k;
+        }
+      };
       const int Xc = min(max(st.xs + 4 * p + cq, st.xlo), st.xhi);
       const int tc0 = max(st.xs, st.xlo) >> 4;
       const unsigned pk = (unsigned)((min(max(st.xs + 4 * p, xclo), xchi) >> 4) - tc0) | ((unsigned)((Xc >> 4) - tc0) << 4) | (st_spread((unsigned)Xc & 15u) << 8);
       const char* smap = sbase + (size_t)nq * srows * srowb;
       auto tab_lane = [&](unsigned ci, int yc) __attribute__((always_inline)) -> unsigned { return qt_tab_lane(a.tab, st, ci, yc); };
+      auto tab_lane_c = [&](unsigned ci, int yc) __attribute__((always_inline)) -> unsigned { return qt_tab_lane(a.tab, st, st.tabc, ci, yc); };
       const int rlo = sideQ ? st.y0 : st.ylo, rhi = sideQ ? st.y1 - 1 : st.yhi;
-      unsigned bV = tab_lane(pk & 15u, min(max(st.y0 - D, rlo), rhi)), bC = sideQ ? 0u : tab_lane((pk >> 4) & 15u, min(max(st.y0 - D, st.ylo), st.yhi));
+      set_tile(tab_lane(pk & 15u, min(max(st.y0 - D, rlo), rhi)));
+      unsigned bC = sideQ ? 0u : tab_lane_c((pk >> 4) & 15u, min(max(st.y0 - D, st.ylo), st.yhi));
       auto row_fetch = [&](int yrow, QRow& R) __attribute__((always_inline)) {
         const int yc = min(max(yrow, rlo), rhi);
-        if (yrow > rlo && yrow <= rhi && (yrow & 15) == 0) bV = tab_lane(pk & 15u, yc);
-        const unsigned rb = (bV + (st_spread((unsigned)yc & 15u) << 1)) * srowb;
+        if (yrow > rlo && yrow <= rhi && (yrow & 15) == 0) set_tile(tab_lane(pk & 15u, yc));
+        const unsigned rb = (unsigned)((int)bV + __mul24(kV, (int)st_spread((unsigned)yc & 15u))) * srowb;
 #pragma unroll
         for (int t = 0; t < 4; ++t) R.t[t] = *reinterpret_cast<const qs_f4*>(smap + (rb + voff[t]));
       };
@@ -140,7 +150,7 @@
       float cd = 0.f;
       auto coef_fetch = [&](int yrow) __attribute__((always_inline)) {
         const int yc = min(max(yrow, st.ylo), st.yhi);
-        if (yrow > st.ylo && yrow <= st.yhi && (yrow & 15) == 0) bC = tab_lane((pk >> 4) & 15u, yc);
+        if (yrow > st.ylo && yrow <= st.yhi && (yrow & 15) == 0) bC = tab_lane_c((pk >> 4) & 15u, yc);
         const size_t rid = bC + ((pk >> 8) | (st_spread((unsigned)yc & 15u) << 1));
         qt_cfetch(a.gvals8, a.gdiag, rid, q4, cv, cd);
       };
diff --git a/deepsphere-cosmo-tf2_amd/csrc/cheb_struct.hip b/deepsphere-cosmo-tf2_amd/csrc/cheb_struct.hip
--- a/deepsphere-cosmo-tf2_amd/csrc/cheb_struct.hip
+++ b/deepsphere-cosmo-tf2_amd/csrc/cheb_struct.hip
@@ -108,10 +108,14 @@
   }
 }
 
-int struct_build_rows(const dsph_plan* plan, float** gvals8, float** gdiag, unsigned char** flag) {
-  const int64_t n = plan->n_cols;
-  DSPH_HIP(hipMalloc((void**)gvals8, (size_t)n * 8 * sizeof(float)));
-  DSPH_HIP(hipMalloc((void**)gdiag, (size_t)n * sizeof(float)));
+int struct_build_rows(const dsph_plan* plan, int64_t rows_alloc, float** gvals8, float** gdiag, unsigned char** flag) {
+  const int64_t n = plan->n_cols, na = std::max(n, rows_alloc);
+  DSPH_HIP(hipMalloc((void**)gvals8, (size_t)na * 8 * sizeof(float)));
+  DSPH_HIP(hipMalloc((void**)gdiag, (size_t)na * sizeof(float)));
+  if (na > n) {
+    DSPH_HIP(hipMemsetAsync(*gvals8 + (size_t)n * 8, 0, (size_t)(na - n) * 8 * sizeof(float), 0));
+    DSPH_HIP(hipMemsetAsync(*gdiag + (size_t)n, 0, (size_t)(na - n) * sizeof(float), 0));
+  }
   DSPH_HIP(hipMalloc((void**)flag, (size_t)n));
 #ifdef DSPH_HOST_EMU
   for (int64_t r = 0; r < n; ++r) struct_row_body(r, plan->d_cols, plan->d_vals, (int)plan->width, plan->n_rows, *gvals8, *gdiag, *flag);
diff --git a/deepsphere-cosmo-tf2_amd/csrc/cheb_tiles.h b/deepsphere-cosmo-tf2_amd/csrc/cheb_tiles.h
--- a/deepsphere-cosmo-tf2_amd/csrc/cheb_tiles.h
+++ b/deepsphere-cosmo-tf2_amd/csrc/cheb_tiles.h
@@ -90,6 +90,8 @@
   float* d_gdiag = nullptr;
   unsigned char* d_rowflag = nullptr;
   bool rows_tried = false;
+  int64_t priv_row0 = 0;
+  int priv_cap = 0;
   bool host_released = false;
   int symmetric = -1;
   bool wide = false;
diff --git a/deepsphere-cosmo-tf2_amd/csrc/cheb_tiles.hip b/deepsphere-cosmo-tf2_amd/csrc/cheb_tiles.hip
--- a/deepsphere-cosmo-tf2_amd/csrc/cheb_tiles.hip
+++ b/deepsphere-cosmo-tf2_amd/csrc/cheb_tiles.hip
@@ -345,28 +345,38 @@
 struct QCand {
   int32_t tile;
   int32_t nbr[8];
+  unsigned char ori[8];
   int32_t tix;
   int32_t sheet, u, v;
   bool taken;
   bool barred;
 };
 
-static bool links_from_table(const int32_t* row, int D, int32_t ntiles, int32_t nbr[8]) {
+static bool links_from_table(const int32_t* row, int D, int32_t ntiles, bool rot, int32_t nbr[8], unsigned char ori[8]) {
   for (int d = 0; d < 8; ++d) {
     const int xa = ddx[d] < 0 ? ST_DMAX - D : (ddx[d] == 0 ? ST_DMAX : ST_DMAX + ST_TILE);
     const int xb = ddx[d] < 0 ? ST_DMAX : (ddx[d] == 0 ? ST_DMAX + ST_TILE : ST_DMAX + ST_TILE + D);
     const int ya = ddy[d] < 0 ? ST_DMAX - D : (ddy[d] == 0 ? ST_DMAX : ST_DMAX + ST_TILE);
     const int yb = ddy[d] < 0 ? ST_DMAX : (ddy[d] == 0 ? ST_DMAX + ST_TILE : ST_DMAX + ST_TILE + D);
-    int64_t base = -1;
-    for (int y = ya; y < yb; ++y)
-      for (int x = xa; x < xb; ++x) {
-        const int64_t r = row[st_cell_off((unsigned)x, (unsigned)y) / 64u];
-        const int64_t b = r - (int64_t)st_morton((unsigned)(x - ST_DMAX) & 15u, (unsigned)(y - ST_DMAX) & 15u);
-        if (b < 0 || (b & (FUSED_P - 1)) != 0 || (base >= 0 && b != base)) return false;
-        base = b;
-      }
-    if (base < 0 || base / FUSED_P >= ntiles) return false;
-    nbr[d] = (int32_t)(base / FUSED_P);
+    bool found = false;
+    for (unsigned o = 0; o < (rot ? 4u : 1u) && !found; ++o) {
+      int64_t base = -1;
+      bool same = true;
+      for (int y = ya; y < yb && same; ++y)
+        for (int x = xa; x < xb && same; ++x) {
+          const int64_t r = row[st_cell_off((unsigned)x, (unsigned)y) / 64u];
+          unsigned gx, gy;
+          qt_rot(o, (unsigned)(x - ST_DMAX) & 15u, (unsigned)(y - ST_DMAX) & 15u, &gx, &gy);
+          const int64_t b = r - (int64_t)st_morton(gx, gy);
+          if (b < 0 || (b & (FUSED_P - 1)) != 0 || (base >= 0 && b != base)) same = false;
+          base = b;
+        }
+      if (!same || base < 0 || base / FUSED_P >= ntiles) continue;
+      nbr[d] = (int32_t)(base / FUSED_P);
+      ori[d] = (unsigned char)o;
+      found = true;
+    }
+    if (!found) return false;
   }
   return true;
 }
@@ -377,6 +387,8 @@
   if (D == Q8_D) return (int64_t)w * h * 275 - ns * (16 * (int64_t)h + Q8_RUNIN) * 26;
   return (int64_t)w * h * 187 - ns * (16 * (int64_t)h + 2 * D + 6) * 28;
 }
+
+constexpr int QT_SLIVER = 60;
 
 static int32_t assign_sheets(std::vector<QCand>& cands, int32_t ntiles) {
   const int n = (int)cands.size();
@@ -400,7 +412,9 @@
       const QCand a = cands[(size_t)queue[h]];
       for (int d = 0; d < 8; d += 2) {
         const int b = cand_at(a.nbr[d]);
-        if (b < 0 || cands[(size_t)b].sheet >= 0 || cands[(size_t)b].nbr[(d + 4) & 7] != a.tile) continue;
+        if (b < 0 || cands[(size_t)b].sheet >= 0 || cands[(size_t)b].nbr[(d + 4) & 7] != a.tile || a.ori[d] != 0 ||
+            cands[(size_t)b].ori[(d + 4) & 7] != 0)
+          continue;
         const int64_t u = (int64_t)a.u + ddx[d], v = (int64_t)a.v + ddy[d];
         if (u <= -OFF + 2 || u >= OFF - 2 || v <= -OFF + 2 || v >= OFF - 2) continue;
         const uint64_t k = key_of(sh, u, v);
@@ -438,8 +452,79 @@
   }
 }
 
+struct QPatches {
+  const std::vector<int32_t>* t_rows = nullptr;
+  const std::vector<float>* t_vals = nullptr;
+  int64_t priv_row0 = 0;
+  int priv_cap = 0, priv_used = 0;
+  std::vector<int32_t> rows;
+  std::vector<float> vals;
+  std::unordered_map<int32_t, size_t> at;
+  std::vector<int32_t> r_rows;
+  std::vector<float> r_vals;
+  std::unordered_map<int32_t, size_t> r_at;
+  std::vector<std::pair<int, int>> r_priv;
+  void begin() { r_rows.clear(); r_vals.clear(); r_at.clear(); r_priv.clear(); }
+  bool put(int32_t row, const float* v) {
+    auto g = at.find(row);
+    if (g != at.end()) return memcmp(&vals[g->second * 9], v, 9 * sizeof(float)) == 0;
+    auto l = r_at.find(row);
+    if (l != r_at.end()) return memcmp(&r_vals[l->second * 9], v, 9 * sizeof(float)) == 0;
+    r_at[row] = r_rows.size();
+    r_rows.push_back(row);
+    r_vals.insert(r_vals.end(), v, v + 9);
+    return true;
+  }
+  int64_t priv_base(int slot) {
+    for (const auto& pr : r_priv)
+      if (pr.first == slot) return priv_row0 + (int64_t)(priv_used + pr.second) * FUSED_P;
+    if (priv_used + (int)r_priv.size() >= priv_cap) return -1;
+    r_priv.push_back({slot, (int)r_priv.size()});
+    return priv_row0 + (int64_t)(priv_used + r_priv.back().second) * FUSED_P;
+  }
+  void commit() {
+    for (size_t i = 0; i < r_rows.size(); ++i) {
+      at[r_rows[i]] = rows.size();
+      rows.push_back(r_rows[i]);
+      vals.insert(vals.end(), r_vals.begin() + 9 * i, r_vals.begin() + 9 * i + 9);
+    }
+    priv_used += (int)r_priv.size();
+  }
+};
+static bool patch_tile(const QCand& q, int i, int j, int TW, const std::vector<int32_t>& t, const std::vector<int32_t>& to, int D,
+                       QPatches& pt) {
+  const int32_t r0 = q.tile * FUSED_P;
+  const int blo = ST_DMAX - D + 1, bhi = ST_DMAX + ST_TILE - 1 + D - 1;
+  for (int y = blo; y <= bhi; ++y)
+    for (int x = blo; x <= bhi; ++x) {
+      const size_t cell = (size_t)q.tix * ST_CELLS + st_cell_off((unsigned)x, (unsigned)y) / 64u;
+      const int32_t r = (*pt.t_rows)[cell];
+      const float* v = &(*pt.t_vals)[cell * ST_TABV];
+      const int sx = x < ST_DMAX ? -1 : (x >= ST_DMAX + ST_TILE ? 1 : 0), sy = y < ST_DMAX ? -1 : (y >= ST_DMAX + ST_TILE ? 1 : 0);
+      if (sx == 0 && sy == 0) {
+        if (!pt.put(r, v)) return false;
+        continue;
+      }
+      if (r == r0) continue;
+      int d = 0;
+      while (ddx[d] != sx || ddy[d] != sy) ++d;
+      const size_t slot = (size_t)(j + sy) * TW + (i + sx);
+      const unsigned lx = (unsigned)(x - ST_DMAX) & 15u, ly = (unsigned)(y - ST_DMAX) & 15u;
+      unsigned gx, gy;
+      qt_rot((unsigned)to[slot], lx, ly, &gx, &gy);
+      if (t[slot] != q.nbr[d] || to[slot] != q.ori[d] || (int64_t)t[slot] * FUSED_P + st_morton(gx, gy) != r) return false;
+      if (to[slot] == 0) {
+        if (!pt.put(r, v)) return false;
+        continue;
+      }
+      const int64_t pb = pt.priv_base((int)slot);
+      if (pb < 0 || !pt.put((int32_t)(pb + st_morton(lx, ly)), v)) return false;
+    }
+  return true;
+}
+
 static void build_qtstrips(std::vector<QCand>& cands, int32_t ntiles, int D, std::vector<QStrip>& strips, std::vector<int32_t>& tab,
-                           int64_t* n_taken) {
+                           int64_t* n_taken, QPatches* pt = nullptr) {
   strips.clear();
   tab.clear();
   *n_taken = 0;
@@ -474,8 +559,9 @@
             const int s0 = stack.back().first, hh = stack.back().second;
             stack.pop_back();
             const int wmax = (int)x - s0;
-            for (int w = std::min(wmax, 1000); w >= std::max(1, std::min(wmax, 1000) - 3); --w) {
-              const int64_t g = qt_gain(w, hh, D);
+            const int wtop = std::min(wmax, 1000);
+            for (int w = wtop; w >= std::max(1, wtop - 3); --w) {
+              const int64_t g = qt_gain(w, hh, D) - (pt ? (int64_t)(wtop - w) * hh * QT_SLIVER : 0);
               if (g > best) { best = g; bu = s0; bv = (int)y - hh + 1; bw = w; bh = hh; }
             }
             start = s0;
@@ -485,7 +571,7 @@
       }
       if (best <= 0) break;
       const int TW = bw + 2, TH = bh + 2;
-      std::vector<int32_t> t((size_t)TW * TH, -1);
+      std::vector<int32_t> t((size_t)TW * TH, -1), to((size_t)TW * TH, 0);
       bool good = true;
       auto inside = [&](int i, int j) { return i >= 1 && i <= bw && j >= 1 && j <= bh; };
       for (int j = 1; j <= bh && good; ++j)
@@ -496,20 +582,34 @@
           for (int d = 0; d < 8 && good; ++d) {
             const int i2 = i + ddx[d], j2 = j + ddy[d];
             int32_t& slot = t[(size_t)j2 * TW + i2];
+            int32_t& slot_o = to[(size_t)j2 * TW + i2];
             if (inside(i2, j2)) {
               const int32_t c2 = grid[(size_t)((bv + j2 - 1) * GW + (bu + i2 - 1))];
-              if (cands[(size_t)c2].tile != q.nbr[d]) good = false;
-            } else if (slot < 0) slot = q.nbr[d];
-            else if (slot != q.nbr[d]) good = false;
+              if (cands[(size_t)c2].tile != q.nbr[d] || q.ori[d] != 0) good = false;
+            } else if (slot < 0) { slot = q.nbr[d]; slot_o = q.ori[d]; }
+            else if (slot != q.nbr[d] || slot_o != q.ori[d]) good = false;
           }
         }
+      if (good && pt) {
+        pt->begin();
+        for (int j = 1; j <= bh && good; ++j)
+          for (int i = 1; i <= bw && good; ++i) {
+            const QCand& q = cands[(size_t)grid[(size_t)((bv + j - 1) * GW + (bu + i - 1))]];
+            if (q.tix >= 0) good = patch_tile(q, i, j, TW, t, to, D, *pt);
+          }
+      }
       if (!good) {
         for (int j = 0; j < bh; ++j)
           for (int i = 0; i < bw; ++i) grid[(size_t)((bv + j) * GW + (bu + i))] = -2;
         continue;
       }
       const int32_t toff = (int32_t)tab.size();
+      for (size_t k = 0; k < t.size(); ++k) tab.push_back(t[k] < 0 ? 0 : t[k] * FUSED_P | to[k] << QT_ORI_SHIFT);
       for (int32_t tile : t) tab.push_back(tile < 0 ? 0 : tile * FUSED_P);
+      if (pt) {
+        for (const auto& pr : pt->r_priv) tab[(size_t)toff + t.size() + (size_t)pr.first] = (int32_t)(pt->priv_row0 + (int64_t)(pt->priv_used + pr.second) * FUSED_P);
+        pt->commit();
+      }
       for (int j = 0; j < bh; ++j)
         for (int i = 0; i < bw; ++i) {
           int32_t& c = grid[(size_t)((bv + j) * GW + (bu + i))];
@@ -524,7 +624,7 @@
         q.x0 = x0; q.w = std::min(use, X1 - x0); q.xs = x0 - lead;
         q.y0 = Y0; q.y1 = Y1;
         q.xlo = X0 - D; q.xhi = X1 - 1 + D; q.ylo = Y0 - D; q.yhi = Y1 - 1 + D;
-        q.tab = toff; q.tws = TW;
+        q.tab = toff; q.tws = TW; q.tabc = toff + TW * TH;
         strips.push_back(q);
       }
     }
@@ -607,12 +707,20 @@
 static void ensure_rows(const dsph_plan* plan, FusedPlan* fp) {
   if (fp->rows_tried) return;
   fp->rows_tried = true;
-  if (struct_build_rows(plan, &fp->d_gvals8, &fp->d_gdiag, &fp->d_rowflag) != DSPH_OK) {
+  const int64_t tiles = (plan->n_cols + FUSED_P - 1) / FUSED_P;
+  int64_t cap = 64;
+  while ((cap - 64) * (cap - 64) < 64 * tiles) cap += 8;
+  cap = std::min(cap, tiles);
+  if ((tiles + cap) * FUSED_P > 0x7fffffffLL) cap = 0;
+  fp->priv_row0 = tiles * FUSED_P;
+  fp->priv_cap = (int)cap;
+  if (struct_build_rows(plan, (tiles + cap) * FUSED_P, &fp->d_gvals8, &fp->d_gdiag, &fp->d_rowflag) != DSPH_OK) {
     if (fp->d_gvals8) (void)hipFree(fp->d_gvals8);
     if (fp->d_gdiag) (void)hipFree(fp->d_gdiag);
     if (fp->d_rowflag) (void)hipFree(fp->d_rowflag);
     fp->d_gvals8 = fp->d_gdiag = nullptr;
     fp->d_rowflag = nullptr;
+    fp->priv_cap = 0;
   }
 }
 
@@ -831,7 +939,7 @@
   return c;
 }
 
-static void quad_strips5(const Graph& g, int D, const Classes& c, FusedTiles& ft, HostTables& h) {
+static void quad_strips5(const Graph& g, int D, const Classes& c, const FusedPlan* fp, FusedTiles& ft, HostTables& h) {
   std::vector<QCand> cands;
   cands.reserve(c.r_in.size() + c.t_in.tiles.size());
   for (int32_t t : c.r_in) cands.push_back(morton_cand(t, g.ntiles));
@@ -844,18 +952,37 @@
       if (q.nbr[d] == ragged) return true;
     return false;
   };
+  std::vector<unsigned char> is_g((size_t)g.ntiles, 0);
+  for (int32_t t : c.g_in) is_g[(size_t)t] = 1;
+  for (int32_t t : c.g_bd) is_g[(size_t)t] = 1;
+  auto rotated_beside_g = [&](const QCand& q) {
+    bool rot = false, beside = false;
+    for (int d = 0; d < 8; ++d) {
+      rot = rot || q.ori[d] != 0;
+      beside = beside || (q.nbr[d] >= 0 && is_g[(size_t)q.nbr[d]]);
+    }
+    return rot && beside;
+  };
 #ifdef DSPH_ABLATE
   const bool only_r = getenv("DSPH_QT_ONLY_R") != nullptr;
+  const bool no_rot = getenv("DSPH_QT_NO_ROT") != nullptr;
 #else
-  const bool only_r = false;
+  const bool only_r = false, no_rot = false;
 #endif
   for (size_t i = 0; i < c.t_in.tiles.size() && !only_r; ++i) {
     QCand q{};
     q.tile = c.t_in.tiles[i]; q.tix = (int32_t)i; q.taken = false;
-    if (links_from_table(&c.t_in.rows[i * ST_CELLS], D, g.ntiles, q.nbr)) cands.push_back(q);
-  }
-  for (QCand& q : cands) q.barred = beside_ragged(q);
-  build_qtstrips(cands, g.ntiles, D, ft.q5.h_strips, ft.q5.h_tab, &ft.q5.n_tiles);
+    if (links_from_table(&c.t_in.rows[i * ST_CELLS], D, g.ntiles, !no_rot, q.nbr, q.ori)) cands.push_back(q);
+  }
+  for (QCand& q : cands) q.barred = beside_ragged(q) || rotated_beside_g(q);
+  QPatches pt;
+  pt.t_rows = &c.t_in.rows;
+  pt.t_vals = &c.t_in.vals;
+  pt.priv_row0 = fp->priv_row0;
+  pt.priv_cap = fp->priv_cap;
+  build_qtstrips(cands, g.ntiles, D, ft.q5.h_strips, ft.q5.h_tab, &ft.q5.n_tiles, &pt);
+  h.patch_rows.swap(pt.rows);
+  h.patch_vals.swap(pt.vals);
   std::vector<int32_t> r_rest;
   std::vector<unsigned char> t_taken(c.t_in.tiles.size(), 0);
   for (size_t i = 0; i < cands.size(); ++i) {
@@ -864,19 +991,8 @@
   }
   h.qrrest = joined(std::move(r_rest), c.r_bd);
   TTabs t_rest;
-  for (size_t i = 0; i < c.t_in.tiles.size(); ++i) {
-    if (!t_taken[i]) {
-      t_rest.add(c.t_in, i);
-      continue;
-    }
-    const int blo = ST_DMAX - D + 1, bhi = ST_DMAX + ST_TILE - 1 + D - 1;
-    for (int y = blo; y <= bhi; ++y)
-      for (int x = blo; x <= bhi; ++x) {
-        const size_t cell = i * ST_CELLS + st_cell_off((unsigned)x, (unsigned)y) / 64u;
-        h.patch_rows.push_back(c.t_in.rows[cell]);
-        h.patch_vals.insert(h.patch_vals.end(), c.t_in.vals.begin() + cell * ST_TABV, c.t_in.vals.begin() + cell * ST_TABV + 9);
-      }
-  }
+  for (size_t i = 0; i < c.t_in.tiles.size(); ++i)
+    if (!t_taken[i]) t_rest.add(c.t_in, i);
   h.qt = joined(std::move(t_rest), c.t_bd);
 }
 
@@ -961,7 +1077,7 @@
   h.part = joined(c.g_in, c.g_bd);
   pair_strips(g, D, fp->num_cu, full, c, ft, h);
   if (!full && D == QS_D && plan->opt.strips != 2 && plan->opt.strip_form == 0 && fp->d_gvals8 != nullptr)
-    quad_strips5(g, D, c, ft, h);
+    quad_strips5(g, D, c, fp, ft, h);
   if (!cls8.empty()) quad_strips8(g, D, cls8, ft, h);
   complements(c, ft, h);
   h.r = joined(c.r_in, c.r_bd);
@@ -1035,7 +1151,10 @@
     const int ya = K == 5 ? q.ylo - 1 : q.ylo, yb = K == 5 ? q.yhi + 6 : q.yhi;
     for (int64_t i = 0; i < n; ++i) {
       const int x = std::min(std::max(xy[2 * i], q.xlo), q.xhi), y = std::min(std::max(xy[2 * i + 1], ya), yb);
-      rows[i] = (int64_t)s->h_tab[(size_t)(q.tab + (y >> 4) * q.tws + (x >> 4))] + (int64_t)st_morton((unsigned)x & 15u, (unsigned)y & 15u);
+      const int32_t e = s->h_tab[(size_t)(q.tab + (y >> 4) * q.tws + (x >> 4))];
+      unsigned gx, gy;
+      qt_rot(((unsigned)e >> QT_ORI_SHIFT) & 3u, (unsigned)x & 15u, (unsigned)y & 15u, &gx, &gy);
+      rows[i] = (int64_t)(e & ~(FUSED_P - 1)) + (int64_t)st_morton(gx, gy);
     }
     return n;
   }
diff --git a/deepsphere-cosmo-tf2_amd/csrc/dsphere_common.h b/deepsphere-cosmo-tf2_amd/csrc/dsphere_common.h
--- a/deepsphere-cosmo-tf2_amd/csrc/dsphere_common.h
+++ b/deepsphere-cosmo-tf2_amd/csrc/dsphere_common.h
@@ -170,7 +170,7 @@
   bool prep_weights = true;
   bool allow_pack = true;
 };
-int struct_build_rows(const dsph_plan* plan, float** gvals8, float** gdiag, unsigned char** flag);
+int struct_build_rows(const dsph_plan* plan, int64_t rows_alloc, float** gvals8, float** gdiag, unsigned char** flag);
 int struct_patch_rows(const dsph_plan* plan, float* gvals8, float* gdiag, const int32_t* rows, const float* vals, int64_t n);
 int struct_classify_tiles(const dsph_plan* plan, const unsigned char* d_flag, int ntiles, int D, int64_t out_rows,
                           unsigned char* h_cls, int dlimit = 4 );
```

Result: no change. 299,300, median of 6 (+0.4%).
